# genetics-statistics/GEMMA

Hardware: AMD Instinct MI355X
Metric: SNPs/s (-lmm 1 Wald) at n=20k on 1/2/4/8 MI355X; U^T x HBM GB/s vs roofline (higher is better)
Workload: dtype f64 (U^T x as int8-digit MFMA products with exact int32 accumulation; every column of U scaled by its exact maximum and rounded to 6 base-256 digits = 2^-48 of that maximum -- fp64 keeps 2^-53 per entry; value_strict / strict_leg (7g6m: U^T x at or below the fp64 GEMM's own error) and fp64_gemm_path

## Files before the change

### gemma_amd/build.py

```python
import os
import shutil
import subprocess

HERE = os.path.dirname(os.path.abspath(__file__))
CSRC = os.path.join(HERE, "csrc")
LIB = os.path.join(HERE, "libgemma_hip.so")
UNITS = {
    "gemma_hip.hip": ["dgemm_mfma.hip.h", "lmm_grid.hip.h", "i8gemm.hip.h", "i8gemm_sparse.hip.h", "i8gemm_sparse2.hip.h", "i8gemm_sparse2_r16.hip.h", "i8gemm_dense16.hip.h", "lmm_assoc.hip.h",
                      "lmm_search.hip.h", "comm.hip.h", "comm_shm.hpp", "kin_i8.hip.h", "ingest.hip.h", "qc.hip.h", "lm_assoc.hip.h", "mvlmm.hip.h",
                      "mvlmm_kernels.hip.h", "eigh_tu.h", "tu_common.h",
                      "abi_kinship.inc.h", "abi_eigen_qc.inc.h", "abi_lmm_stage.inc.h", "abi_utx.inc.h", "abi_lmm_batch.inc.h",
                      "abi_mvlmm.inc.h", "abi_gxe_lm.inc.h", "abi_kept_comm.inc.h", "abi_vc.inc.h", "vc_tu.h", "abi_prdt.inc.h", "prdt_tu.h",
                      "abi_mqs.inc.h", "mqs_tu.h", "abi_cor.inc.h", "cor_tu.h"],
    "eigh_tu.hip": ["dgemm_mfma.hip.h", "eigh.hip.h", "eigh2.hip.h", "eigh_tu.h", "tu_common.h"],
    "vc_tu.hip": ["dgemm_mfma.hip.h", "spd_inv.hip.h", "vc.hip.h", "vc_tu.h", "tu_common.h", "host_linalg.h", "../../include/gemma_vc_hybrid.hpp"],
    "prdt_tu.hip": ["dgemm_mfma.hip.h", "geno_mv.hip.h", "dev_common.hip.h", "eigh_tu.h", "prdt_tu.h", "tu_common.h"],
    "mqs_tu.hip": ["dgemm_mfma.hip.h", "mqs.hip.h", "dev_common.hip.h", "mqs_tu.h", "tu_common.h", "host_linalg.h"],
    "cor_tu.hip": ["dgemm_mfma.hip.h", "cor.hip.h", "dev_common.hip.h", "cor_tu.h", "tu_common.h"],
    "mvlmm_kernels.hip": ["mvlmm.hip.h", "mvlmm_kernels.hip.h"],
    "mvlmm_kernels_wide.hip": ["mvlmm.hip.h", "mvlmm_kernels.hip.h"],
    "mvlmm_kernels_rt.hip": ["mvlmm.hip.h", "mvlmm_kernels.hip.h"],
    "mvlmm_kernels_d6.hip": ["mvlmm.hip.h", "mvlmm_kernels.hip.h"],
    "mvlmm_kernels_d7.hip": ["mvlmm.hip.h", "mvlmm_kernels.hip.h"],
    "mvlmm_kernels_d8.hip": ["mvlmm.hip.h", "mvlmm_kernels.hip.h"],
}
PUBLIC_HEADER_USERS = ("gemma_hip.hip", "eigh_tu.hip", "vc_tu.hip", "prdt_tu.hip", "mqs_tu.hip", "cor_tu.hip")
SOURCES = list(UNITS)
HEADERS = sorted({h for hs in UNITS.values() for h in hs})


def hipcc():
    for cand in (os.environ.get("HIPCC"), "/opt/rocm/bin/hipcc", shutil.which("hipcc")):
        if cand and os.path.exists(cand):
            return cand
    raise RuntimeError("hipcc not found: the gfx950 library cannot be built")


def stale():
    if not os.path.exists(LIB):
        return True
    t = os.path.getmtime(LIB)
    deps = [os.path.join(CSRC, f) for f in SOURCES + HEADERS]
    deps.append(os.path.join(HERE, "..", "include", "gemma_hip.h"))
    return any(os.path.getmtime(d) > t for d in deps)


def build(force=False, verbose=False):
    if not force and not stale():
        return LIB
    cc = hipcc()
    objdir = os.path.join(HERE, "_obj")
    os.makedirs(objdir, exist_ok=True)
    procs, objs = [], []
    for src in SOURCES:
        obj = os.path.join(objdir, src.replace(".hip", ".o"))
        objs.append(obj)
        hdrs = UNITS[src]
        deps = [os.path.join(CSRC, f) for f in [src] + hdrs]
        if src in PUBLIC_HEADER_USERS:
            deps.append(os.path.join(HERE, "..", "include", "gemma_hip.h"))
        if not force and os.path.exists(obj) and all(os.path.getmtime(d) <= os.path.getmtime(obj) for d in deps):
            continue
        cmd = [cc, "--offload-arch=gfx950", "-O3", "-std=c++17", "-fPIC", "-c", os.path.join(CSRC, src), "-o", obj]
        if verbose:
            print(" ".join(cmd))
        procs.append((cmd, subprocess.Popen(cmd, cwd=CSRC)))
    for cmd, pr in procs:
        if pr.wait() != 0:
            raise subprocess.CalledProcessError(pr.returncode, cmd)
    cmd = [cc, "--offload-arch=gfx950", "-fPIC", "-shared", "-o", LIB] + objs
    if verbose:
        print(" ".join(cmd))
    subprocess.check_call(cmd, cwd=CSRC)
    return LIB


if __name__ == "__main__":
    print(build(force=True, verbose=True))
```

### gemma_amd/csrc/abi_gxe_lm.inc.h

```cpp

extern "C" int gemma_hip_lmm_set_env(const double *env) {
  NEED_INIT();
  if (!g_ctx.lmm_active) return fail(GEMMA_HIP_ESTATE, "lmm_set_env before lmm_setup");
  if (!env) return fail(GEMMA_HIP_EINVAL, "lmm_set_env: null pointer");
  const size_t n = g_ctx.cfg.n, c = g_ctx.cfg.n_cvt;
  if (c + 2 > (size_t)GEN_CMAX_WIDE)
    return fail(GEMMA_HIP_EINVAL, "lmm_set_env: n_cvt + 2 = %zu covariates not supported (<= %d)", c + 2, GEN_CMAX_WIDE);
  if (n <= c + 3) return fail(GEMMA_HIP_EINVAL, "lmm_set_env: n <= n_cvt + 3");
  if (g_ctx.gxe_env.reserve(n * 8) || g_ctx.gxe_UtWt.reserve((c + 1) * n * 8))
    return fail(GEMMA_HIP_ENOMEM, "lmm_set_env: buffers");
  HIPCHK(hipMemcpy(g_ctx.gxe_env.p, env, n * 8, hipMemcpyHostToDevice));
  HIPCHK(hipMemcpy(g_ctx.gxe_UtWt.p, g_ctx.UtWt.p, c * n * 8, hipMemcpyDeviceToDevice));
  HIPCHK(launch_dgemm('T', 'N', (long)n, 1, (long)n, 1.0, g_ctx.U, (long)n, g_ctx.gxe_env.as<double>(), 1, 0.0,
                      g_ctx.gxe_UtWt.as<double>() + c * n, 1, false, false, 0));
  HIPCHK(hipDeviceSynchronize());
  const double df = (double)n - (double)(c + 2) - 1.0;
  g_ctx.gxe_lnbeta = lgamma(df / 2.0) + lgamma(0.5) - lgamma(df / 2.0 + 0.5);
  g_ctx.gxe_ready = true;
  return GEMMA_HIP_OK;
}

extern "C" int gemma_hip_lmm_gxe_batch_d(int kind, const void *geno, size_t l, size_t ld, gemma_sumstat *out_d,
                                         void *stream) {
  NEED_INIT();
  if (!g_ctx.lmm_active || !g_ctx.gxe_ready) return fail(GEMMA_HIP_ESTATE, "lmm_gxe_batch before lmm_setup + lmm_set_env");
  if (l == 0) return GEMMA_HIP_OK;
  if (kind == GEMMA_GENO_F64_IDV_MAJOR) return fail(GEMMA_HIP_EINVAL, "lmm_gxe_batch: SNP-major input only");
  int rc = check_batch_args("lmm_gxe_batch", kind, geno, l, ld, out_d);
  if (rc) return rc;
  hipStream_t s = S(stream);
  const size_t n = g_ctx.cfg.n, c = g_ctx.cfg.n_cvt;
  const size_t ldx = (n + 1) & ~(size_t)1;
  if (int rcf = xp_flush(s)) return rcf;
  if (g_ctx.X.reserve(l * ldx * 8) || g_ctx.UtX.reserve(l * ldx * 8) || g_ctx.gxe_Z.reserve(l * ldx * 8) ||
      g_ctx.gxe_UtZ.reserve(l * ldx * 8) || g_ctx.gxe_flip.reserve(l * sizeof(int)))
    return fail(GEMMA_HIP_ENOMEM, "lmm_gxe_batch: cannot allocate 4 x %zu bytes", l * ldx * 8);
  double *X = g_ctx.X.as<double>(), *UtX = g_ctx.UtX.as<double>();
  double *Z = g_ctx.gxe_Z.as<double>(), *UtZ = g_ctx.gxe_UtZ.as<double>();
  {
    ProfScope ps(GEMMA_STAGE_INGEST, s);
    IngestGxeArgs a;
    a.src = geno; a.ld = (long)ld; a.l = (long)l;
    a.idx_map = g_ctx.have_map ? g_ctx.idx_map.as<int>() : nullptr;
    a.n = (int)n; a.env = g_ctx.gxe_env.as<double>(); a.X = X; a.Z = Z; a.ldo = (long)ldx;
    a.flip = g_ctx.gxe_flip.as<int>();
    const unsigned grid = (unsigned)((l + 3) / 4);
    if (kind == GEMMA_GENO_PLINK_2BIT)
      hipLaunchKernelGGL(ingest_gxe_kernel<true>, dim3(grid), dim3(256), 0, s, a);
    else
      hipLaunchKernelGGL(ingest_gxe_kernel<false>, dim3(grid), dim3(256), 0, s, a);
    HIPCHK(hipGetLastError());
  }
  {
    ProfScope ps(GEMMA_STAGE_UTX_GEMM, s);
    const double *Ug;
    long ldu;
    int rcu = gemm_U(&Ug, &ldu, s);
    if (rcu) return rcu;
    HIPCHK(launch_dgemm('N', 'N', (long)l, (long)n, (long)n, 1.0, X, (long)ldx, Ug, ldu, 0.0, UtX, (long)ldx,
                        false, false, s));
    HIPCHK(launch_dgemm('N', 'N', (long)l, (long)n, (long)n, 1.0, Z, (long)ldx, Ug, ldu, 0.0, UtZ, (long)ldx,
                        false, false, s));
  }
  AssocArgs a = g_ctx.assoc_proto;
  a.UtX = UtX; a.UtZ = UtZ; a.flip = g_ctx.gxe_flip.as<int>();
  a.ld = (long)ldx; a.l = (long)l;
  a.eval = g_ctx.eval; a.Uty = g_ctx.Uty; a.UtWt = g_ctx.gxe_UtWt.as<double>();
  a.out = reinterpret_cast<SumStat *>(out_d);
  a.lnbeta_half_df = g_ctx.gxe_lnbeta;
  a.grid_T = nullptr;
  a.have_grid = 0;
  a.have_logdet_ends = g_ctx.assoc_proto.have_logdet_ends;
  const unsigned grid = (unsigned)((l + 3) / 4);
  {
    ProfScope ps(GEMMA_STAGE_ASSOC, s);
    switch (c + 2) {
    case 3: hipLaunchKernelGGL(lmm_gxe_kernel<3>, dim3(grid), dim3(256), 0, s, a); break;
    case 4: hipLaunchKernelGGL(lmm_gxe_kernel<4>, dim3(grid), dim3(256), 0, s, a); break;
    default:
      if (c + 2 > (size_t)GEN_CMAX) {
        int rcw = wide_attr(lmm_gxe_wide_kernel);
        if (rcw) return rcw;
        hipLaunchKernelGGL(lmm_gxe_wide_kernel, dim3((unsigned)l), dim3(64), wide_lds_bytes(c + 2), s, a, (int)(c + 2));
      } else {
        hipLaunchKernelGGL(lmm_gxe_generic_kernel, dim3(grid), dim3(256), 0, s, a, (int)(c + 2));
      }
      break;
    }
    HIPCHK(hipGetLastError());
  }
  return GEMMA_HIP_OK;
}

extern "C" int gemma_hip_lmm_gxe_batch(int kind, const void *geno, size_t l, size_t ld, gemma_sumstat *out) {
  NEED_INIT();
  if (!g_ctx.lmm_active || !g_ctx.gxe_ready) return fail(GEMMA_HIP_ESTATE, "lmm_gxe_batch before lmm_setup + lmm_set_env");
  if (l == 0) return GEMMA_HIP_OK;
  if (kind == GEMMA_GENO_F64_IDV_MAJOR) return fail(GEMMA_HIP_EINVAL, "lmm_gxe_batch: SNP-major input only");
  int rc = check_batch_args("lmm_gxe_batch", kind, geno, l, ld, out);
  if (rc) return rc;
  const size_t esz = (kind == GEMMA_GENO_PLINK_2BIT) ? 1 : 8;
  if (g_ctx.stage_in.reserve(l * ld * esz) || g_ctx.stage_out.reserve(l * sizeof(gemma_sumstat)))
    return fail(GEMMA_HIP_ENOMEM, "lmm_gxe_batch: staging %zu bytes", l * ld * esz);
  HIPCHK(hipMemcpy(g_ctx.stage_in.p, geno, l * ld * esz, hipMemcpyHostToDevice));
  rc = gemma_hip_lmm_gxe_batch_d(kind, g_ctx.stage_in.p, l, ld, g_ctx.stage_out.as<gemma_sumstat>(), nullptr);
  if (rc) return rc;
  HIPCHK(hipMemcpy(out, g_ctx.stage_out.p, l * sizeof(gemma_sumstat), hipMemcpyDeviceToHost));
  return GEMMA_HIP_OK;
}

extern "C" int gemma_hip_dbg_utx(int kind, const void *geno, size_t l, size_t ld, int path, double *UtX_host) {
  NEED_INIT();
  if (!g_ctx.lmm_active) return fail(GEMMA_HIP_ESTATE, "dbg_utx before lmm_setup");
  if (l == 0) return GEMMA_HIP_OK;
  int rc = check_batch_args("dbg_utx", kind, geno, l, ld, UtX_host);
  if (rc) return rc;
  const size_t n = g_ctx.cfg.n;
  const size_t rows = (kind == GEMMA_GENO_F64_IDV_MAJOR) ? n : l;
  const size_t esz = (kind == GEMMA_GENO_PLINK_2BIT) ? 1 : 8;
  if (g_ctx.stage_in.reserve(rows * ld * esz)) return fail(GEMMA_HIP_ENOMEM, "dbg_utx: staging");
  HIPCHK(hipMemcpy(g_ctx.stage_in.p, geno, rows * ld * esz, hipMemcpyHostToDevice));
  double *UtX;
  size_t ldx;
  rc = compute_utx(kind, g_ctx.stage_in.p, l, ld, path ? 1 : 0, &UtX, &ldx, 0);
  if (rc) return rc;
  HIPCHK(hipMemcpy2D(UtX_host, n * 8, UtX, ldx * 8, n * 8, l, hipMemcpyDeviceToHost));
  return GEMMA_HIP_OK;
}

extern "C" int gemma_hip_lmm_batch(int kind, const void *geno, size_t l, size_t ld, gemma_sumstat *out) {
  NEED_INIT();
  if (!g_ctx.lmm_active) return fail(GEMMA_HIP_ESTATE, "lmm_batch before lmm_setup");
  if (l == 0) return GEMMA_HIP_OK;
  const size_t n = g_ctx.cfg.n;
  const size_t per_row = (kind == GEMMA_GENO_PLINK_2BIT && g_ctx.have_map) ? g_ctx.ni_total : n;
  const size_t need = min_ld_for(kind, per_row, l);
  if (need == (size_t)-1) return fail(GEMMA_HIP_EINVAL, "lmm_batch: unknown geno_kind %d", kind);
  if (!geno || !out || ld < need) return fail(GEMMA_HIP_EINVAL, "lmm_batch: ld=%zu < %zu", ld, need);
  const size_t rows = (kind == GEMMA_GENO_F64_IDV_MAJOR) ? n : l;
  const size_t esz = (kind == GEMMA_GENO_PLINK_2BIT) ? 1 : 8;
  if (g_ctx.stage_in.reserve(rows * ld * esz) || g_ctx.stage_out.reserve(l * sizeof(gemma_sumstat)))
    return fail(GEMMA_HIP_ENOMEM, "lmm_batch: staging %zu bytes", rows * ld * esz);
  HIPCHK(hipMemcpy2D(g_ctx.stage_in.p, ld * esz, geno, ld * esz, need * esz, rows, hipMemcpyHostToDevice));
  int rc = gemma_hip_lmm_batch_d(kind, g_ctx.stage_in.p, l, ld, g_ctx.stage_out.as<gemma_sumstat>(), nullptr);
  if (rc) return rc;
  HIPCHK(hipMemcpy(out, g_ctx.stage_out.p, l * sizeof(gemma_sumstat), hipMemcpyDeviceToHost));
  return GEMMA_HIP_OK;
}

extern "C" int gemma_hip_lm_setup(int a_mode, size_t n, size_t n_cvt, const double *W, const double *y) {
  NEED_INIT();
  g_ctx.knobs.load();
  if (g_ctx.lmm_active) return fail(GEMMA_HIP_ESTATE, "lm_setup while an LMM run is active");
  if (a_mode < 51 || a_mode > 54) return fail(GEMMA_HIP_EINVAL, "lm_setup: a_mode %d (51..54)", a_mode);
  if (!W || !y || n == 0 || n_cvt == 0 || n_cvt > (size_t)LM_CMAX || n <= n_cvt + 1 || n > 0x7fffffffUL)
    return fail(GEMMA_HIP_EINVAL, "lm_setup: bad arguments (n_cvt 1..%d)", LM_CMAX);
  const int c = (int)n_cvt;
  std::vector<double> WtW((size_t)c * c, 0.0), Wt((size_t)c * n), Wty(c, 0.0);
  double yy = 0.0;
  for (size_t i = 0; i < n; ++i) {
    yy += y[i] * y[i];
    for (int a = 0; a < c; ++a) {
      Wt[(size_t)a * n + i] = W[i * c + a];
      Wty[a] += W[i * c + a] * y[i];
      for (int b = 0; b < c; ++b) WtW[(size_t)a * c + b] += W[i * c + a] * W[i * c + b];
    }
  }
  if (!invert_small(WtW, c)) return fail(GEMMA_HIP_EINVAL, "lm_setup: W^T W is singular");
  double d = 0.0;
  for (int a = 0; a < c; ++a) {
    double t = 0.0;
    for (int b = 0; b < c; ++b) t += WtW[(size_t)a * c + b] * Wty[b];
    d += t * Wty[a];
  }
  if (g_ctx.lm_Wt.reserve(Wt.size() * 8) || g_ctx.lm_y.reserve(n * 8) || g_ctx.lm_small.reserve(((size_t)c * c + c) * 8))
    return fail(GEMMA_HIP_ENOMEM, "lm_setup: allocation");
  HIPCHK(hipMemcpy(g_ctx.lm_Wt.p, Wt.data(), Wt.size() * 8, hipMemcpyHostToDevice));
  HIPCHK(hipMemcpy(g_ctx.lm_y.p, y, n * 8, hipMemcpyHostToDevice));
  HIPCHK(hipMemcpy(g_ctx.lm_small.p, WtW.data(), (size_t)c * c * 8, hipMemcpyHostToDevice));
  HIPCHK(hipMemcpy(g_ctx.lm_small.as<double>() + (size_t)c * c, Wty.data(), c * 8, hipMemcpyHostToDevice));
  LmArgs &a = g_ctx.lm_proto;
  memset(&a, 0, sizeof a);
  a.Wt = g_ctx.lm_Wt.as<double>();
  a.y = g_ctx.lm_y.as<double>();
  a.WtWi = g_ctx.lm_small.as<double>();
  a.Wty = g_ctx.lm_small.as<double>() + (size_t)c * c;
  a.yPwy = yy - d;
  a.n = (int)n;
  a.c = c;
  a.test_mode = a_mode - 50;
  const double df = (double)n - (double)c - 1.0;
  a.lnbeta_half_df = lgamma(df / 2.0) + lgamma(0.5) - lgamma(df / 2.0 + 0.5);
  g_ctx.cfg.n = n;
  g_ctx.cfg.n_cvt = n_cvt;
  g_ctx.have_map = false;
  g_ctx.ni_total = 0;
  g_ctx.lm_active = true;
  return GEMMA_HIP_OK;
}

extern "C" int gemma_hip_lm_batch_d(int kind, const void *geno, size_t l, size_t ld, gemma_sumstat *out_d, void *stream) {
  NEED_INIT();
  if (!g_ctx.lm_active) return fail(GEMMA_HIP_ESTATE, "lm_batch before lm_setup");
  if (l == 0) return GEMMA_HIP_OK;
  const size_t n = g_ctx.cfg.n;
  const size_t per_row = (kind == GEMMA_GENO_PLINK_2BIT && g_ctx.have_map) ? g_ctx.ni_total : n;
  const size_t need = min_ld_for(kind, per_row, l);
  if (need == (size_t)-1) return fail(GEMMA_HIP_EINVAL, "lm_batch: unknown geno_kind %d", kind);
  if (!geno || !out_d || ld < need) return fail(GEMMA_HIP_EINVAL, "lm_batch: ld=%zu < %zu", ld, need);
  hipStream_t s = S(stream);
  const size_t ldx = (n + 1) & ~(size_t)1;
  if (g_ctx.X.reserve(l * ldx * 8)) return fail(GEMMA_HIP_ENOMEM, "lm_batch: cannot allocate %zu bytes", l * ldx * 8);
  double *X = g_ctx.X.as<double>();
  {
    ProfScope ps(GEMMA_STAGE_INGEST, s);
    if (kind == GEMMA_GENO_F64_IDV_MAJOR) {
      dim3 grid((unsigned)((l + 31) / 32), (unsigned)((n + 31) / 32));
      hipLaunchKernelGGL(transpose_kernel, grid, dim3(32, 8), 0, s, reinterpret_cast<const double *>(geno), (long)n,
                         (long)l, (long)ld, X, (long)ldx);
    } else {
      IngestArgs a;
      a.src = geno; a.ld = (long)ld; a.l = (long)l;
      a.idx_map = g_ctx.have_map ? g_ctx.idx_map.as<int>() : nullptr;
      a.n = (int)n; a.dst = X; a.ldo = (long)ldx; a.k_mode = 0;
      const unsigned grid = (unsigned)((l + 3) / 4);
      if (kind == GEMMA_GENO_PLINK_2BIT)
        hipLaunchKernelGGL(ingest_lmm_kernel<true>, dim3(grid), dim3(256), 0, s, a);
      else
        hipLaunchKernelGGL(ingest_lmm_kernel<false>, dim3(grid), dim3(256), 0, s, a);
    }
    HIPCHK(hipGetLastError());
  }
  LmArgs a = g_ctx.lm_proto;
  a.X = X; a.ld = (long)ldx; a.l = (long)l;
  a.out = reinterpret_cast<SumStat *>(out_d);
  {
    ProfScope ps(GEMMA_STAGE_ASSOC, s);
    hipLaunchKernelGGL(lm_assoc_kernel, dim3((unsigned)((l + 3) / 4)), dim3(256), 0, s, a);
    HIPCHK(hipGetLastError());
  }
  return GEMMA_HIP_OK;
}

extern "C" int gemma_hip_lm_batch(int kind, const void *geno, size_t l, size_t ld, gemma_sumstat *out) {
  NEED_INIT();
  if (!g_ctx.lm_active) return fail(GEMMA_HIP_ESTATE, "lm_batch before lm_setup");
  if (l == 0) return GEMMA_HIP_OK;
  const size_t n = g_ctx.cfg.n;
  const size_t per_row = (kind == GEMMA_GENO_PLINK_2BIT && g_ctx.have_map) ? g_ctx.ni_total : n;
  const size_t need = min_ld_for(kind, per_row, l);
  if (need == (size_t)-1) return fail(GEMMA_HIP_EINVAL, "lm_batch: unknown geno_kind %d", kind);
  if (!geno || !out || ld < need) return fail(GEMMA_HIP_EINVAL, "lm_batch: ld=%zu < %zu", ld, need);
  const size_t rows = (kind == GEMMA_GENO_F64_IDV_MAJOR) ? n : l;
  const size_t esz = (kind == GEMMA_GENO_PLINK_2BIT) ? 1 : 8;
  if (g_ctx.stage_in.reserve(rows * ld * esz) || g_ctx.stage_out.reserve(l * sizeof(gemma_sumstat)))
    return fail(GEMMA_HIP_ENOMEM, "lm_batch: staging %zu bytes", rows * ld * esz);
  HIPCHK(hipMemcpy2D(g_ctx.stage_in.p, ld * esz, geno, ld * esz, need * esz, rows, hipMemcpyHostToDevice));
  int rc = gemma_hip_lm_batch_d(kind, g_ctx.stage_in.p, l, ld, g_ctx.stage_out.as<gemma_sumstat>(), nullptr);
  if (rc) return rc;
  HIPCHK(hipMemcpy(out, g_ctx.stage_out.p, l * sizeof(gemma_sumstat), hipMemcpyDeviceToHost));
  return GEMMA_HIP_OK;
}

extern "C" int gemma_hip_lm_finish(void) {
  NEED_INIT();
  if (!g_ctx.lm_active) return fail(GEMMA_HIP_ESTATE, "lm_finish before lm_setup");
  HIPCHK(hipDeviceSynchronize());
  g_ctx.lm_Wt.release(); g_ctx.lm_y.release(); g_ctx.lm_small.release();
  g_ctx.X.release(); g_ctx.stage_in.release(); g_ctx.stage_out.release(); g_ctx.idx_map.release();
  g_ctx.lm_active = false;
  return GEMMA_HIP_OK;
}

extern "C" int gemma_hip_lmm_null(size_t n, size_t n_cvt, const double *eval, const double *UtW,
                                  const double *Uty, double l_min, double l_max, size_t n_region,
                                  double trace_G, double *out8) {
  NEED_INIT();
  if (!eval || !UtW || !Uty || !out8 || n == 0 || n_cvt == 0 || n_cvt > (size_t)GEN_CMAX_WIDE + 1)
    return fail(GEMMA_HIP_EINVAL, "lmm_null: bad arguments (n_cvt 1..%d)", GEN_CMAX_WIDE + 1);
  if (!(l_max > l_min) || n_region == 0 || n_region > (size_t)ASSOC_MAX_REGION || n <= n_cvt)
    return fail(GEMMA_HIP_EINVAL, "lmm_null: l_min/l_max/n_region/n");
  DevBuf dE, dW, dWt, dY, dO;
  auto cleanup = [&]() { dE.release(); dW.release(); dWt.release(); dY.release(); dO.release(); };
  if (dE.reserve(n * 8) || dW.reserve(n * n_cvt * 8) || dWt.reserve(n * n_cvt * 8) || dY.reserve(n * 8) ||
      dO.reserve(sizeof(NullOut))) {
    cleanup();
    return fail(GEMMA_HIP_ENOMEM, "lmm_null: allocation");
  }
  hipError_t e = hipMemcpy(dE.p, eval, n * 8, hipMemcpyHostToDevice);
  if (e == hipSuccess) e = hipMemcpy(dW.p, UtW, n * n_cvt * 8, hipMemcpyHostToDevice);
  if (e == hipSuccess) e = hipMemcpy(dY.p, Uty, n * 8, hipMemcpyHostToDevice);
  if (e == hipSuccess) {
    dim3 grid((unsigned)((n_cvt + 31) / 32), (unsigned)((n + 31) / 32));
    hipLaunchKernelGGL(transpose_kernel, grid, dim3(32, 8), 0, 0, dW.as<double>(), (long)n, (long)n_cvt,
                       (long)n_cvt, dWt.as<double>(), (long)n);
    AssocArgs a;
    memset(&a, 0, sizeof a);
    a.n = (int)n; a.n_region = (int)n_region; a.l_min = l_min; a.l_max = l_max;
    a.eval = dE.as<double>(); a.Uty = dY.as<double>(); a.UtWt = dWt.as<double>();
    const double lambda_interval = log(l_max / l_min) / (double)n_region;
    for (size_t i = 0; i <= n_region; ++i) a.lam_grid[i] = l_min * exp(lambda_interval * (double)i);
    NullOut *o = dO.as<NullOut>();
    switch (n_cvt) {
    case 1: hipLaunchKernelGGL(lmm_null_kernel<0>, dim3(1), dim3(64), 0, 0, a, o); break;
    case 2: hipLaunchKernelGGL(lmm_null_kernel<1>, dim3(1), dim3(64), 0, 0, a, o); break;
    case 3: hipLaunchKernelGGL(lmm_null_kernel<2>, dim3(1), dim3(64), 0, 0, a, o); break;
    case 4: hipLaunchKernelGGL(lmm_null_kernel<3>, dim3(1), dim3(64), 0, 0, a, o); break;
    case 5: hipLaunchKernelGGL(lmm_null_kernel<4>, dim3(1), dim3(64), 0, 0, a, o); break;
    default:
      if (n_cvt - 1 > (size_t)GEN_CMAX) {
        (void)hipFuncSetAttribute(reinterpret_cast<const void *>(lmm_null_wide_kernel),
                                  hipFuncAttributeMaxDynamicSharedMemorySize, (int)wide_lds_bytes(GEN_CMAX_WIDE));
        hipLaunchKernelGGL(lmm_null_wide_kernel, dim3(1), dim3(64), wide_lds_bytes(n_cvt - 1), 0, a, (int)n_cvt - 1, o);
      } else {
        hipLaunchKernelGGL(lmm_null_generic_kernel, dim3(1), dim3(64), 0, 0, a, (int)n_cvt - 1, o);
      }
      break;
    }
    e = hipGetLastError();
  }
  NullOut h;
  if (e == hipSuccess) e = hipMemcpy(&h, dO.p, sizeof h, hipMemcpyDeviceToHost);
  cleanup();
  if (e != hipSuccess) return fail(GEMMA_HIP_ERUNTIME, "lmm_null: %s", hipGetErrorString(e));
  out8[0] = h.l_mle; out8[1] = h.logl_mle; out8[2] = h.l_remle; out8[3] = h.logl_remle;
  double arg = -1.0 / h.dev2_remle, d1 = arg;
  if (arg < 0.001) d1 = fabs(arg);
  const double se = (d1 < 0.0) ? NAN : sqrt(d1);
  out8[4] = trace_G * h.l_remle / (trace_G * h.l_remle + 1.0);
  out8[5] = trace_G / ((trace_G * h.l_remle + 1.0) * (trace_G * h.l_remle + 1.0)) * se;
  out8[7] = h.Pyy_remle / (double)(n - n_cvt);
  out8[6] = out8[7] * h.l_remle;
  return GEMMA_HIP_OK;
}

extern "C" int gemma_hip_lmm_finish(double *time_UtX_min, double *time_opt_min) {
  NEED_INIT();
  if (!g_ctx.lmm_active) return fail(GEMMA_HIP_ESTATE, "lmm_finish before lmm_setup");
  HIPCHK(hipDeviceSynchronize());
  pipe_release();
  xp_release();
  prof_collect(GEMMA_STAGE_UTX_GEMM);
  prof_collect(GEMMA_STAGE_UTX_POST);
  prof_collect(GEMMA_STAGE_ASSOC);
  if (time_UtX_min)
    *time_UtX_min = (g_ctx.prof[GEMMA_STAGE_UTX_GEMM].acc_ms + g_ctx.prof[GEMMA_STAGE_UTX_POST].acc_ms) / 60000.0;
  if (time_opt_min) *time_opt_min = g_ctx.prof[GEMMA_STAGE_ASSOC].acc_ms / 60000.0;
  g_ctx.own_U.release(); g_ctx.own_eval.release(); g_ctx.own_Uty.release(); g_ctx.own_UtW.release();
  g_ctx.UtWt.release(); g_ctx.idx_map.release(); g_ctx.X.release(); g_ctx.UtX.release();
  g_ctx.stage_in.release(); g_ctx.stage_out.release();
  g_ctx.grid_R.release(); g_ctx.grid_F.release(); g_ctx.grid_T.release();
  g_ctx.table_P.release();
  g_ctx.cheb_R.release(); g_ctx.cheb_F.release(); g_ctx.cheb_T.release(); g_ctx.cheb_slots.release();
  g_ctx.cheb_list.release(); g_ctx.cheb_count.release(); g_ctx.cheb_D.release(); g_ctx.cheb_Ck.release();
  g_ctx.cheb_Gk.release(); g_ctx.cheb_Lk.release(); g_ctx.cheb_iv.release(); g_ctx.cheb_dends.release(); g_ctx.cheb_res.release();
  g_ctx.i8_Bt.release(); g_ctx.i8_q.release(); g_ctx.i8_qinv.release(); g_ctx.i8_cmax.release(); g_ctx.i8_A.release(); g_ctx.i8_C.release();
  raster_release();
  g_ctx.i8_mean.release(); g_ctx.i8_meta.release(); g_ctx.i8_rowsur.release(); g_ctx.i8_colsum.release(); g_ctx.i8_surlist.release();
  g_ctx.i8_ready = false;
  g_ctx.i8_colsum_ready = false;
  g_ctx.gxe_env.release(); g_ctx.gxe_UtWt.release(); g_ctx.gxe_Z.release(); g_ctx.gxe_UtZ.release();
  g_ctx.mv_Yt.release(); g_ctx.mv_out.release(); g_ctx.mv_scratch.release();
  g_ctx.mv_ready = g_ctx.mv_gxe = false;
  g_ctx.gxe_flip.release();
  g_ctx.gxe_ready = false;
  g_ctx.U = g_ctx.eval = g_ctx.Uty = nullptr;
  g_ctx.U_even_of = nullptr;
  g_ctx.U_even.release();
  g_ctx.lmm_active = false;
  return GEMMA_HIP_OK;
}
```

### gemma_amd/csrc/abi_kinship.inc.h

```cpp

extern "C" int gemma_hip_kin_begin(size_t n_total, int k_mode) {
  NEED_INIT();
  if (n_total == 0) return fail(GEMMA_HIP_EINVAL, "kin_begin: n_total == 0");
  if (k_mode != 1 && k_mode != 2) return fail(GEMMA_HIP_EINVAL, "kin_begin: k_mode %d", k_mode);
  g_ctx.qc_G.release(); g_ctx.qc_M.release(); g_ctx.qc_W.release(); g_ctx.qc_O.release();
  g_ctx.kin_ingested_valid = false;
  if (g_ctx.kin_K.reserve(n_total * n_total * 8))
    return fail(GEMMA_HIP_ENOMEM, "kin_begin: cannot allocate K (%zu bytes)", n_total * n_total * 8);
  HIPCHK(hipMemsetAsync(g_ctx.kin_K.p, 0, n_total * n_total * 8, 0));
  g_ctx.kin_active = true;
  g_ctx.kin_n = n_total;
  g_ctx.kin_mode = k_mode;
  g_ctx.kin_ns = 0;
  g_ctx.knobs.load();
  g_ctx.kin_i8 = (k_mode == 1) && g_ctx.knobs.kin_i8;
  g_ctx.kin_i8_used = false;
  return GEMMA_HIP_OK;
}

static void kin_i8_release() {
  g_ctx.kin_GtG.release(); g_ctx.kin_S.release(); g_ctx.kin_a.release(); g_ctx.kin_At.release(); g_ctx.kin_Gt.release();
  g_ctx.kin_A2.release(); g_ctx.kin_cnt.release(); g_ctx.kin_off.release(); g_ctx.kin_listS.release();
  g_ctx.kin_listJ.release(); g_ctx.kin_sub.release(); g_ctx.kin_cj.release(); g_ctx.kin_flag.release();
  g_ctx.kin_tmap.release();
  g_ctx.kin_tmap_tm = g_ctx.kin_tmap_tn = g_ctx.kin_tmap_count = 0;
  g_ctx.kin_i8_used = false;
}

static int kin_i8_tile_map(int tiles_m, int tiles_n) {
  if (g_ctx.kin_tmap_tm == tiles_m && g_ctx.kin_tmap_tn == tiles_n && g_ctx.kin_tmap.p) return GEMMA_HIP_OK;
  std::vector<int> map;
  const int GM = 8;
  for (int first = 0; first < tiles_m; first += GM) {
    const int gsz = std::min(GM, tiles_m - first);
    for (int tn = first >> 1; tn < tiles_n; ++tn)
      for (int tm = first; tm < first + gsz; ++tm)
        if (tn >= (tm >> 1)) {
          map.push_back(tm);
          map.push_back(tn);
        }
  }
  if (g_ctx.kin_tmap.reserve(map.size() * sizeof(int))) return fail(GEMMA_HIP_ENOMEM, "kin_add: tile map");
  HIPCHK(hipMemcpy(g_ctx.kin_tmap.p, map.data(), map.size() * sizeof(int), hipMemcpyHostToDevice));
  g_ctx.kin_tmap_tm = tiles_m;
  g_ctx.kin_tmap_tn = tiles_n;
  g_ctx.kin_tmap_count = (int)(map.size() / 2);
  return GEMMA_HIP_OK;
}

static int kin_add_i8(const void *geno, size_t l, size_t ld, hipStream_t s) {
  const size_t n = g_ctx.kin_n;
  const size_t ldk = (n + I8_BK - 1) / I8_BK * I8_BK;
  const size_t ldl = (l + I8_BK - 1) / I8_BK * I8_BK;
  const size_t rows_a = (n + I8P_BM - 1) / I8P_BM * I8P_BM;
  const size_t rows_b = (n + I8_BN - 1) / I8_BN * I8_BN;
  const size_t rows_t = std::max(rows_a, rows_b);
  if (!g_ctx.kin_i8_used) {
    if (g_ctx.kin_GtG.reserve(n * n * 8) || g_ctx.kin_S.reserve(n * n * 8) || g_ctx.kin_a.reserve((n + 1) * 8))
      return fail(GEMMA_HIP_ENOMEM, "kin_add: integer-path accumulators (%zu bytes)", 2 * n * n * 8);
    HIPCHK(hipMemsetAsync(g_ctx.kin_GtG.p, 0, n * n * 8, s));
    HIPCHK(hipMemsetAsync(g_ctx.kin_S.p, 0, n * n * 8, s));
    HIPCHK(hipMemsetAsync(g_ctx.kin_a.p, 0, (n + 1) * 8, s));
    g_ctx.kin_i8_used = true;
  }
  if (g_ctx.i8_A.reserve(l * ldk) || g_ctx.i8_mean.reserve(l * 8) || g_ctx.kin_At.reserve(rows_t * ldl) ||
      g_ctx.kin_Gt.reserve(rows_t * ldl) || g_ctx.i8_C.reserve(rows_a * rows_b * 4))
    return fail(GEMMA_HIP_ENOMEM, "kin_add: integer-path buffers");
  {
    ProfScope ps(GEMMA_STAGE_INGEST, s);
    IngestI8Args a;
    a.src = reinterpret_cast<const unsigned char *>(geno); a.ld = (long)ld; a.l = (long)l; a.idx_map = nullptr;
    a.n = (int)n; a.A = g_ctx.i8_A.as<int8_t>(); a.ldk = (long)ldk; a.mean = g_ctx.i8_mean.as<double>();
    hipLaunchKernelGGL(ingest_i8_kernel, dim3((unsigned)((l + 3) / 4)), dim3(256), 0, s, a);
    HIPCHK(hipGetLastError());
    if (g_ctx.kin_host_call) {
      HIPCHK(hipEventRecord(g_ctx.kin_ingested, s));
      g_ctx.kin_ingested_valid = true;
    }
    hipLaunchKernelGGL(kin_i8_transpose_kernel, dim3((unsigned)((ldl + 63) / 64), (unsigned)((rows_t + 63) / 64)), dim3(256), 0,
                       s, g_ctx.i8_A.as<int8_t>(), (long)l, (long)ldk, (long)n, g_ctx.kin_At.as<int8_t>(),
                       g_ctx.kin_Gt.as<int8_t>(), (long)ldl, (long)rows_t);
    HIPCHK(hipGetLastError());
  }
  {
    ProfScope ps(GEMMA_STAGE_KIN_GEMM, s);
    static bool attr_set = false;
    if (!attr_set) {
      HIPCHK(hipFuncSetAttribute(reinterpret_cast<const void *>(i8gemm_packed_kernel_t<false>),
                                 hipFuncAttributeMaxDynamicSharedMemorySize, 3 * I8P_STAGE));
      attr_set = true;
    }
    I8PackArgs g;
    g.A = g_ctx.kin_At.as<int8_t>();
    g.Bt = g_ctx.kin_Gt.as<int8_t>();
    g.C = g_ctx.i8_C.as<int>();
    g.ldk = (long)ldl; g.ldc = (long)rows_b;
    g.strideB = 0; g.strideC = 0;
    g.m_row0 = (long)rows_a;
    g.tiles_m = (int)(rows_a / I8P_BM); g.tiles_n = (int)(rows_b / I8_BN);
    g.nk = (int)(ldl / I8_BK);
    g.gm = 0; g.fuse = 0; g.digits = 1;
    unsigned ntiles = (unsigned)(g.tiles_m * g.tiles_n);
    {
      if (g_ctx.knobs.kin_upper) {
        if (int rc = kin_i8_tile_map(g.tiles_m, g.tiles_n)) return rc;
        g.tile_map = g_ctx.kin_tmap.as<int>();
        ntiles = (unsigned)g_ctx.kin_tmap_count;
      }
    }
    hipLaunchKernelGGL(i8gemm_packed_kernel_t<false>, dim3(ntiles, 1), dim3(512), 3 * I8P_STAGE, s, g);
    HIPCHK(hipGetLastError());
    hipLaunchKernelGGL(kin_i8_accum_kernel, dim3((unsigned)((n + 255) / 256), (unsigned)std::min<size_t>(n, 32768)), dim3(256), 0, s,
                       g_ctx.i8_C.as<int>(), (long)rows_b, (long)n, g_ctx.kin_GtG.as<double>());
    HIPCHK(hipGetLastError());
    KinCorrArgs c;
    c.A = g_ctx.i8_A.as<int8_t>(); c.At = g_ctx.kin_At.as<int8_t>(); c.mean = g_ctx.i8_mean.as<double>();
    c.l = (long)l; c.ldk = (long)ldk; c.ldl = (long)ldl; c.n = (long)n;
    c.S = g_ctx.kin_S.as<double>(); c.a = g_ctx.kin_a.as<double>(); c.smu2 = g_ctx.kin_a.as<double>() + n;
    c.lists_ok = nullptr;
    bool lists = g_ctx.knobs.kin_lists && l < ((size_t)1 << 18);
    const unsigned nseg = (unsigned)((n + KI8_SEG - 1) / KI8_SEG);
    size_t cap = std::max<size_t>(l * n / 16, (size_t)1 << 20);
    if (g_ctx.knobs.kin_list_cap) cap = std::max<size_t>((size_t)g_ctx.knobs.kin_list_cap, 1);
    cap = std::min<size_t>(cap, (size_t)1 << 30);
    const size_t ld2 = (size_t)256 * nseg;
    if (lists && (g_ctx.knobs.kin_lists_oom ||
                  g_ctx.kin_A2.reserve(l * ld2 * 4) || g_ctx.kin_cnt.reserve((l + n) * 4) || g_ctx.kin_off.reserve((l + n + 2) * 4) ||
                  g_ctx.kin_listS.reserve(cap * 4) || g_ctx.kin_listJ.reserve(cap * 4) ||
                  g_ctx.kin_sub.reserve(l * (size_t)(nseg + 1) * 4) || g_ctx.kin_cj.reserve(n * 8) || g_ctx.kin_flag.reserve(16))) {
      (void)hipGetLastError();
      lists = false;
    }
    if (lists) {
      int *cntS = g_ctx.kin_cnt.as<int>(), *cntJ = cntS + l, *offS = g_ctx.kin_off.as<int>(), *offJ = offS + l + 1;
      int *ok = g_ctx.kin_flag.as<int>();
      hipLaunchKernelGGL(kin_i8_pack2_kernel, dim3((unsigned)l, nseg), dim3(256), 0, s, g_ctx.i8_A.as<int8_t>(), (long)l,
                         (long)ldk, (int)nseg, g_ctx.kin_A2.as<unsigned>());
      hipLaunchKernelGGL(kin_i8_count_kernel, dim3((unsigned)((l + 3) / 4)), dim3(256), 0, s, g_ctx.i8_A.as<int8_t>(), (long)l,
                         (long)ldk, (long)ldk, cntS);
      hipLaunchKernelGGL(kin_i8_count_kernel, dim3((unsigned)((n + 3) / 4)), dim3(256), 0, s, g_ctx.kin_At.as<int8_t>(), (long)n,
                         (long)ldl, (long)ldl, cntJ);
      KinScanArgs sc;
      sc.cntS = cntS; sc.cntJ = cntJ; sc.offS = offS; sc.offJ = offJ; sc.l = (long)l; sc.n = (long)n; sc.cap = (long)cap;
      sc.ok = ok; sc.mean = g_ctx.i8_mean.as<double>(); sc.smu2 = g_ctx.kin_a.as<double>() + n;
      hipLaunchKernelGGL(kin_i8_scan_kernel, dim3(1), dim3(1024), 0, s, sc);
      hipLaunchKernelGGL(kin_i8_fill_kernel<false>, dim3((unsigned)((l + 3) / 4)), dim3(256), 0, s, g_ctx.i8_A.as<int8_t>(),
                         (long)l, (long)ldk, (long)ldk, offS, g_ctx.kin_listS.as<int>(), ok, (const double *)nullptr, (long)l,
                         (double *)nullptr, (double *)nullptr);
      hipLaunchKernelGGL(kin_i8_fill_kernel<true>, dim3((unsigned)((n + 3) / 4)), dim3(256), 0, s, g_ctx.kin_At.as<int8_t>(),
                         (long)n, (long)ldl, (long)ldl, offJ, g_ctx.kin_listJ.as<int>(), ok, g_ctx.i8_mean.as<double>(), (long)l,
                         g_ctx.kin_a.as<double>(), g_ctx.kin_cj.as<double>());
      hipLaunchKernelGGL(kin_i8_sub_kernel, dim3((unsigned)((l * (nseg + 1) + 255) / 256)), dim3(256), 0, s, offS,
                         g_ctx.kin_listS.as<int>(), (long)l, (int)nseg, ok, g_ctx.kin_sub.as<int>());
      KinCorr2Args c2;
      c2.A2 = g_ctx.kin_A2.as<unsigned>(); c2.ld2 = (long)ld2; c2.mean = g_ctx.i8_mean.as<double>(); c2.n = (long)n;
      c2.offJ = offJ; c2.listJ = g_ctx.kin_listJ.as<int>(); c2.offS = offS; c2.listS = g_ctx.kin_listS.as<int>();
      c2.sub = g_ctx.kin_sub.as<int>(); c2.nseg = (int)nseg; c2.cj = g_ctx.kin_cj.as<double>();
      c2.S = g_ctx.kin_S.as<double>(); c2.ok = ok;
      c2.dbg_skip_pairs = c2.dbg_skip_main = 0;
#ifdef GEMMA_HIP_KIN_TIMING_SWITCHES
      {
        const char *ed = getenv("GEMMA_HIP_KIN_DBG");
        c2.dbg_skip_pairs = (ed && ed[0] == '1') ? 1 : 0;
        c2.dbg_skip_main = (ed && ed[0] == '2') ? 1 : 0;
      }
#endif
      hipLaunchKernelGGL(kin_i8_corr2_kernel, dim3((unsigned)n, nseg), dim3(256), 0, s, c2);
      HIPCHK(hipGetLastError());
      c.lists_ok = ok;
    }
    hipLaunchKernelGGL(kin_i8_corr_kernel, dim3((unsigned)n, nseg), dim3(256), 0, s, c);
    HIPCHK(hipGetLastError());
  }
  g_ctx.kin_ns += l;
  return GEMMA_HIP_OK;
}

static int kin_fold_i8(hipStream_t s) {
  if (!g_ctx.kin_i8_used) return GEMMA_HIP_OK;
  const size_t n = g_ctx.kin_n;
  const unsigned nb = (unsigned)((n + 31) / 32);
  hipLaunchKernelGGL(kin_i8_fold_kernel, dim3(nb, nb), dim3(32, 8), 0, s, g_ctx.kin_K.as<double>(), (long)n,
                     g_ctx.kin_GtG.as<double>(), g_ctx.kin_S.as<double>(), g_ctx.kin_a.as<double>(),
                     g_ctx.kin_a.as<double>() + n);
  HIPCHK(hipGetLastError());
  HIPCHK(hipStreamSynchronize(s));
  kin_i8_release();
  return GEMMA_HIP_OK;
}

static size_t min_ld_for(int kind, size_t n_items_per_row, size_t l) {
  switch (kind) {
  case GEMMA_GENO_F64_SNP_MAJOR: return n_items_per_row;
  case GEMMA_GENO_PLINK_2BIT: return (n_items_per_row + 3) / 4;
  case GEMMA_GENO_F64_IDV_MAJOR: return l;
  default: return (size_t)-1;
  }
}

extern "C" int gemma_hip_kin_add_d(int kind, const void *geno, size_t l, size_t ld, void *stream) {
  NEED_INIT();
  if (!g_ctx.kin_active) return fail(GEMMA_HIP_ESTATE, "kin_add before kin_begin");
  if (l == 0) return GEMMA_HIP_OK;
  const size_t n = g_ctx.kin_n;
  const size_t need = min_ld_for(kind, n, l);
  if (need == (size_t)-1) return fail(GEMMA_HIP_EINVAL, "kin_add: unknown geno_kind %d", kind);
  if (!geno || ld < need) return fail(GEMMA_HIP_EINVAL, "kin_add: ld=%zu < %zu", ld, need);
  hipStream_t s = S(stream);
  if (g_ctx.kin_i8 && kind == GEMMA_GENO_PLINK_2BIT) return kin_add_i8(geno, l, ld, s);
  const size_t ldx = (n + 1) & ~(size_t)1;
  if (g_ctx.kin_X.reserve(l * ldx * 8))
    return fail(GEMMA_HIP_ENOMEM, "kin_add: cannot allocate %zu bytes", l * ldx * 8);
  double *X = g_ctx.kin_X.as<double>();
  {
    ProfScope ps(GEMMA_STAGE_INGEST, s);
    if (kind == GEMMA_GENO_F64_IDV_MAJOR) {
      dim3 grid((unsigned)((l + 31) / 32), (unsigned)((n + 31) / 32));
      hipLaunchKernelGGL(transpose_kernel, grid, dim3(32, 8), 0, s,
                         reinterpret_cast<const double *>(geno), (long)n, (long)l, (long)ld, X, (long)ldx);
    } else {
      IngestArgs a;
      a.src = geno; a.ld = (long)ld; a.l = (long)l; a.idx_map = nullptr; a.n = (int)n;
      a.dst = X; a.ldo = (long)ldx; a.k_mode = g_ctx.kin_mode;
      const unsigned grid = (unsigned)((l + 3) / 4);
      if (kind == GEMMA_GENO_PLINK_2BIT)
        hipLaunchKernelGGL(ingest_kin_kernel<true>, dim3(grid), dim3(256), 0, s, a);
      else
        hipLaunchKernelGGL(ingest_kin_kernel<false>, dim3(grid), dim3(256), 0, s, a);
    }
    HIPCHK(hipGetLastError());
  }
  if (g_ctx.kin_host_call) {
    HIPCHK(hipEventRecord(g_ctx.kin_ingested, s));
    g_ctx.kin_ingested_valid = true;
  }
  {
    ProfScope ps(GEMMA_STAGE_KIN_GEMM, s);
    HIPCHK(launch_dgemm('T', 'N', (long)n, (long)n, (long)l, 1.0, X, (long)ldx, X, (long)ldx, 1.0,
                        g_ctx.kin_K.as<double>(), (long)n, true, false, s));
  }
  g_ctx.kin_ns += l;
  return GEMMA_HIP_OK;
}

extern "C" int gemma_hip_kin_add(int kind, const void *geno, size_t l, size_t ld) {
  NEED_INIT();
  if (!g_ctx.kin_active) return fail(GEMMA_HIP_ESTATE, "kin_add before kin_begin");
  if (l == 0) return GEMMA_HIP_OK;
  const size_t n = g_ctx.kin_n;
  const size_t need = min_ld_for(kind, n, l);
  if (need == (size_t)-1) return fail(GEMMA_HIP_EINVAL, "kin_add: unknown geno_kind %d", kind);
  if (!geno || ld < need) return fail(GEMMA_HIP_EINVAL, "kin_add: ld=%zu < %zu", ld, need);
  const size_t rows = (kind == GEMMA_GENO_F64_IDV_MAJOR) ? n : l;
  const size_t esz = (kind == GEMMA_GENO_PLINK_2BIT) ? 1 : 8;
  const size_t bytes = rows * ld * esz;
  if (bytes > g_ctx.kin_stage.cap) g_ctx.kin_ingested_valid = false;
  if (g_ctx.kin_stage.reserve(bytes)) return fail(GEMMA_HIP_ENOMEM, "kin_add: staging %zu bytes", bytes);
  const size_t width = need * esz;
  if (!g_ctx.kin_copy) {
    if (hipStreamCreateWithFlags(&g_ctx.kin_copy, hipStreamNonBlocking) != hipSuccess ||
        hipEventCreateWithFlags(&g_ctx.kin_copied, hipEventDisableTiming) != hipSuccess ||
        hipEventCreateWithFlags(&g_ctx.kin_ingested, hipEventDisableTiming) != hipSuccess) {
      (void)hipGetLastError();
      if (g_ctx.kin_copy) (void)hipStreamDestroy(g_ctx.kin_copy);
      g_ctx.kin_copy = nullptr;
    }
  }
  if (!g_ctx.kin_copy) {
    HIPCHK(hipMemcpy2D(g_ctx.kin_stage.p, ld * esz, geno, ld * esz, width, rows, hipMemcpyHostToDevice));
    return gemma_hip_kin_add_d(kind, g_ctx.kin_stage.p, l, ld, nullptr);
  }
  if (g_ctx.kin_ingested_valid) HIPCHK(hipStreamWaitEvent(g_ctx.kin_copy, g_ctx.kin_ingested, 0));
  HIPCHK(hipMemcpy2DAsync(g_ctx.kin_stage.p, ld * esz, geno, ld * esz, width, rows, hipMemcpyHostToDevice, g_ctx.kin_copy));
  HIPCHK(hipEventRecord(g_ctx.kin_copied, g_ctx.kin_copy));
  HIPCHK(hipStreamWaitEvent(nullptr, g_ctx.kin_copied, 0));
  g_ctx.kin_host_call = true;
  const int rc = gemma_hip_kin_add_d(kind, g_ctx.kin_stage.p, l, ld, nullptr);
  g_ctx.kin_host_call = false;
  HIPCHK(hipEventSynchronize(g_ctx.kin_copied));
  return rc;
}

extern "C" int gemma_hip_kin_end_d(double *K_d, size_t *ns_used, void *stream) {
  NEED_INIT();
  if (!g_ctx.kin_active) return fail(GEMMA_HIP_ESTATE, "kin_end before kin_begin");
  const size_t n = g_ctx.kin_n;
  hipStream_t s = S(stream);
  {
    int rc = kin_fold_i8(s);
    if (rc) return rc;
  }
  if (ns_used) *ns_used = g_ctx.kin_ns;
  const double scale = g_ctx.kin_ns ? 1.0 / (double)g_ctx.kin_ns : 1.0;
  const unsigned nb = (unsigned)((n + 31) / 32);
  hipLaunchKernelGGL(symm_fill_scale_kernel, dim3(nb, nb), dim3(32, 8), 0, s, g_ctx.kin_K.as<double>(),
                     (long)n, (long)n, scale);
  HIPCHK(hipGetLastError());
  if (K_d) HIPCHK(hipMemcpyAsync(K_d, g_ctx.kin_K.p, n * n * 8, hipMemcpyDeviceToDevice, s));
  HIPCHK(hipStreamSynchronize(s));
  g_ctx.kin_active = false;
  g_ctx.kin_X.release();
  g_ctx.kin_stage.release();
  g_ctx.kin_K.release();
  return GEMMA_HIP_OK;
}

extern "C" int gemma_hip_kin_end(double *K, size_t *ns_used) {
  NEED_INIT();
  if (!g_ctx.kin_active) return fail(GEMMA_HIP_ESTATE, "kin_end before kin_begin");
  const size_t n = g_ctx.kin_n;
  {
    int rc = kin_fold_i8(nullptr);
    if (rc) return rc;
  }
  if (ns_used) *ns_used = g_ctx.kin_ns;
  const double scale = g_ctx.kin_ns ? 1.0 / (double)g_ctx.kin_ns : 1.0;
  const unsigned nb = (unsigned)((n + 31) / 32);
  hipLaunchKernelGGL(symm_fill_scale_kernel, dim3(nb, nb), dim3(32, 8), 0, 0, g_ctx.kin_K.as<double>(),
                     (long)n, (long)n, scale);
  HIPCHK(hipGetLastError());
  if (K) HIPCHK(hipMemcpy(K, g_ctx.kin_K.p, n * n * 8, hipMemcpyDeviceToHost));
  g_ctx.kin_active = false;
  g_ctx.kin_X.release();
  g_ctx.kin_stage.release();
  g_ctx.kin_K.release();
  return GEMMA_HIP_OK;
}
```

### gemma_amd/csrc/abi_lmm_batch.inc.h

```cpp

static void xp_release() {
  Ctx::XPipe &x = g_ctx.xp;
  if (x.P) (void)hipStreamDestroy(x.P);
  if (x.Q) (void)hipStreamDestroy(x.Q);
  if (x.in_ready) (void)hipEventDestroy(x.in_ready);
  if (x.ingest_done) (void)hipEventDestroy(x.ingest_done);
  x.ingest_done = nullptr;
  x.ingest_valid = false;
  for (int i = 0; i < 2; ++i) {
    if (x.prod_done[i]) (void)hipEventDestroy(x.prod_done[i]);
    if (x.post_done[i]) (void)hipEventDestroy(x.post_done[i]);
    x.prod_done[i] = x.post_done[i] = nullptr;
    x.post_valid[i] = false;
  }
  x.P = x.Q = nullptr;
  x.in_ready = nullptr;
  x.count = 0;
  x.pending = false;
  x.cus = -1;
  x.shadow_A.release(); x.shadow_C.release(); x.shadow_mean.release(); x.shadow_rowsur.release();
}
static int xp_init() {
  Ctx::XPipe &x = g_ctx.xp;
  const int ncu = g_ctx.prop.multiProcessorCount;
  int cus = g_ctx.knobs.pipe_cus;
  if (cus < 0 || cus * 2 > ncu || ncu % 32 != 0 || cus % 8 != 0 || (cus && (ncu / 8) % (cus / 8) != 0)) cus = 0;
  if (x.P && x.cus == cus) return GEMMA_HIP_OK;
  HIPCHK(hipDeviceSynchronize());
  xp_release();
  if (cus > 0) {
    const int words = ncu / 32, per_xcd = cus / 8, cu_per_xcd = ncu / 8, stepj = cu_per_xcd / per_xcd;
    std::vector<unsigned> mp((size_t)words, 0xFFFFFFFFu), mq((size_t)words, 0u);
    for (int j = 0; j < cu_per_xcd; j += stepj)
      for (int xcd = 0; xcd < 8; ++xcd) {
        const int c = 8 * j + xcd;
        mp[c >> 5] &= ~(1u << (c & 31));
        mq[c >> 5] |= 1u << (c & 31);
      }
    HIPCHK(hipExtStreamCreateWithCUMask(&x.P, (uint32_t)words, mp.data()));
    HIPCHK(hipExtStreamCreateWithCUMask(&x.Q, (uint32_t)words, mq.data()));
  } else {
    HIPCHK(hipStreamCreateWithFlags(&x.P, hipStreamDefault));
    HIPCHK(hipStreamCreateWithFlags(&x.Q, hipStreamDefault));
  }
  HIPCHK(hipEventCreateWithFlags(&x.in_ready, hipEventDisableTiming));
  HIPCHK(hipEventCreateWithFlags(&x.ingest_done, hipEventDisableTiming));
  for (int i = 0; i < 2; ++i) {
    HIPCHK(hipEventCreateWithFlags(&x.prod_done[i], hipEventDisableTiming));
    HIPCHK(hipEventCreateWithFlags(&x.post_done[i], hipEventDisableTiming));
  }
  x.cus = cus;
  return GEMMA_HIP_OK;
}
static int xp_flush(hipStream_t s) {
  Ctx::XPipe &x = g_ctx.xp;
  if (!x.pending) return GEMMA_HIP_OK;
  for (int i = 0; i < 2; ++i)
    if (x.post_valid[i]) HIPCHK(hipStreamWaitEvent(s, x.post_done[i], 0));
  x.pending = false;
  x.ingest_valid = false;
  return GEMMA_HIP_OK;
}
static int xp_abort(int rc) {
  Ctx::XPipe &x = g_ctx.xp;
  (void)hipDeviceSynchronize();
  x.count = 0;
  x.post_valid[0] = x.post_valid[1] = false;
  x.pending = false;
  x.ingest_valid = false;
  return rc;
}
static void xp_swap_sets() {
  Ctx::XPipe &x = g_ctx.xp;
  std::swap(g_ctx.i8_A, x.shadow_A); std::swap(g_ctx.i8_C, x.shadow_C);
  std::swap(g_ctx.i8_mean, x.shadow_mean); std::swap(g_ctx.i8_rowsur, x.shadow_rowsur);
}


static int compute_utx(int kind, const void *geno, size_t l, size_t ld, int path, double **UtX_out, size_t *ldx_out,
                       hipStream_t s) {
  {
    int rcf = xp_flush(s);
    if (rcf) return rcf;
  }
  const size_t n = g_ctx.cfg.n;
  const size_t ldx = (n + 1) & ~(size_t)1;
  const bool want_i8 = (path < 0 ? utx_i8_mode() == 1 : path == 1);
  const bool plink_i8 = want_i8 && kind == GEMMA_GENO_PLINK_2BIT;
  if (g_ctx.UtX.reserve(l * ldx * 8) || (!plink_i8 && g_ctx.X.reserve(l * ldx * 8)))
    return fail(GEMMA_HIP_ENOMEM, "lmm_batch: cannot allocate 2 x %zu bytes", l * ldx * 8);
  double *UtX = g_ctx.UtX.as<double>();
  *UtX_out = UtX;
  *ldx_out = ldx;
  g_ctx.last_utx_path = plink_i8 ? 1 : 0;
  if (plink_i8) return utx_plink_i8(geno, l, ld, UtX, ldx, s);
  double *X = g_ctx.X.as<double>();
  bool done = false;
  if (kind == GEMMA_GENO_F64_IDV_MAJOR) {
    {
      ProfScope ps(GEMMA_STAGE_INGEST, s);
      dim3 grid((unsigned)((l + 31) / 32), (unsigned)((n + 31) / 32));
      hipLaunchKernelGGL(transpose_kernel, grid, dim3(32, 8), 0, s, reinterpret_cast<const double *>(geno),
                         (long)n, (long)l, (long)ld, X, (long)ldx);
      HIPCHK(hipGetLastError());
    }
    if (want_i8) {
      int rc = utx_f64_try_i8(X, l, ldx, false, UtX, ldx, s, &done);
      if (rc) return rc;
    }
  } else if (kind == GEMMA_GENO_F64_SNP_MAJOR && want_i8) {
    int rc = utx_f64_try_i8(reinterpret_cast<const double *>(geno), l, ld, true, UtX, ldx, s, &done);
    if (rc) return rc;
  }
  if (done) return GEMMA_HIP_OK;
  if (kind != GEMMA_GENO_F64_IDV_MAJOR) {
    ProfScope ps(GEMMA_STAGE_INGEST, s);
    IngestArgs a;
    a.src = geno; a.ld = (long)ld; a.l = (long)l;
    a.idx_map = g_ctx.have_map ? g_ctx.idx_map.as<int>() : nullptr;
    a.n = (int)n; a.dst = X; a.ldo = (long)ldx; a.k_mode = 0;
    const unsigned grid = (unsigned)((l + 3) / 4);
    if (kind == GEMMA_GENO_PLINK_2BIT)
      hipLaunchKernelGGL(ingest_lmm_kernel<true>, dim3(grid), dim3(256), 0, s, a);
    else
      hipLaunchKernelGGL(ingest_lmm_kernel<false>, dim3(grid), dim3(256), 0, s, a);
    HIPCHK(hipGetLastError());
  }
  {
    ProfScope ps(GEMMA_STAGE_UTX_GEMM, s);
    const double *Ug;
    long ldu;
    int rcu = gemm_U(&Ug, &ldu, s);
    if (rcu) return rcu;
    note_utx_kernel(GEMMA_UTX_KERNEL_DGEMM_F64, 0, 0, 0);
    HIPCHK(launch_dgemm('N', 'N', (long)l, (long)n, (long)n, 1.0, X, (long)ldx, Ug, ldu, 0.0, UtX,
                        (long)ldx, false, false, s));
  }
  return GEMMA_HIP_OK;
}

static int check_batch_args(const char *who, int kind, const void *geno, size_t l, size_t ld, const void *out) {
  const size_t n = g_ctx.cfg.n;
  const size_t per_row = (kind == GEMMA_GENO_PLINK_2BIT && g_ctx.have_map) ? g_ctx.ni_total : n;
  const size_t need = min_ld_for(kind, per_row, l);
  if (need == (size_t)-1) return fail(GEMMA_HIP_EINVAL, "%s: unknown geno_kind %d", who, kind);
  if (!geno || !out || ld < need) return fail(GEMMA_HIP_EINVAL, "%s: ld=%zu < %zu", who, ld, need);
  return GEMMA_HIP_OK;
}

static int overlap_chunks(size_t l) {
  if (!g_ctx.knobs.overlap) return 1;
  if (utx_i8_mode() != 1 || i8_sparse_mode() != 2) return 1;
  int q = g_ctx.knobs.overlap_chunks;
  q = std::max(1, std::min(q, 16));
  while (q > 1 && l < (size_t)q * 2 * S2_BM) --q;
  return q;
}
static int overlap_init() {
  if (g_ctx.ov_stream) return GEMMA_HIP_OK;
  HIPCHK(hipStreamCreateWithFlags(&g_ctx.ov_stream, hipStreamNonBlocking));
  for (auto &e : g_ctx.ov_ready) HIPCHK(hipEventCreateWithFlags(&e, hipEventDisableTiming));
  HIPCHK(hipEventCreateWithFlags(&g_ctx.ov_done, hipEventDisableTiming));
  return GEMMA_HIP_OK;
}
static int lmm_batch_plink_chunked(const void *geno, size_t l, size_t ld, gemma_sumstat *out_d, int chunks, hipStream_t s) {
  const size_t n = g_ctx.cfg.n;
  const size_t ldx = (n + 1) & ~(size_t)1;
  int rc = overlap_init();
  if (rc) return rc;
  if (g_ctx.UtX.reserve(l * ldx * 8)) return fail(GEMMA_HIP_ENOMEM, "lmm_batch: cannot allocate %zu bytes", l * ldx * 8);
  double *UtX = g_ctx.UtX.as<double>();
  g_ctx.last_utx_path = 1;
  I8Dims d;
  if ((rc = i8_begin(l, &d, s))) return rc;
  {
    ProfScope ps(GEMMA_STAGE_INGEST, s);
    IngestI8Args a;
    a.src = reinterpret_cast<const unsigned char *>(geno); a.ld = (long)ld; a.l = (long)l;
    a.idx_map = g_ctx.have_map ? g_ctx.idx_map.as<int>() : nullptr;
    a.n = (int)d.n; a.A = g_ctx.i8_A.as<int8_t>(); a.ldk = (long)d.ldk;
    a.mean = g_ctx.i8_mean.as<double>();
    hipLaunchKernelGGL(ingest_i8_kernel, dim3((unsigned)((l + 3) / 4)), dim3(256), 0, s, a);
    HIPCHK(hipGetLastError());
  }
  if ((rc = i8_meta_build(d, s))) return rc;
  const size_t per = round_up((l + chunks - 1) / chunks, (size_t)S2_BM);
  hipStream_t side = g_ctx.ov_stream;
  int c = 0;
  for (size_t row0 = 0; row0 < l; row0 += per, ++c) {
    const size_t rows = std::min(per, l - row0), rows_pad = std::min(per, d.lpad - row0);
    if ((rc = i8_gemm_rows(d, row0, rows_pad, s, UtX, ldx, rows))) break;
    if (hipEventRecord(g_ctx.ov_ready[c], s) != hipSuccess || hipStreamWaitEvent(side, g_ctx.ov_ready[c], 0) != hipSuccess) {
      rc = fail(GEMMA_HIP_ERUNTIME, "lmm_batch: %s", hipGetErrorString(hipGetLastError()));
      break;
    }
    if ((rc = i8_post_rows(l, d, row0, rows, UtX, ldx, side))) break;
    if ((rc = launch_assoc(UtX + row0 * ldx, rows, ldx, out_d + row0, side))) break;
  }
  (void)hipEventRecord(g_ctx.ov_done, side);
  (void)hipStreamWaitEvent(s, g_ctx.ov_done, 0);
  return rc;
}

static int xp_flush_fwd(hipStream_t s) { return xp_flush(s); }

extern "C" int gemma_hip_lmm_pipe_flush(void *stream) {
  NEED_INIT();
  return xp_flush(S(stream));
}

extern "C" int gemma_hip_lmm_batch_pipe_d(int kind, const void *geno, size_t l, size_t ld, gemma_sumstat *out_d, void *stream) {
  NEED_INIT();
  if (!g_ctx.lmm_active) return fail(GEMMA_HIP_ESTATE, "lmm_batch_pipe before lmm_setup");
  if (l == 0) return GEMMA_HIP_OK;
  int rc = check_batch_args("lmm_batch_pipe", kind, geno, l, ld, out_d);
  if (rc) return rc;
  hipStream_t s = S(stream);
  if (kind != GEMMA_GENO_PLINK_2BIT || utx_i8_mode() != 1 || i8_sparse_mode() != 2) {
    if ((rc = xp_flush(s))) return rc;
    return gemma_hip_lmm_batch_d(kind, geno, l, ld, out_d, stream);
  }
  if ((rc = xp_init())) return rc;
  Ctx::XPipe &x = g_ctx.xp;
  const int slot = (int)(x.count & 1);
  const size_t n = g_ctx.cfg.n;
  const size_t ldx = (n + 1) & ~(size_t)1;
  if (g_ctx.UtX.reserve(l * ldx * 8)) return fail(GEMMA_HIP_ENOMEM, "lmm_batch_pipe: cannot allocate %zu bytes", l * ldx * 8);
  if (s != nullptr && x.ingest_valid) HIPCHK(hipStreamWaitEvent(s, x.ingest_done, 0));
  xp_swap_sets();
  if (s != nullptr) {
    HIPCHK(hipEventRecord(x.in_ready, s));
    HIPCHK(hipStreamWaitEvent(x.P, x.in_ready, 0));
  }
  if (x.post_valid[slot]) HIPCHK(hipStreamWaitEvent(x.P, x.post_done[slot], 0));
  g_ctx.last_utx_path = 1;
  I8Dims d;
  if ((rc = i8_begin(l, &d, x.P, false))) return xp_abort(rc);
  {
    ProfScope ps(GEMMA_STAGE_INGEST, x.P);
    IngestI8Args a;
    a.src = reinterpret_cast<const unsigned char *>(geno); a.ld = (long)ld; a.l = (long)l;
    a.idx_map = g_ctx.have_map ? g_ctx.idx_map.as<int>() : nullptr;
    a.n = (int)d.n; a.A = g_ctx.i8_A.as<int8_t>(); a.ldk = (long)d.ldk;
    a.mean = g_ctx.i8_mean.as<double>();
    hipLaunchKernelGGL(ingest_i8_kernel, dim3((unsigned)((l + 3) / 4)), dim3(256), 0, x.P, a);
    if (hipGetLastError() != hipSuccess) return xp_abort(fail(GEMMA_HIP_ERUNTIME, "lmm_batch_pipe: ingest launch"));
  }
  if (hipEventRecord(x.ingest_done, x.P) != hipSuccess) return xp_abort(fail(GEMMA_HIP_ERUNTIME, "lmm_batch_pipe: event"));
  x.ingest_valid = true;
  if ((rc = i8_meta_build(d, x.P))) return xp_abort(rc);
  if ((rc = i8_gemm_rows(d, 0, d.lpad, x.P))) return xp_abort(rc);
  HIPCHK(hipEventRecord(x.prod_done[slot], x.P));
  HIPCHK(hipStreamWaitEvent(x.Q, x.prod_done[slot], 0));
  double *UtX = g_ctx.UtX.as<double>();
  rc = i8_post_rows(l, d, 0, l, UtX, ldx, x.Q);
  if (!rc) rc = launch_assoc(UtX, l, ldx, out_d, x.Q);
  (void)hipEventRecord(x.post_done[slot], x.Q);
  x.post_valid[slot] = true;
  x.pending = true;
  x.count += 1;
  return rc;
}

extern "C" int gemma_hip_lmm_batch_d(int kind, const void *geno, size_t l, size_t ld, gemma_sumstat *out_d,
                                     void *stream) {
  NEED_INIT();
  if (!g_ctx.lmm_active) return fail(GEMMA_HIP_ESTATE, "lmm_batch before lmm_setup");
  if (l == 0) return GEMMA_HIP_OK;
  int rc = check_batch_args("lmm_batch", kind, geno, l, ld, out_d);
  if (rc) return rc;
  hipStream_t s = S(stream);
  if ((rc = xp_flush(s))) return rc;
  if (kind == GEMMA_GENO_PLINK_2BIT) {
    const int chunks = overlap_chunks(l);
    if (chunks > 1) return lmm_batch_plink_chunked(geno, l, ld, out_d, chunks, s);
  }
  double *UtX;
  size_t ldx;
  rc = compute_utx(kind, geno, l, ld, -1, &UtX, &ldx, s);
  if (rc) return rc;
  return launch_assoc(UtX, l, ldx, out_d, s);
}

extern "C" int gemma_hip_lmm_gene_batch_d(const double *Y_d, size_t l, size_t ld, gemma_sumstat *out_d, void *stream) {
  NEED_INIT();
  if (!g_ctx.lmm_active) return fail(GEMMA_HIP_ESTATE, "lmm_gene_batch before lmm_setup");
  if (l == 0) return GEMMA_HIP_OK;
  const size_t n = g_ctx.cfg.n, c = g_ctx.cfg.n_cvt;
  if (!Y_d || !out_d || ld < n) return fail(GEMMA_HIP_EINVAL, "lmm_gene_batch: ld=%zu < n=%zu", ld, n);
  hipStream_t s = S(stream);
  const size_t ldx = (n + 1) & ~(size_t)1;
  if (int rcf = xp_flush(S(stream))) return rcf;
  if (g_ctx.UtX.reserve(l * ldx * 8)) return fail(GEMMA_HIP_ENOMEM, "lmm_gene_batch: %zu bytes", l * ldx * 8);
  double *UtY = g_ctx.UtX.as<double>();
  {
    ProfScope ps(GEMMA_STAGE_UTX_GEMM, s);
    const double *Ug;
    long ldu;
    int rcu = gemm_U(&Ug, &ldu, s);
    if (rcu) return rcu;
    HIPCHK(launch_dgemm('N', 'N', (long)l, (long)n, (long)n, 1.0, Y_d, (long)ld, Ug, ldu, 0.0, UtY, (long)ldx,
                        false, false, s));
  }
  AssocArgs a = g_ctx.assoc_proto;
  a.UtX = UtY; a.ld = (long)ldx; a.l = (long)l;
  a.eval = g_ctx.eval; a.Uty = g_ctx.Uty; a.UtWt = g_ctx.UtWt.as<double>();
  a.out = reinterpret_cast<SumStat *>(out_d);
  a.grid_T = nullptr;
  a.have_grid = 0;
  const unsigned grid = (unsigned)((l + 3) / 4);
  {
    ProfScope ps(GEMMA_STAGE_ASSOC, s);
    switch (c) {
    case 1: hipLaunchKernelGGL(lmm_gene_kernel<1>, dim3(grid), dim3(256), 0, s, a); break;
    case 2: hipLaunchKernelGGL(lmm_gene_kernel<2>, dim3(grid), dim3(256), 0, s, a); break;
    case 3: hipLaunchKernelGGL(lmm_gene_kernel<3>, dim3(grid), dim3(256), 0, s, a); break;
    case 4: hipLaunchKernelGGL(lmm_gene_kernel<4>, dim3(grid), dim3(256), 0, s, a); break;
    default:
      if (c > (size_t)GEN_CMAX) {
        int rcw = wide_attr(lmm_gene_wide_kernel);
        if (rcw) return rcw;
        hipLaunchKernelGGL(lmm_gene_wide_kernel, dim3((unsigned)l), dim3(64), wide_lds_bytes(c), s, a, (int)c);
      } else {
        hipLaunchKernelGGL(lmm_gene_generic_kernel, dim3(grid), dim3(256), 0, s, a, (int)c);
      }
      break;
    }
    HIPCHK(hipGetLastError());
  }
  return GEMMA_HIP_OK;
}

extern "C" int gemma_hip_lmm_gene_batch(const double *Y, size_t l, size_t ld, gemma_sumstat *out) {
  NEED_INIT();
  if (!g_ctx.lmm_active) return fail(GEMMA_HIP_ESTATE, "lmm_gene_batch before lmm_setup");
  if (l == 0) return GEMMA_HIP_OK;
  const size_t n = g_ctx.cfg.n;
  if (!Y || !out || ld < n) return fail(GEMMA_HIP_EINVAL, "lmm_gene_batch: ld=%zu < n=%zu", ld, n);
  if (g_ctx.stage_in.reserve(l * ld * 8) || g_ctx.stage_out.reserve(l * sizeof(gemma_sumstat)))
    return fail(GEMMA_HIP_ENOMEM, "lmm_gene_batch: staging %zu bytes", l * ld * 8);
  HIPCHK(hipMemcpy(g_ctx.stage_in.p, Y, l * ld * 8, hipMemcpyHostToDevice));
  int rc = gemma_hip_lmm_gene_batch_d(g_ctx.stage_in.as<double>(), l, ld, g_ctx.stage_out.as<gemma_sumstat>(), nullptr);
  if (rc) return rc;
  HIPCHK(hipMemcpy(out, g_ctx.stage_out.p, l * sizeof(gemma_sumstat), hipMemcpyDeviceToHost));
  return GEMMA_HIP_OK;
}
```

### gemma_amd/csrc/abi_utx.inc.h

```cpp

struct I8Dims {
  size_t n, ldk, npad, lpad, mrows;
  int fuse, digits, nplanes;
  int mdrop;
  int complete;
  int epi;
};
static const int *i8_anymiss(const I8Dims &d) { return d.complete ? g_ctx.i8_rowsur.as<int>() + d.lpad : nullptr; }
static int i8_sparse_mode() { return g_ctx.knobs.i8_sparse; }
static int i8_begin(size_t l, I8Dims *d, hipStream_t s, bool allow_epi = true) {
  int rc = i8_prepare_u(s);
  if (rc) return rc;
  d->n = g_ctx.cfg.n; d->ldk = g_ctx.i8_ldk; d->npad = g_ctx.i8_npad;
  d->lpad = round_up(l, i8_sparse_mode() == 2 ? (size_t)S2_BM : (size_t)I8P_BM); d->mrows = 2 * d->lpad;
  d->fuse = (g_ctx.knobs.i8_fuse && (double)d->n * 2.0 * 128.0 * 257.0 < 2147483648.0) ? 1 : 0;
  d->digits = g_ctx.i8_digits;
  d->nplanes = d->fuse ? (d->digits + 1) / 2 : d->digits;
  d->mdrop = (g_ctx.knobs.i8_mdrop && d->fuse && d->digits == 7 && i8_sparse_mode() == 2 && g_ctx.knobs.i8_rows == 16) ? 1 : 0;
  d->complete = (g_ctx.knobs.i8_complete && i8_sparse_mode() == 2 && g_ctx.knobs.i8_rows == 16) ? 1 : 0;
  d->epi = (allow_epi && g_ctx.knobs.i8_epilogue && i8_sparse_mode() == 2 && g_ctx.knobs.i8_rows == 16 && d->nplanes >= 2) ? 1 : 0;
  const size_t c_elems = (size_t)(d->nplanes - d->epi) * d->mrows * d->npad;
  if (g_ctx.i8_A.reserve(d->lpad * d->ldk) || g_ctx.i8_C.reserve(c_elems * 4) || g_ctx.i8_mean.reserve(l * 8))
    return fail(GEMMA_HIP_ENOMEM, "lmm_batch: int8 product buffers (%zu bytes)", d->lpad * d->ldk + c_elems * 4);
  if (d->lpad != l) HIPCHK(hipMemsetAsync(g_ctx.i8_A.p, 0, d->lpad * d->ldk, s));
  return GEMMA_HIP_OK;
}

static int i8_meta_build(const I8Dims &d, hipStream_t s) {
  const int mode = i8_sparse_mode();
  if (mode == 0) return GEMMA_HIP_OK;
  ProfScope ps(GEMMA_STAGE_INGEST, s);
  const size_t nk = d.ldk / I8_BK, total = d.lpad * nk * (mode == 2 ? 4 : 2);
  if (g_ctx.i8_meta.reserve(total * sizeof(uint4)) || g_ctx.i8_rowsur.reserve((d.lpad + 1) * sizeof(int)))
    return fail(GEMMA_HIP_ENOMEM, "lmm_batch: mask words of the sparse product");
  HIPCHK(hipMemsetAsync(g_ctx.i8_rowsur.p, 0, (d.lpad + 1) * sizeof(int), s));
  if (mode == 2)
    hipLaunchKernelGGL(sparse2_meta_kernel, dim3((unsigned)((total + 255) / 256)), dim3(256), 0, s, g_ctx.i8_A.as<int8_t>(),
                       (long)d.lpad, (long)d.ldk, g_ctx.i8_meta.as<uint4>(), g_ctx.i8_rowsur.as<int>(),
                       const_cast<int *>(i8_anymiss(d)));
  else
    hipLaunchKernelGGL(sparse_meta_kernel, dim3((unsigned)((total + 255) / 256)), dim3(256), 0, s, g_ctx.i8_A.as<int8_t>(),
                       (long)d.lpad, (long)d.ldk, g_ctx.i8_meta.as<uint4>(), g_ctx.i8_rowsur.as<int>());
  HIPCHK(hipGetLastError());
  g_ctx.i8_flag_at = (mode == 2 && d.complete) ? (long)d.lpad : -1;
  g_ctx.i8_rowsur_n = (long)d.lpad;
  return GEMMA_HIP_OK;
}

static int raster_for(int tiles_m, int tiles_n, int rb, hipStream_t s, const int2 **map_d) {
  Ctx::RasterSlot *lru = &g_ctx.i8_raster[0];
  for (auto &r : g_ctx.i8_raster) {
    if (r.tm == tiles_m && r.tn == tiles_n && r.rb == rb && r.dev.p) {
      r.used = ++g_ctx.i8_raster_clock;
      *map_d = r.dev.as<int2>();
      return GEMMA_HIP_OK;
    }
    if (r.used < lru->used) lru = &r;
  }
  if (lru->dev.p) HIPCHK(hipDeviceSynchronize());
  s2_build_raster(tiles_m, tiles_n, rb, lru->host);
  lru->tm = lru->tn = lru->rb = 0;
  if (lru->dev.reserve(lru->host.size() * sizeof(int2)))
    return fail(GEMMA_HIP_ENOMEM, "lmm_batch: tile raster (%zu bytes)", lru->host.size() * sizeof(int2));
  HIPCHK(hipMemcpyAsync(lru->dev.p, lru->host.data(), lru->host.size() * sizeof(int2), hipMemcpyHostToDevice, s));
  HIPCHK(hipStreamSynchronize(s));
  lru->tm = tiles_m; lru->tn = tiles_n; lru->rb = rb;
  lru->used = ++g_ctx.i8_raster_clock;
  *map_d = lru->dev.as<int2>();
  return GEMMA_HIP_OK;
}

static int i8_gemm_rows(const I8Dims &d, size_t row0, size_t rows_pad, hipStream_t s, double *UtX = nullptr, size_t ldx = 0,
                        size_t rows = 0) {
  const int mode = i8_sparse_mode();
  const bool sparse = mode != 0;
  if (d.epi && (mode != 2 || g_ctx.knobs.i8_rows != 16 || !UtX || rows == 0))
    return fail(GEMMA_HIP_ESTATE, "lmm_batch: the epilogue form of the int8 product without its destination");
  g_ctx.i8_last_epi = d.epi;
  ProfScope ps(GEMMA_STAGE_UTX_GEMM, s);
  static bool attr_set = false;
  if (!attr_set) {
    HIPCHK(hipFuncSetAttribute(reinterpret_cast<const void *>(i8gemm_packed_kernel_t<true>),
                               hipFuncAttributeMaxDynamicSharedMemorySize, 3 * I8P_STAGE));
    attr_set = true;
  }
  I8PackArgs g;
  g.A = g_ctx.i8_A.as<int8_t>();
  g.Bt = g_ctx.i8_Bt.as<int8_t>();
  g.C = g_ctx.i8_C.as<int>();
  g.ldk = (long)d.ldk; g.ldc = (long)d.npad;
  g.strideB = (long)(d.npad * d.ldk); g.strideC = (long)(d.mrows * d.npad);
  g.m_row0 = (long)d.lpad;
  g.tiles_m = (int)(d.lpad / I8P_BM); g.tiles_n = (int)(d.npad / I8_BN);
  g.nk = (int)(d.ldk / I8_BK);
  g.gm = g_ctx.knobs.i8_gm;
  g.fuse = d.fuse;
  g.digits = d.digits;
  const dim3 grid((unsigned)(g.tiles_m * g.tiles_n), (unsigned)d.nplanes);
  if (mode == 2) {
    static bool attr3 = false;
    if (!attr3) {
      HIPCHK(hipFuncSetAttribute(reinterpret_cast<const void *>(i8gemm_sparse2_kernel),
                                 hipFuncAttributeMaxDynamicSharedMemorySize, S2_NST * S2_STAGE));
      HIPCHK(hipFuncSetAttribute(reinterpret_cast<const void *>(i8gemm_sparse2_r16_kernel),
                                 hipFuncAttributeMaxDynamicSharedMemorySize, S2_R16_LDS));
      HIPCHK(hipFuncSetAttribute(reinterpret_cast<const void *>(i8gemm_sparse2_r16_g_kernel),
                                 hipFuncAttributeMaxDynamicSharedMemorySize, S2_R16_LDS));
      HIPCHK(hipFuncSetAttribute(reinterpret_cast<const void *>(i8gemm_sparse2_r16_ep_kernel),
                                 hipFuncAttributeMaxDynamicSharedMemorySize, S2_R16_LDS));
      HIPCHK(hipFuncSetAttribute(reinterpret_cast<const void *>(i8gemm_sparse2_r16_ep_g_kernel),
                                 hipFuncAttributeMaxDynamicSharedMemorySize, S2_R16_LDS));
      attr3 = true;
    }
    Sparse2Args g2;
    g2.AM = g_ctx.i8_meta.as<uint4>() + (row0 / S2_BM) * (size_t)g.nk * S2_BM * 4;
    g2.Bt = g.Bt; g2.C = g.C + row0 * (size_t)g.ldc - (d.epi ? g.strideC : 0); g2.ldk = g.ldk; g2.ldc = g.ldc; g2.strideB = g.strideB; g2.strideC = g.strideC;
    g2.m_row0 = g.m_row0;
    g2.tiles_m = (int)(rows_pad / S2_BM); g2.tiles_n = (int)(d.npad / S2_BN);
    g2.nk = g.nk; g2.gm = g.gm; g2.fuse = g.fuse; g2.digits = g.digits;
    int raster_rb = 0;
    {
      const int rb = g_ctx.knobs.i8_raster;
      if (rb > 0) {
        const int2 *map_d = nullptr;
        int rc_map = raster_for(g2.tiles_m, g2.tiles_n, rb, s, &map_d);
        if (rc_map) return rc_map;
        g2.tile_map = map_d;
        raster_rb = rb;
      }
    }
    note_utx_kernel(g_ctx.knobs.i8_rows == 32 ? GEMMA_UTX_KERNEL_RECORDS_R32 : GEMMA_UTX_KERNEL_RECORDS_R16, d.digits, d.fuse,
                    raster_rb);
    if (g_ctx.knobs.i8_rows == 32) {
      hipLaunchKernelGGL(i8gemm_sparse2_kernel, dim3((unsigned)(g2.tiles_m * g2.tiles_n), (unsigned)d.nplanes), dim3(512),
                         S2_NST * S2_STAGE, s, g2);
    } else if (d.epi) {
      const unsigned wgs = (unsigned)(g2.tiles_m * g2.tiles_n);
      g2.anymiss = i8_anymiss(d);
      g2.plane0 = 1;
      g2.run_if = g2.anymiss ? 1 : 0;
      hipLaunchKernelGGL(i8gemm_sparse2_r16_kernel, dim3(wgs, (unsigned)d.nplanes - 1u), dim3(512), S2_R16_LDS, s, g2);
      if (g2.anymiss) {
        g2.run_if = 2;
        hipLaunchKernelGGL(i8gemm_sparse2_r16_g_kernel, dim3(wgs, (unsigned)d.nplanes - 1u), dim3(512), S2_R16_LDS, s, g2);
      }
      g2.plane0 = 0;
      g2.UtX = UtX + row0 * ldx; g2.ldx = (long)ldx; g2.l = (long)rows; g2.n = (long)d.n;
      g2.mean = g_ctx.i8_mean.as<double>() + row0; g2.qinv = g_ctx.i8_qinv.as<double>();
      g2.m_scale = 1.0; g2.nplanes = d.nplanes;
      if (d.mdrop) {
        g2.run_if = 0;
        hipLaunchKernelGGL(i8gemm_sparse2_r16_ep_g_kernel, dim3(wgs, 1u), dim3(512), S2_R16_LDS, s, g2);
      } else {
        g2.run_if = g2.anymiss ? 1 : 0;
        hipLaunchKernelGGL(i8gemm_sparse2_r16_ep_kernel, dim3(wgs, 1u), dim3(512), S2_R16_LDS, s, g2);
        if (g2.anymiss) {
          g2.run_if = 2;
          hipLaunchKernelGGL(i8gemm_sparse2_r16_ep_g_kernel, dim3(wgs, 1u), dim3(512), S2_R16_LDS, s, g2);
        }
      }
    } else {
      const unsigned wgs = (unsigned)(g2.tiles_m * g2.tiles_n), first = d.mdrop ? 1u : 0u;
      g2.anymiss = i8_anymiss(d);
      g2.plane0 = (int)first;
      g2.run_if = g2.anymiss ? 1 : 0;
      hipLaunchKernelGGL(i8gemm_sparse2_r16_kernel, dim3(wgs, (unsigned)d.nplanes - first), dim3(512), S2_R16_LDS, s, g2);
      if (g2.anymiss) {
        g2.run_if = 2;
        hipLaunchKernelGGL(i8gemm_sparse2_r16_g_kernel, dim3(wgs, (unsigned)d.nplanes - first), dim3(512), S2_R16_LDS, s, g2);
      }
      if (d.mdrop) {
        g2.plane0 = 0; g2.run_if = 0;
        hipLaunchKernelGGL(i8gemm_sparse2_r16_g_kernel, dim3(wgs, 1u), dim3(512), S2_R16_LDS, s, g2);
      }
    }
  } else if (sparse) {
    static bool attr2 = false;
    if (!attr2) {
      HIPCHK(hipFuncSetAttribute(reinterpret_cast<const void *>(i8gemm_sparse_kernel),
                                 hipFuncAttributeMaxDynamicSharedMemorySize, 3 * SP_STAGE));
      attr2 = true;
    }
    SparseMeta sm;
    sm.m4 = g_ctx.i8_meta.as<uint4>();
    sm.row_surplus = g_ctx.i8_rowsur.as<int>();
    sm.ntiles = (long)g.nk;
    note_utx_kernel(GEMMA_UTX_KERNEL_SPARSE_BYTES, d.digits, d.fuse, 0);
    hipLaunchKernelGGL(i8gemm_sparse_kernel, grid, dim3(512), 3 * SP_STAGE, s, g, sm);
  } else {
    note_utx_kernel(GEMMA_UTX_KERNEL_DENSE_I8, d.digits, d.fuse, 0);
    hipLaunchKernelGGL(i8gemm_packed_kernel_t<true>, grid, dim3(512), 3 * I8P_STAGE, s, g);
  }
  HIPCHK(hipGetLastError());
  return GEMMA_HIP_OK;
}

static int i8_post_rows(size_t l, const I8Dims &d, size_t row0, size_t rows, double *UtX, size_t ldx, hipStream_t s) {
  const bool sparse = i8_sparse_mode() != 0;
  ProfScope ps(GEMMA_STAGE_UTX_POST, s);
  int *sur_cnt = nullptr, *sur_list = nullptr;
  const int8_t *Arow = g_ctx.i8_A.as<int8_t>() + row0 * d.ldk;
  if (sparse) {
    if (g_ctx.i8_surlist.reserve(l * (SUR_MAX + 1) * sizeof(int)))
      return fail(GEMMA_HIP_ENOMEM, "lmm_batch: dropped-call lists");
    sur_cnt = g_ctx.i8_surlist.as<int>() + row0;
    sur_list = g_ctx.i8_surlist.as<int>() + l + row0 * SUR_MAX;
    hipLaunchKernelGGL(i8_surplus_list_kernel, dim3((unsigned)((rows + 3) / 4)), dim3(256), 0, s, Arow, (long)d.ldk,
                       g_ctx.i8_rowsur.as<int>() + row0, (long)rows, sur_cnt, sur_list);
    HIPCHK(hipGetLastError());
  }
  if (!d.epi) {
    hipLaunchKernelGGL(i8_combine_kernel, dim3((unsigned)((d.n + 1023) / 1024), (unsigned)std::min<size_t>(rows, 65535)),
                       dim3(256), 0, s,
                       g_ctx.i8_C.as<int>() + row0 * d.npad, (long)d.npad, (long)(d.mrows * d.npad), (long)d.lpad,
                       g_ctx.i8_mean.as<double>() + row0, g_ctx.i8_qinv.as<double>(), (long)rows, (long)d.n, UtX + row0 * ldx, (long)ldx,
                       1.0, d.fuse, d.digits, sur_cnt, sur_list, g_ctx.U, (long)d.n, d.mdrop, i8_anymiss(d));
    HIPCHK(hipGetLastError());
  } else if (sparse) {
    hipLaunchKernelGGL(i8_surplus_short_kernel, dim3((unsigned)rows), dim3(256), 0, s, sur_cnt, sur_list,
                       g_ctx.i8_mean.as<double>() + row0, g_ctx.U, (long)d.n, (long)d.n, (long)rows, UtX + row0 * ldx, (long)ldx);
    HIPCHK(hipGetLastError());
  }
  if (sparse) {
    hipLaunchKernelGGL(i8_surplus_fix_kernel, dim3((unsigned)rows), dim3(256), 0, s, Arow, (long)d.ldk,
                       g_ctx.i8_rowsur.as<int>() + row0, g_ctx.i8_mean.as<double>() + row0, g_ctx.U, (long)d.n, (long)d.n,
                       (long)rows, UtX + row0 * ldx, (long)ldx, SUR_MAX);
    HIPCHK(hipGetLastError());
  }
  return GEMMA_HIP_OK;
}

static int i8_product(size_t l, const I8Dims &d, double *UtX, size_t ldx, hipStream_t s) {
  int rc = i8_meta_build(d, s);
  if (!rc) rc = i8_gemm_rows(d, 0, d.lpad, s, UtX, ldx, l);
  if (!rc) rc = i8_post_rows(l, d, 0, l, UtX, ldx, s);
  return rc;
}

static int utx_plink_i8(const void *geno, size_t l, size_t ld, double *UtX, size_t ldx, hipStream_t s) {
  I8Dims d;
  int rc = i8_begin(l, &d, s);
  if (rc) return rc;
  {
    ProfScope ps(GEMMA_STAGE_INGEST, s);
    IngestI8Args a;
    a.src = reinterpret_cast<const unsigned char *>(geno); a.ld = (long)ld; a.l = (long)l;
    a.idx_map = g_ctx.have_map ? g_ctx.idx_map.as<int>() : nullptr;
    a.n = (int)d.n; a.A = g_ctx.i8_A.as<int8_t>(); a.ldk = (long)d.ldk;
    a.mean = g_ctx.i8_mean.as<double>();
    hipLaunchKernelGGL(ingest_i8_kernel, dim3((unsigned)((l + 3) / 4)), dim3(256), 0, s, a);
    HIPCHK(hipGetLastError());
  }
  return i8_product(l, d, UtX, ldx, s);
}

static bool dosage_i8_enabled() { return g_ctx.knobs.dosage_i8 != 0; }
static int utx_dosage_i8(const double *src, size_t l, size_t ld, bool nan_missing, bool two, bool have_m, const I8Dims &d,
                         double *UtX, size_t ldx, hipStream_t s) {
  const int np = (two ? 2 : 1) + (have_m ? 1 : 0);
  const size_t plane_a = d.lpad * d.ldk, plane_c = d.lpad * d.npad;
  if (g_ctx.i8_A.reserve((size_t)np * plane_a) || g_ctx.i8_C.reserve((size_t)np * d.digits * plane_c * 4) ||
      g_ctx.i8_colsum.reserve(d.n * 8))
    return fail(GEMMA_HIP_ENOMEM, "lmm_batch: dosage planes (%zu bytes)", (size_t)np * (plane_a + d.digits * plane_c * 4));
  int8_t *A0 = g_ctx.i8_A.as<int8_t>();
  {
    ProfScope ps(GEMMA_STAGE_INGEST, s);
    if (d.lpad != l) HIPCHK(hipMemsetAsync(A0, 0, (size_t)np * plane_a, s));
    PackDosageArgs a;
    a.src = src; a.ld = (long)ld; a.l = (long)l; a.n = (int)d.n; a.nan_missing = nan_missing ? 1 : 0; a.two = two ? 1 : 0;
    a.A0 = A0; a.A1 = two ? A0 + plane_a : nullptr; a.Am = have_m ? A0 + (size_t)(np - 1) * plane_a : nullptr;
    a.ldk = (long)d.ldk; a.mean = g_ctx.i8_mean.as<double>();
    hipLaunchKernelGGL(pack_dosage_kernel, dim3((unsigned)((l + 3) / 4)), dim3(256), 0, s, a);
    HIPCHK(hipGetLastError());
    if (!g_ctx.i8_colsum_ready) {
      hipLaunchKernelGGL(u_digit_colsum_kernel, dim3((unsigned)((d.n + 3) / 4)), dim3(256), 0, s, g_ctx.i8_Bt.as<int8_t>(),
                         (long)d.ldk, (long)(d.npad * d.ldk), g_ctx.i8_qinv.as<double>(), (long)d.n, d.digits,
                         g_ctx.i8_colsum.as<double>());
      HIPCHK(hipGetLastError());
      g_ctx.i8_colsum_ready = true;
    }
  }
  {
    ProfScope ps(GEMMA_STAGE_UTX_GEMM, s);
    static bool attr_set = false;
    if (!attr_set) {
      HIPCHK(hipFuncSetAttribute(reinterpret_cast<const void *>(i8gemm_packed_kernel_t<false, true>),
                                 hipFuncAttributeMaxDynamicSharedMemorySize, 3 * I8P_STAGE));
      HIPCHK(hipFuncSetAttribute(reinterpret_cast<const void *>(i8gemm_dense16_kernel_t<true>),
                                 hipFuncAttributeMaxDynamicSharedMemorySize, 3 * I8P_STAGE));
      attr_set = true;
    }
    for (int a = 0; a < np; ++a) {
      I8PackArgs g;
      g.A = A0 + (size_t)a * plane_a;
      g.Bt = g_ctx.i8_Bt.as<int8_t>();
      g.C = g_ctx.i8_C.as<int>() + (size_t)a * d.digits * plane_c;
      g.ldk = (long)d.ldk; g.ldc = (long)d.npad;
      g.strideB = (long)(d.npad * d.ldk); g.strideC = (long)plane_c;
      g.m_row0 = 0;
      g.tiles_m = (int)(d.lpad / I8P_BM); g.tiles_n = (int)(d.npad / I8_BN);
      g.nk = (int)(d.ldk / I8_BK);
      g.gm = g_ctx.knobs.i8_gm;
      g.fuse = 0;
      g.digits = d.digits;
      if (g_ctx.knobs.dosage_rows == 32) {
        note_utx_kernel(GEMMA_UTX_KERNEL_DOSAGE_I8, d.digits, 0, 0);
        hipLaunchKernelGGL((i8gemm_packed_kernel_t<false, true>), dim3((unsigned)(g.tiles_m * g.tiles_n), (unsigned)d.digits),
                           dim3(512), 3 * I8P_STAGE, s, g);
      } else {
        note_utx_kernel(GEMMA_UTX_KERNEL_DOSAGE_I8_R16, d.digits, 0, 0);
        hipLaunchKernelGGL((i8gemm_dense16_kernel_t<true>), dim3((unsigned)(g.tiles_m * g.tiles_n), (unsigned)d.digits),
                           dim3(512), 3 * I8P_STAGE, s, g);
      }
      HIPCHK(hipGetLastError());
    }
  }
  {
    ProfScope ps(GEMMA_STAGE_UTX_POST, s);
    hipLaunchKernelGGL(i8_combine_dosage_kernel, dim3((unsigned)((d.n + 255) / 256), (unsigned)std::min<size_t>(l, 65535)),
                       dim3(256), 0, s, g_ctx.i8_C.as<int>(), (long)d.npad, (long)plane_c, g_ctx.i8_mean.as<double>(),
                       g_ctx.i8_qinv.as<double>(), g_ctx.i8_colsum.as<double>(), (long)l, (long)d.n, UtX, (long)ldx, d.digits,
                       two ? 1 : 0, have_m ? 1 : 0, two ? 1000.0 : 100.0);
    HIPCHK(hipGetLastError());
  }
  return GEMMA_HIP_OK;
}

static int utx_f64_try_i8(const double *src, size_t l, size_t ld, bool nan_missing, double *UtX, size_t ldx,
                          hipStream_t s, bool *done) {
  *done = false;
  I8Dims d;
  int rc = i8_begin(l, &d, s);
  if (rc) return rc;
  if (g_ctx.scratch.reserve(16)) return fail(GEMMA_HIP_ENOMEM, "lmm_batch: scratch");
  const int init[4] = {1, 1, 1, 0};
  HIPCHK(hipMemcpyAsync(g_ctx.scratch.p, init, sizeof init, hipMemcpyHostToDevice, s));
  {
    ProfScope ps(GEMMA_STAGE_INGEST, s);
    PackF64Args a;
    a.src = src; a.ld = (long)ld; a.l = (long)l; a.n = (int)d.n; a.nan_missing = nan_missing ? 1 : 0;
    a.A = g_ctx.i8_A.as<int8_t>(); a.ldk = (long)d.ldk; a.mean = g_ctx.i8_mean.as<double>();
    a.all_hard = g_ctx.scratch.as<int>();
    hipLaunchKernelGGL(pack_f64_kernel, dim3((unsigned)((l + 3) / 4)), dim3(256), 0, s, a);
    HIPCHK(hipGetLastError());
  }
  int verdict[4] = {0, 0, 0, 0};
  HIPCHK(hipMemcpyAsync(verdict, g_ctx.scratch.p, sizeof verdict, hipMemcpyDeviceToHost, s));
  HIPCHK(hipStreamSynchronize(s));
  if (verdict[0]) {
    *done = true;
    g_ctx.last_utx_path = 1;
    return i8_product(l, d, UtX, ldx, s);
  }
  if (verdict[1] && dosage_i8_enabled()) {
    *done = true;
    g_ctx.last_utx_path = verdict[2] ? 2 : 3;
    return utx_dosage_i8(src, l, ld, nan_missing, !verdict[2], verdict[3] != 0, d, UtX, ldx, s);
  }
  return GEMMA_HIP_OK;
}

static int gemm_U(const double **U, long *ld, hipStream_t s) {
  const size_t n = g_ctx.cfg.n;
  *U = g_ctx.U;
  *ld = (long)n;
  if ((n & 1) == 0) return GEMMA_HIP_OK;
  if (g_ctx.U_even_of != g_ctx.U) {
    if (g_ctx.U_even.reserve(n * (n + 1) * 8)) return fail(GEMMA_HIP_ENOMEM, "lmm_batch: even-ld copy of U");
    HIPCHK(hipMemcpy2DAsync(g_ctx.U_even.p, (n + 1) * 8, g_ctx.U, n * 8, n * 8, n, hipMemcpyDeviceToDevice, s));
    g_ctx.U_even_of = g_ctx.U;
  }
  *U = g_ctx.U_even.as<double>();
  *ld = (long)n + 1;
  return GEMMA_HIP_OK;
}
```

### gemma_amd/csrc/gemma_hip.hip

```cpp
#include <hip/hip_runtime.h>

#include <cmath>
#include <cstdarg>
#include <cstdio>
#include <cstdlib>
#include <cstring>
#include <string>
#include <vector>

#include "../../include/gemma_hip.h"
#include "tu_common.h"
#include "dgemm_mfma.hip.h"
#include "eigh_tu.h"
#include "vc_tu.h"
#include "prdt_tu.h"
#include "mqs_tu.h"
#include "cor_tu.h"
#include "ingest.hip.h"
#include "lm_assoc.hip.h"
#include "lmm_assoc.hip.h"
#include "lmm_grid.hip.h"
#include "i8gemm.hip.h"
#include "i8gemm_sparse.hip.h"
#include "i8gemm_sparse2.hip.h"
#include "i8gemm_sparse2_r16.hip.h"
#include "i8gemm_dense16.hip.h"
#include "qc.hip.h"
#include "mvlmm.hip.h"
#include "comm.hip.h"
#include "kin_i8.hip.h"

using namespace gemma_hip;

namespace {

struct StageProf {
  std::vector<std::pair<hipEvent_t, hipEvent_t>> ev;
  double acc_ms = 0.0;
  long launches = 0;
};

struct Knobs {
  int utx_i8 = 1;
  int i8_digits = 0;
  int i8_sparse = 2;
  int i8_fuse = 1;
  int i8_gm = 0;
  int i8_raster = S2_DEFAULT_RASTER;
  int i8_rows = 16;
  int i8_scale_max = 1;
  int i8_mdrop = 0;
  int i8_complete = 1;
  int i8_epilogue = 1;
  int dosage_i8 = 1;
  int dosage_rows = 16;
  int overlap = 0;
  int overlap_chunks = 4;
  int table_v2 = 1;
  int table_pf = 0;
  int force_generic = 0;
  int assoc_variant = 44;
  int mvlmm_rt = 0;
  int pipe_cus = 64;
  int kin_i8 = 1, kin_upper = 1, kin_lists = 1, kin_lists_oom = 0;
  long long kin_list_cap = 0;
  static int geti(const char *name, int dflt) {
    const char *e = getenv(name);
    return (e && *e) ? atoi(e) : dflt;
  }
  void load() {
    utx_i8 = geti("GEMMA_HIP_UTX_I8", 1);
    const int dg = geti("GEMMA_HIP_I8_DIGITS", 0);
    i8_digits = (dg == 6 || dg == 7) ? dg : 0;
    const char *es = getenv("GEMMA_HIP_I8_SPARSE");
    i8_sparse = (es && es[0] >= '0' && es[0] <= '2') ? es[0] - '0' : 2;
    const char *ef = getenv("GEMMA_HIP_I8_FUSE");
    i8_fuse = (ef && ef[0] == '0') ? 0 : 1;
    i8_gm = geti("GEMMA_HIP_I8_GM", 0);
    i8_raster = geti("GEMMA_HIP_I8_RASTER", S2_DEFAULT_RASTER);
    i8_rows = geti("GEMMA_HIP_I8_ROWS", 16) == 32 ? 32 : 16;
    const char *esc = getenv("GEMMA_HIP_I8_SCALE");
    i8_scale_max = (esc && strcmp(esc, "pow2") == 0) ? 0 : 1;
    const char *efm = getenv("GEMMA_HIP_I8_FORM");
    i8_mdrop = (efm && strcmp(efm, "7g6m") == 0) ? 1 : 0;
    if (i8_mdrop) i8_digits = 7;
    const char *ecp = getenv("GEMMA_HIP_I8_COMPLETE");
    i8_complete = (ecp && ecp[0] == '0') ? 0 : 1;
    const char *eep = getenv("GEMMA_HIP_I8_EPILOGUE");
    i8_epilogue = (eep && eep[0] == '0') ? 0 : 1;
    const char *ed = getenv("GEMMA_HIP_UTX_DOSAGE_I8");
    dosage_i8 = (ed && ed[0] == '0') ? 0 : 1;
    dosage_rows = geti("GEMMA_HIP_DOSAGE_ROWS", 16) == 32 ? 32 : 16;
    const char *eo = getenv("GEMMA_HIP_OVERLAP");
    overlap = (eo && eo[0] == '1') ? 1 : 0;
    overlap_chunks = geti("GEMMA_HIP_OVERLAP_CHUNKS", 4);
    const char *et = getenv("GEMMA_HIP_TABLE_V2");
    table_v2 = (et && et[0] == '0') ? 0 : 1;
    const char *ep = getenv("GEMMA_HIP_TABLE_PF");
    table_pf = (ep && ep[0] == '1') ? 1 : 0;
    const char *eg = getenv("GEMMA_HIP_FORCE_GENERIC");
    force_generic = (eg && eg[0] == '1') ? 1 : 0;
    assoc_variant = geti("GEMMA_HIP_ASSOC_VARIANT", 44);
    const char *er = getenv("GEMMA_HIP_MVLMM_RT");
    mvlmm_rt = (er && er[0] == '1') ? 1 : 0;
    pipe_cus = geti("GEMMA_HIP_PIPE_CUS", 64);
    const char *k1 = getenv("GEMMA_HIP_KIN_I8"), *k2 = getenv("GEMMA_HIP_KIN_UPPER"), *k3 = getenv("GEMMA_HIP_KIN_LISTS");
    const char *k4 = getenv("GEMMA_HIP_KIN_LISTS_OOM"), *k5 = getenv("GEMMA_HIP_KIN_LIST_CAP");
    kin_i8 = (k1 && k1[0] == '0') ? 0 : 1;
    kin_upper = (k2 && k2[0] == '0') ? 0 : 1;
    kin_lists = (k3 && k3[0] == '0') ? 0 : 1;
    kin_lists_oom = (k4 && k4[0] == '1') ? 1 : 0;
    kin_list_cap = (k5 && *k5) ? atoll(k5) : 0;
  }
};

struct Ctx {
  bool inited = false;
  Knobs knobs;
  int device = -1;
  int verbose = 0;
  std::string last_error;
  hipDeviceProp_t prop;
  bool profiling = false;
  StageProf prof[GEMMA_STAGE_COUNT];

  bool kin_active = false;
  size_t kin_n = 0;
  int kin_mode = 1;
  size_t kin_ns = 0;
  DevBuf kin_K, kin_X, kin_stage;
  hipStream_t kin_copy = nullptr;
  hipEvent_t kin_copied = nullptr, kin_ingested = nullptr;
  bool kin_ingested_valid = false, kin_host_call = false;
  DevBuf qc_G, qc_M, qc_W, qc_O;
  bool kin_i8 = false, kin_i8_used = false;
  DevBuf i8_meta, i8_rowsur;
  DevBuf U_even;
  const double *U_even_of = nullptr;
  DevBuf kin_GtG, kin_S, kin_a, kin_At, kin_Gt;
  DevBuf kin_A2, kin_cnt, kin_off, kin_listS, kin_listJ, kin_sub, kin_cj, kin_flag;
  DevBuf kin_tmap;
  hipStream_t ov_stream = nullptr;
  hipEvent_t ov_ready[16] = {}, ov_done = nullptr;
  struct XPipe {
    hipStream_t P = nullptr, Q = nullptr;
    hipEvent_t in_ready = nullptr, prod_done[2] = {}, post_done[2] = {};
    hipEvent_t ingest_done = nullptr;
    bool ingest_valid = false;
    bool post_valid[2] = {false, false};
    unsigned long long count = 0;
    bool pending = false;
    int cus = -1;
    DevBuf shadow_A, shadow_C, shadow_mean, shadow_rowsur;
  } xp;
  int kin_tmap_tm = 0, kin_tmap_tn = 0, kin_tmap_count = 0;

  bool lmm_active = false;
  gemma_lmm_cfg cfg;
  const double *U = nullptr, *eval = nullptr, *Uty = nullptr;
  DevBuf own_U, own_eval, own_Uty, own_UtW, UtWt, idx_map;
  size_t ni_total = 0;
  bool have_map = false;
  DevBuf X, UtX, stage_in, stage_out, carry;
  DevBuf grid_R, grid_F, grid_T;
  DevBuf cheb_R, cheb_F, cheb_T, cheb_slots, cheb_list, cheb_count, cheb_D, cheb_Ck, cheb_Gk, cheb_Lk, cheb_iv, cheb_dends, cheb_res;
  double cheb_mid[ASSOC_MAX_REGION], cheb_inv_half[ASSOC_MAX_REGION];
  GridGeom cheb_geom;
  DevBuf table_P;
  DevBuf gxe_env, gxe_UtWt, gxe_Z, gxe_UtZ, gxe_flip;
  bool gxe_ready = false;
  double gxe_lnbeta = 0.0;
  DevBuf mv_Yt, mv_out;
  DevBuf mv_scratch;
  bool mv_ready = false, mv_gxe = false;
  size_t mv_d = 0;
  MvArgs mv_proto;
  DevBuf i8_Bt, i8_q, i8_qinv, i8_cmax, i8_A, i8_C, i8_mean;
  unsigned long long cheb_qmask = 0;
  struct RasterSlot {
    DevBuf dev;
    std::vector<int2> host;
    int tm = 0, tn = 0, rb = 0, xcds = 8;
    unsigned long long used = 0;
  } i8_raster[6];
  unsigned long long i8_raster_clock = 0;
  DevBuf i8_surlist;
  DevBuf i8_colsum;
  bool i8_colsum_ready = false;
  int last_utx_path = 0;
  gemma_utx_kernel_info last_utx_kernel = {};
  int i8_last_epi = -1;
  long i8_rowsur_n = 0;
  long i8_flag_at = -1;
  bool i8_ready = false;
  size_t i8_ldk = 0, i8_npad = 0;
  int i8_digits = I8_DIGITS;
  GridGeom grid_geom;
  int carry_flip = 0;
  AssocArgs assoc_proto;

  bool lm_active = false;
  LmArgs lm_proto;
  DevBuf lm_Wt, lm_y, lm_small;

  DevBuf scratch;

  struct PipeSlot {
    void *pin_in = nullptr, *pin_out = nullptr;
    size_t pin_in_cap = 0, pin_out_cap = 0;
    DevBuf dev_in, dev_out;
    hipEvent_t h2d = nullptr, done = nullptr;
    size_t l = 0;
    bool busy = false;
  } pipe[2];
  hipStream_t pipe_copy = nullptr, pipe_comp = nullptr;
  int pipe_head = 0, pipe_count = 0;

  DevBuf kept_K, kept_UE;
  size_t kept_K_n = 0, kept_n = 0;
  double kept_trace = 0.0;
  Comm comm;
} g_ctx;

int fail(int code, const char *fmt, ...) {
  char buf[512];
  va_list ap;
  va_start(ap, fmt);
  vsnprintf(buf, sizeof buf, fmt, ap);
  va_end(ap);
  g_ctx.last_error = buf;
  if (g_ctx.verbose) fprintf(stderr, "gemma_hip: %s\n", buf);
  return code;
}

int ret(int rc, const std::string &msg) { return rc ? fail(rc, "%s", msg.c_str()) : GEMMA_HIP_OK; }

#define HIPCHK(expr)                                                                        \
  do {                                                                                      \
    hipError_t e_ = (expr);                                                                 \
    if (e_ != hipSuccess)                                                                   \
      return fail(GEMMA_HIP_ERUNTIME, "%s failed: %s (%s:%d)", #expr, hipGetErrorString(e_), \
                  __FILE__, __LINE__);                                                      \
  } while (0)

#define NEED_INIT()                                                                              \
  do {                                                                                           \
    if (!g_ctx.inited) {                                                                         \
      int rc_ = gemma_hip_init(-1, 0);                                                           \
      if (rc_ != GEMMA_HIP_OK) return rc_;                                                       \
    }                                                                                            \
  } while (0)

struct ProfScope {
  int stage;
  hipStream_t s;
  hipEvent_t a = nullptr, b = nullptr;
  ProfScope(int st, hipStream_t stream) : stage(st), s(stream) {
    if (g_ctx.profiling) {
      if (hipEventCreate(&a) == hipSuccess && hipEventCreate(&b) == hipSuccess)
        (void)hipEventRecord(a, s);
      else
        a = b = nullptr;
    }
  }
  ~ProfScope() {
    if (a && b) {
      (void)hipEventRecord(b, s);
      g_ctx.prof[stage].ev.emplace_back(a, b);
    }
  }
};

int prof_collect(int stage) {
  StageProf &p = g_ctx.prof[stage];
  for (auto &pr : p.ev) {
    (void)hipEventSynchronize(pr.second);
    float ms = 0.f;
    if (hipEventElapsedTime(&ms, pr.first, pr.second) == hipSuccess) {
      p.acc_ms += ms;
      p.launches += 1;
    }
    (void)hipEventDestroy(pr.first);
    (void)hipEventDestroy(pr.second);
  }
  p.ev.clear();
  return GEMMA_HIP_OK;
}

inline hipStream_t S(void *s) { return reinterpret_cast<hipStream_t>(s); }

}

static void pipe_release();
static void xp_release();
static int xp_flush_fwd(hipStream_t s);
static void raster_release() {
  for (auto &r : g_ctx.i8_raster) {
    r.dev.release();
    r.host.clear();
    r.tm = r.tn = r.rb = 0;
    r.used = 0;
  }
}
static void kin_i8_release();

extern "C" int gemma_hip_abi_version(void) { return GEMMA_HIP_ABI_VERSION; }

extern "C" const char *gemma_hip_strerror(int code) {
  switch (code) {
  case GEMMA_HIP_OK: return "ok";
  case GEMMA_HIP_EINVAL: return "invalid argument (range error)";
  case GEMMA_HIP_ENODEV: return "no usable gfx950 device";
  case GEMMA_HIP_ENOMEM: return "device memory allocation failed";
  case GEMMA_HIP_ERUNTIME: return "HIP runtime error";
  case GEMMA_HIP_ESTATE: return "call sequence violated";
  case GEMMA_HIP_ENOCONV: return "eigensolver did not converge";
  case GEMMA_HIP_ENOTPD: return "matrix not positive definite";
  default: return "unknown error";
  }
}

extern "C" const char *gemma_hip_last_error(void) { return g_ctx.last_error.c_str(); }

extern "C" int gemma_hip_init(int device, int verbose) {
  g_ctx.verbose = verbose;
  int ndev = 0;
  if (hipGetDeviceCount(&ndev) != hipSuccess || ndev <= 0) {
    (void)hipGetLastError();
    return fail(GEMMA_HIP_ENODEV, "no HIP device visible (this library has no CPU fallback)");
  }
  if (device >= 0) {
    if (device >= ndev) return fail(GEMMA_HIP_ENODEV, "device %d out of range (%d visible)", device, ndev);
    HIPCHK(hipSetDevice(device));
  }
  int cur = 0;
  HIPCHK(hipGetDevice(&cur));
  HIPCHK(hipGetDeviceProperties(&g_ctx.prop, cur));
  if (strncmp(g_ctx.prop.gcnArchName, "gfx950", 6) != 0)
    return fail(GEMMA_HIP_ENODEV, "device %d is %s; this build targets gfx950 only", cur,
                g_ctx.prop.gcnArchName);
  g_ctx.device = cur;
  g_ctx.inited = true;
  g_ctx.knobs.load();
  gemm_aux_init();
  if (verbose)
    fprintf(stderr, "gemma_hip: device %d %s (%s), %d CUs, %.1f GB\n", cur, g_ctx.prop.name,
            g_ctx.prop.gcnArchName, g_ctx.prop.multiProcessorCount,
            (double)g_ctx.prop.totalGlobalMem / 1e9);
  return GEMMA_HIP_OK;
}

extern "C" void gemma_hip_shutdown(void) {
  if (!g_ctx.inited) return;
  (void)hipDeviceSynchronize();
  for (int s = 0; s < GEMMA_STAGE_COUNT; ++s) prof_collect(s);
  g_ctx.kin_K.release(); g_ctx.kin_X.release(); g_ctx.kin_stage.release();
  g_ctx.qc_G.release(); g_ctx.qc_M.release(); g_ctx.qc_W.release(); g_ctx.qc_O.release();
  kin_i8_release();
  g_ctx.own_U.release(); g_ctx.own_eval.release(); g_ctx.own_Uty.release(); g_ctx.own_UtW.release();
  g_ctx.UtWt.release(); g_ctx.idx_map.release(); g_ctx.X.release(); g_ctx.UtX.release();
  g_ctx.stage_in.release(); g_ctx.stage_out.release(); g_ctx.carry.release(); g_ctx.scratch.release();
  g_ctx.i8_Bt.release(); g_ctx.i8_q.release(); g_ctx.i8_qinv.release(); g_ctx.i8_cmax.release(); g_ctx.i8_A.release(); g_ctx.i8_C.release();
  raster_release();
  g_ctx.mv_Yt.release(); g_ctx.mv_out.release(); g_ctx.mv_scratch.release();
  g_ctx.mv_ready = g_ctx.mv_gxe = false;
  g_ctx.i8_mean.release(); g_ctx.i8_meta.release(); g_ctx.i8_rowsur.release(); g_ctx.i8_colsum.release(); g_ctx.i8_surlist.release();
  g_ctx.i8_ready = g_ctx.i8_colsum_ready = false;
  g_ctx.table_P.release(); g_ctx.U_even.release();
  g_ctx.U_even_of = nullptr;
  pipe_release();
  xp_release();
  if (g_ctx.ov_stream) {
    (void)hipStreamDestroy(g_ctx.ov_stream);
    for (auto &e : g_ctx.ov_ready)
      if (e) (void)hipEventDestroy(e);
    if (g_ctx.ov_done) (void)hipEventDestroy(g_ctx.ov_done);
    g_ctx.ov_stream = nullptr;
    for (auto &e : g_ctx.ov_ready) e = nullptr;
    g_ctx.ov_done = nullptr;
  }
  if (g_ctx.kin_copy) {
    (void)hipStreamDestroy(g_ctx.kin_copy);
    if (g_ctx.kin_copied) (void)hipEventDestroy(g_ctx.kin_copied);
    if (g_ctx.kin_ingested) (void)hipEventDestroy(g_ctx.kin_ingested);
    g_ctx.kin_copy = nullptr;
    g_ctx.kin_copied = g_ctx.kin_ingested = nullptr;
    g_ctx.kin_ingested_valid = false;
  }
  g_ctx.kin_active = g_ctx.lmm_active = false;
  g_ctx.kept_K.release(); g_ctx.kept_UE.release();
  g_ctx.kept_K_n = g_ctx.kept_n = 0;
  g_ctx.comm.finalize();
  gemm_aux_destroy();
  eigh_tu_shutdown();
  vc_tu_shutdown();
  prdt_tu_shutdown();
  mqs_tu_shutdown();
  cor_tu_shutdown();
  g_ctx.inited = false;
}

extern "C" int gemma_hip_device_info(char *name, size_t len, int *n_cu, size_t *hbm_bytes) {
  NEED_INIT();
  if (name && len) {
    snprintf(name, len, "%s (%s)", g_ctx.prop.name, g_ctx.prop.gcnArchName);
  }
  if (n_cu) *n_cu = g_ctx.prop.multiProcessorCount;
  if (hbm_bytes) *hbm_bytes = g_ctx.prop.totalGlobalMem;
  return GEMMA_HIP_OK;
}

extern "C" int gemma_hip_profile_enable(int on) {
  g_ctx.profiling = (on != 0);
  return GEMMA_HIP_OK;
}

extern "C" int gemma_hip_profile_read(int stage, double *total_ms, long *launches, int reset) {
  NEED_INIT();
  if (stage < 0 || stage >= GEMMA_STAGE_COUNT) return fail(GEMMA_HIP_EINVAL, "bad stage %d", stage);
  prof_collect(stage);
  if (total_ms) *total_ms = g_ctx.prof[stage].acc_ms;
  if (launches) *launches = g_ctx.prof[stage].launches;
  if (reset) {
    g_ctx.prof[stage].acc_ms = 0.0;
    g_ctx.prof[stage].launches = 0;
  }
  return GEMMA_HIP_OK;
}

static int check_gemm(char ta, char tb, size_t M, size_t N, size_t K, size_t lda, size_t ldb,
                      size_t ldc) {
  const bool tA = (ta == 'T' || ta == 't'), tB = (tb == 'T' || tb == 't');
  if (!tA && ta != 'N' && ta != 'n') return fail(GEMMA_HIP_EINVAL, "dgemm: bad TransA '%c'", ta);
  if (!tB && tb != 'N' && tb != 'n') return fail(GEMMA_HIP_EINVAL, "dgemm: bad TransB '%c'", tb);
  const size_t a_cols = tA ? M : K, b_cols = tB ? K : N;
  if (lda < a_cols || ldb < b_cols || ldc < N)
    return fail(GEMMA_HIP_EINVAL, "Range error in dgemm (lda=%zu ldb=%zu ldc=%zu for M=%zu N=%zu K=%zu)",
                lda, ldb, ldc, M, N, K);
  return GEMMA_HIP_OK;
}

extern "C" int gemma_hip_dgemm_d(char ta, char tb, size_t M, size_t N, size_t K, double alpha,
                                 const double *A, size_t lda, const double *B, size_t ldb,
                                 double beta, double *C, size_t ldc, void *stream) {
  NEED_INIT();
  int rc = check_gemm(ta, tb, M, N, K, lda, ldb, ldc);
  if (rc) return rc;
  if (M == 0 || N == 0) return GEMMA_HIP_OK;
  ProfScope ps(GEMMA_STAGE_UTX_GEMM, S(stream));
  HIPCHK(launch_dgemm(ta, tb, (long)M, (long)N, (long)K, alpha, A, (long)lda, B, (long)ldb, beta, C,
                      (long)ldc, false, false, S(stream)));
  return GEMMA_HIP_OK;
}

extern "C" int gemma_hip_dgemm(char ta, char tb, size_t M, size_t N, size_t K, double alpha,
                               const double *A, size_t lda, const double *B, size_t ldb,
                               double beta, double *C, size_t ldc) {
  NEED_INIT();
  int rc = check_gemm(ta, tb, M, N, K, lda, ldb, ldc);
  if (rc) return rc;
  if (M == 0 || N == 0) return GEMMA_HIP_OK;
  const bool tA = (ta == 'T' || ta == 't'), tB = (tb == 'T' || tb == 't');
  const size_t a_rows = tA ? K : M, b_rows = tB ? N : K;
  const size_t a_bytes = a_rows * lda * 8, b_bytes = b_rows * ldb * 8, c_bytes = M * ldc * 8;
  DevBuf dA, dB, dC;
  if (dA.reserve(a_bytes ? a_bytes : 8) || dB.reserve(b_bytes ? b_bytes : 8) || dC.reserve(c_bytes)) {
    dA.release(); dB.release(); dC.release();
    return fail(GEMMA_HIP_ENOMEM, "dgemm: cannot allocate %zu bytes", a_bytes + b_bytes + c_bytes);
  }
  auto h2d = [&](void *d, const double *h, size_t rows, size_t cols, size_t ld) -> hipError_t {
    if (rows == 0 || cols == 0) return hipSuccess;
    return hipMemcpy2D(d, ld * 8, h, ld * 8, cols * 8, rows, hipMemcpyHostToDevice);
  };
  hipError_t e = h2d(dA.p, A, a_rows, tA ? M : K, lda);
  if (e == hipSuccess) e = h2d(dB.p, B, b_rows, tB ? K : N, ldb);
  if (e == hipSuccess && beta != 0.0) e = h2d(dC.p, C, M, N, ldc);
  if (e == hipSuccess)
    e = launch_dgemm(ta, tb, (long)M, (long)N, (long)K, alpha, dA.as<double>(), (long)lda,
                     dB.as<double>(), (long)ldb, beta, dC.as<double>(), (long)ldc, false, false, 0);
  if (e == hipSuccess) e = hipMemcpy2D(C, ldc * 8, dC.p, ldc * 8, N * 8, M, hipMemcpyDeviceToHost);
  dA.release(); dB.release(); dC.release();
  if (e != hipSuccess) return fail(GEMMA_HIP_ERUNTIME, "dgemm: %s", hipGetErrorString(e));
  return GEMMA_HIP_OK;
}

#include "abi_kinship.inc.h"
#include "abi_eigen_qc.inc.h"
#include "abi_lmm_stage.inc.h"
#include "abi_utx.inc.h"
#include "abi_lmm_batch.inc.h"
#include "abi_mvlmm.inc.h"
#include "abi_gxe_lm.inc.h"
#include "abi_kept_comm.inc.h"
#include "abi_vc.inc.h"
#include "abi_prdt.inc.h"
#include "abi_mqs.inc.h"
#include "abi_cor.inc.h"
```

### gemma_amd/csrc/i8gemm_sparse2.hip.h

```cpp
#pragma once
#include <algorithm>
#include <vector>
#include "i8gemm_sparse.hip.h"

namespace gemma_hip {

constexpr int S2_BM = 256, S2_BN = 128;
constexpr int S2_AMB = 16384;
constexpr int S2_STAGE = 32768;
constexpr int S2_NST = 4;
#ifndef S2_ADVANCE
#define S2_ADVANCE 1
#endif
#ifndef S2_LOOPDMA
#define S2_LOOPDMA 1
#endif

struct Sparse2Args {
  const uint4 *AM;
  const int8_t *Bt;
  int *C;
  long ldk, ldc, strideB, strideC, m_row0;
  int tiles_m, tiles_n, nk, gm, fuse, digits;
  int plane0 = 0;
  const int2 *tile_map = nullptr;
  const int *anymiss = nullptr;
  int run_if = 0;
  double *UtX = nullptr;
  long ldx = 0, l = 0, n = 0;
  const double *mean = nullptr, *qinv = nullptr;
  double m_scale = 1.0;
  int nplanes = 0;
};

__global__ __launch_bounds__(256) void sparse2_meta_kernel(const int8_t *__restrict__ A, long lpad, long ldk,
                                                           uint4 *__restrict__ AM, int *__restrict__ row_surplus,
                                                           int *anymiss = nullptr ) {
  const long nk = ldk / I8_BK;
  const long id = (long)blockIdx.x * 256 + threadIdx.x;
  if (id >= lpad * nk * 4) return;
  const int c = (int)(id & 3);
  const long rr = (id >> 2) & 255, tk = id >> 10;
  const long tmi = tk / nk, kt = tk - tmi * nk;
  const long row = tmi * S2_BM + rr;
  const int p = c >> 1, h = c & 1;
  const int8_t *base = A + row * ldk + kt * I8_BK;
  unsigned w[4];
#pragma unroll
  for (int e = 0; e < 2; ++e) {
    const int8_t *src = base + 32 * (2 * p + e) + 16 * h;
    unsigned g2 = 0;
#pragma unroll
    for (int i = 0; i < 4; ++i) g2 |= (*reinterpret_cast<const unsigned *>(src + 4 * i) & 0x03030303u) << (2 * i);
    w[e] = g2;
  }
  {
    const int8_t *src = base + 32 * (2 * p + h);
    unsigned idx = 0, bits = 0;
    int surplus = 0;
    for (int gq = 0; gq < 8; ++gq) {
      const unsigned word = *reinterpret_cast<const unsigned *>(src + 4 * gq);
      const unsigned m = (word >> 4) & 0x01010101u;
      const unsigned pat = (m | (m >> 7) | (m >> 14) | (m >> 21)) & 0xFu;
      const int cnt = __popc(pat);
      const int p0 = cnt >= 1 ? __ffs(pat) - 1 : 0;
      const unsigned rest = pat & (pat - 1);
      const int p1 = cnt >= 2 ? __ffs(rest) - 1 : (p0 == 3 ? 2 : 3);
      idx |= (unsigned)(p0 | (p1 << 2)) << (4 * gq);
      const int e0 = 2 * gq, e1 = 2 * gq + 1;
      bits |= (unsigned)(cnt >= 1) << (8 * (e0 & 3) + (e0 >> 2));
      bits |= (unsigned)(cnt >= 2) << (8 * (e1 & 3) + (e1 >> 2));
      surplus += cnt > 2 ? cnt - 2 : 0;
    }
    w[2] = idx;
    w[3] = bits;
    if (surplus) atomicAdd(row_surplus + row, surplus);
    if (anymiss && bits != 0 && *reinterpret_cast<volatile int *>(anymiss) == 0) *reinterpret_cast<volatile int *>(anymiss) = 1;
  }
  AM[id] = make_uint4(w[0], w[1], w[2], w[3]);
}

__device__ __forceinline__ i32x4 s2_unpack_g(int w) {
  i32x4 v;
  const unsigned u = (unsigned)w;
#pragma unroll
  for (int i = 0; i < 4; ++i) v[i] = (int)((u >> (2 * i)) & 0x03030303u);
  return v;
}
__device__ __forceinline__ i32x4 s2_expand(int bits) {
  i32x4 v;
  const unsigned u = (unsigned)bits;
#pragma unroll
  for (int i = 0; i < 4; ++i) v[i] = (int)((u >> i) & 0x01010101u);
  return v;
}

static inline void s2_build_raster(int tiles_m, int tiles_n, int rb, std::vector<int2> &map, int PR = 8) {
  const int NX = 8, PC = 32 / PR;
  if (rb != 1 && rb != 2 && rb != 4 && rb != 8) rb = 2;
  const int cbs = NX / rb;
  std::vector<std::vector<int2>> seq(NX);
  for (int band0 = 0, band = 0; band0 < tiles_m; band0 += rb * PR, ++band)
    for (int col0 = 0; col0 < tiles_n; col0 += cbs * PC)
      for (int xx = 0; xx < NX; ++xx) {
        const int x = (xx + band) % NX;
        const int r0 = band0 + (xx % rb) * PR, c0 = col0 + (xx / rb) * PC;
        const int nr = std::min(PR, std::min(tiles_m, band0 + rb * PR) - r0), nc = std::min(PC, std::min(tiles_n, col0 + cbs * PC) - c0);
        if (nr <= 0 || nc <= 0) continue;
        for (int c = 0; c < nc; ++c)
          for (int r = 0; r < nr; ++r) seq[x].push_back(make_int2(r0 + r, c0 + c));
      }
  const int total = tiles_m * tiles_n;
  std::vector<int> want(NX);
  for (int x = 0; x < NX; ++x) want[x] = total / NX + (x < total % NX ? 1 : 0);
  std::vector<int2> spare;
  for (int x = 0; x < NX; ++x)
    while ((int)seq[x].size() > want[x]) {
      spare.push_back(seq[x].back());
      seq[x].pop_back();
    }
  for (int x = 0; x < NX; ++x)
    while ((int)seq[x].size() < want[x]) {
      seq[x].push_back(spare.back());
      spare.pop_back();
    }
  map.assign((size_t)total, make_int2(0, 0));
  for (int x = 0; x < NX; ++x)
    for (int o = 0; o < want[x]; ++o) map[(size_t)o * NX + x] = seq[x][o];
}

template <int NI>
__global__ __launch_bounds__(512, 2) void i8gemm_sparse2_kernel_t(Sparse2Args g) {
  constexpr int NJ = 4 / NI;
  extern __shared__ __attribute__((aligned(1024))) int8_t i8lds[];
  int tm, tn;
  if (g.tile_map) {
    const int2 t2 = g.tile_map[blockIdx.x];
    tm = __builtin_amdgcn_readfirstlane(t2.x);
    tn = __builtin_amdgcn_readfirstlane(t2.y);
  } else {
    const int nwg = gridDim.x, b = blockIdx.x;
    const int q = nwg >> 3, r = nwg & 7, x = b & 7, o = b >> 3;
    const int L = (x < r ? x * (q + 1) : r * (q + 1) + (x - r) * q) + o;
    const int GM = g.gm > 0 ? g.gm : 8;
    const int per_group = GM * g.tiles_n;
    const int grp = L / per_group;
    const int first_m = grp * GM;
    const int gsz = min(g.tiles_m - first_m, GM);
    const int in = L - grp * per_group;
    tm = first_m + in % gsz;
    tn = in / gsz;
  }
  const int plane = blockIdx.y;
  const int odd = g.digits & 1;
  const int d_first = g.fuse ? (odd ? (plane == 0 ? 0 : 2 * plane) : 2 * plane + 1) : plane;
  const int nd = (g.fuse && !(odd && plane == 0)) ? 2 : 1;
  const int t = threadIdx.x, lane = t & 63;
  const int wave = __builtin_amdgcn_readfirstlane(t >> 6);
  const int wm = NI == 2 ? wave >> 1 : wave, wn = NI == 2 ? wave & 1 : 0;
  const int r32 = lane & 31, h = lane >> 5;

  const uint4 *asrc[2];
  const int8_t *bsrc[2];
  int adst[2], bdst[2];
#define S2_INIT_SRC(DIGIT)                                                                                        \
  do {                                                                                                            \
    _Pragma("unroll") for (int j = 0; j < 2; ++j) {                                                               \
      const int qp = 2 * wave + j;                                                                                \
      const int row = 16 * qp + (lane >> 2);                                                                      \
      asrc[j] = g.AM + ((long)tm * g.nk * S2_BM + row) * 4 + ((lane & 3) ^ ((row >> 2) & 3));                     \
      adst[j] = qp * 1024;                                                                                        \
      const int col = 8 * qp + (lane >> 3);                                                                       \
      bsrc[j] = g.Bt + (long)(DIGIT) * g.strideB + ((long)tn * S2_BN + col) * g.ldk + 16 * ((lane & 7) ^ ((col >> 1) & 7)); \
      bdst[j] = S2_AMB + qp * 1024;                                                                               \
    }                                                                                                             \
  } while (0)
  int amo[2], fb[4];
  {
    const int row = wm * 32 * NI + r32;
#pragma unroll
    for (int p = 0; p < 2; ++p) amo[p] = row * 64 + (((2 * p + h) ^ ((row >> 2) & 3)) << 4);
    const int col = wn * 32 * NJ + r32;
#pragma unroll
    for (int ks = 0; ks < 4; ++ks) fb[ks] = S2_AMB + col * 128 + (((2 * ks + h) ^ ((col >> 1) & 7)) << 4);
  }

  i32x16 accg[NI][NJ], accm[NI][NJ];
#pragma unroll
  for (int i = 0; i < NI; ++i)
#pragma unroll
    for (int j = 0; j < NJ; ++j)
#pragma unroll
      for (int r = 0; r < 16; ++r) { accg[i][j][r] = 0; accm[i][j][r] = 0; }

  i32x4 am[2][NI];
  i32x4 ga[2][NI];
  i32x4 bb[2][NJ];
  i32x4 ms[NI];

#define S2_DMA_A(j, SOFF)                                                                                         \
  do {                                                                                                            \
    __builtin_amdgcn_global_load_lds((gemma_gptr_t)asrc[j], (gemma_lptr_t)(i8lds + (SOFF) + adst[j]), 16, 0, 0);  \
    if (S2_ADVANCE) asrc[j] += S2_BM * 4;                                                                         \
  } while (0)
#define S2_DMA_B(j, SOFF)                                                                                         \
  do {                                                                                                            \
    __builtin_amdgcn_global_load_lds((gemma_gptr_t)bsrc[j], (gemma_lptr_t)(i8lds + (SOFF) + bdst[j]), 16, 0, 0);  \
    if (S2_ADVANCE) bsrc[j] += I8_BK;                                                                             \
  } while (0)
#define S2_RAM(SOFF, P, i) am[(P)&1][i] = *reinterpret_cast<const i32x4 *>(i8lds + (SOFF) + amo[(P)&1] + (i) * 2048)
#define S2_RB(SOFF, KS, j) bb[(KS)&1][j] = *reinterpret_cast<const i32x4 *>(i8lds + (SOFF) + fb[KS] + (j) * 4096)
#define S2_UNP(KS, i) ga[(KS)&1][i] = s2_unpack_g(am[((KS) >> 1) & 1][i][(KS)&1])
#define S2_EXP(P, i) ms[i] = s2_expand(am[(P)&1][i][3])
#define S2_G(KS, i, j)                                                                                            \
  asm volatile("s_nop 1\n\tv_mfma_i32_32x32x32_i8 %0, %1, %2, %0"                                                 \
               : "+v"(accg[i][j]) : "v"(ga[(KS)&1][i]), "v"(bb[(KS)&1][j]))
#define S2_S(P, i, j)                                                                                             \
  do {                                                                                                            \
    const i32x8 bp_ = __builtin_shufflevector(bb[0][j], bb[1][j], 0, 1, 2, 3, 4, 5, 6, 7);                         \
    asm volatile("s_nop 1\n\tv_smfmac_i32_32x32x64_i8 %0, %1, %2, %3"                                             \
                 : "+v"(accm[i][j]) : "v"(ms[i]), "v"(bp_), "v"(am[(P)&1][i][2]));                                 \
  } while (0)
#define S2_KTILE(SC, SN, SD, MORE, LOAD3, VMW)                                                                    \
  do {                                                                                                            \
         \
    S2_G(0, 0, 0); S2_RB(SC, 1, 0); GEMMA_SB();                                                                   \
    S2_G(0, 0, 1); S2_RB(SC, 1, 1); S2_EXP(0, 0); GEMMA_SB();                                                     \
    S2_G(0, 1, 0); if ((LOAD3) && S2_LOOPDMA) S2_DMA_A(0, SD); GEMMA_SB();                                                        \
    S2_G(0, 1, 1); S2_EXP(0, 1); GEMMA_SB();                                                                      \
         \
    S2_S(0, 0, 0); S2_RAM(SC, 1, 0); GEMMA_SB();                                                                  \
    S2_S(0, 0, 1); S2_RAM(SC, 1, 1); S2_UNP(1, 0); GEMMA_SB();                                                    \
    S2_S(0, 1, 0); if ((LOAD3) && S2_LOOPDMA) S2_DMA_A(1, SD); GEMMA_SB();                                                        \
    S2_S(0, 1, 1); S2_UNP(1, 1); GEMMA_SB();                                                                      \
        \
    S2_G(1, 0, 0); S2_UNP(2, 0); GEMMA_SB(); S2_RB(SC, 2, 0); GEMMA_SB();                                         \
    S2_G(1, 0, 1); S2_RB(SC, 2, 1); GEMMA_SB();                                                                   \
    S2_G(1, 1, 0); S2_UNP(2, 1); if ((LOAD3) && S2_LOOPDMA) S2_DMA_B(0, SD); GEMMA_SB();                                          \
    S2_G(1, 1, 1); if ((LOAD3) && S2_LOOPDMA) S2_DMA_B(1, SD); GEMMA_SB();                                                        \
     \
                                                     \
    S2_G(2, 0, 0); S2_RB(SC, 3, 0); GEMMA_SB();                                                                   \
    S2_G(2, 0, 1); S2_RB(SC, 3, 1); GEMMA_SB();                                                                   \
    asm volatile("s_waitcnt vmcnt(" #VMW ")" ::: "memory");                                                       \
    __builtin_amdgcn_s_barrier();                                                                                 \
    GEMMA_SB();                                                                                                   \
    S2_G(2, 1, 0); S2_EXP(1, 0); GEMMA_SB();                                                                      \
    S2_G(2, 1, 1); S2_EXP(1, 1); GEMMA_SB();                                                                      \
     \
    S2_S(1, 0, 0); if (MORE) S2_RAM(SN, 0, 0); GEMMA_SB();                                                        \
    S2_S(1, 0, 1); if (MORE) S2_RAM(SN, 0, 1); GEMMA_SB();                                                        \
    S2_S(1, 1, 0); S2_UNP(3, 0); GEMMA_SB();                                                                      \
    S2_S(1, 1, 1); S2_UNP(3, 1); GEMMA_SB();                                                                      \
     \
    S2_G(3, 0, 0); if (MORE) S2_UNP(0, 0); GEMMA_SB();                                                            \
    if (MORE) { S2_RB(SN, 0, 0); S2_RB(SN, 0, 1); } GEMMA_SB();                                                   \
    S2_G(3, 0, 1); if (MORE) S2_UNP(0, 1); GEMMA_SB();                                                            \
    S2_G(3, 1, 0); GEMMA_SB();                                                                                    \
    S2_G(3, 1, 1); GEMMA_SB();                                                                                    \
  } while (0)

#define S2_KTILE_81(SC, SN, SD, MORE, LOAD3, VMW)                                                                 \
  do {                                                                                                            \
    S2_G(0, 0, 0); S2_RB(SC, 1, 0); S2_RB(SC, 1, 1); GEMMA_SB();                                                  \
    S2_G(0, 0, 1); S2_RB(SC, 1, 2); S2_RB(SC, 1, 3); GEMMA_SB();                                                  \
    S2_G(0, 0, 2); S2_EXP(0, 0); if ((LOAD3) && S2_LOOPDMA) S2_DMA_A(0, SD); GEMMA_SB();                          \
    S2_G(0, 0, 3); GEMMA_SB();                                                                                    \
    S2_S(0, 0, 0); S2_RAM(SC, 1, 0); GEMMA_SB();                                                                  \
    S2_S(0, 0, 1); S2_UNP(1, 0); GEMMA_SB();                                                                      \
    S2_S(0, 0, 2); if ((LOAD3) && S2_LOOPDMA) S2_DMA_A(1, SD); GEMMA_SB();                                        \
    S2_S(0, 0, 3); GEMMA_SB();                                                                                    \
    S2_G(1, 0, 0); S2_UNP(2, 0); GEMMA_SB(); S2_RB(SC, 2, 0); S2_RB(SC, 2, 1); GEMMA_SB();                        \
    S2_G(1, 0, 1); S2_RB(SC, 2, 2); S2_RB(SC, 2, 3); GEMMA_SB();                                                  \
    S2_G(1, 0, 2); if ((LOAD3) && S2_LOOPDMA) S2_DMA_B(0, SD); GEMMA_SB();                                        \
    S2_G(1, 0, 3); if ((LOAD3) && S2_LOOPDMA) S2_DMA_B(1, SD); GEMMA_SB();                                        \
    S2_G(2, 0, 0); S2_RB(SC, 3, 0); S2_RB(SC, 3, 1); GEMMA_SB();                                                  \
    S2_G(2, 0, 1); S2_RB(SC, 3, 2); S2_RB(SC, 3, 3); GEMMA_SB();                                                  \
    asm volatile("s_waitcnt vmcnt(" #VMW ")" ::: "memory");                                                       \
    __builtin_amdgcn_s_barrier();                                                                                 \
    GEMMA_SB();                                                                                                   \
    S2_G(2, 0, 2); S2_EXP(1, 0); GEMMA_SB();                                                                      \
    S2_G(2, 0, 3); GEMMA_SB();                                                                                    \
    S2_S(1, 0, 0); if (MORE) S2_RAM(SN, 0, 0); GEMMA_SB();                                                        \
    S2_S(1, 0, 1); S2_UNP(3, 0); GEMMA_SB();                                                                      \
    S2_S(1, 0, 2); GEMMA_SB();                                                                                    \
    S2_S(1, 0, 3); GEMMA_SB();                                                                                    \
    S2_G(3, 0, 0); if (MORE) S2_UNP(0, 0); GEMMA_SB();                                                            \
    if (MORE) { S2_RB(SN, 0, 0); S2_RB(SN, 0, 1); } GEMMA_SB();                                                   \
    S2_G(3, 0, 1); if (MORE) { S2_RB(SN, 0, 2); S2_RB(SN, 0, 3); } GEMMA_SB();                                    \
    S2_G(3, 0, 2); GEMMA_SB();                                                                                    \
    S2_G(3, 0, 3); GEMMA_SB();                                                                                    \
  } while (0)
#define S2_TILE(SC, SN, SD, MORE, LOAD3, VMW)                                                                     \
  do {                                                                                                            \
    if constexpr (NI == 2) S2_KTILE(SC, SN, SD, MORE, LOAD3, VMW);                                                \
    else S2_KTILE_81(SC, SN, SD, MORE, LOAD3, VMW);                                                               \
  } while (0)
  if (wave >= 4) __builtin_amdgcn_s_setprio(1);
  const int nk = g.nk;
  for (int dd = 0; dd < nd; ++dd) {
    if (dd > 0) {
      asm volatile("s_nop 15\n\ts_nop 7" ::: "memory");
#pragma unroll
      for (int i = 0; i < NI; ++i)
#pragma unroll
        for (int j = 0; j < NJ; ++j)
#pragma unroll
          for (int r = 0; r < 16; ++r) { accg[i][j][r] <<= 8; accm[i][j][r] <<= 8; }
    }
    S2_INIT_SRC(d_first - dd);
#pragma unroll
    for (int j = 0; j < 2; ++j) { S2_DMA_A(j, 0); S2_DMA_B(j, 0); }
    if (nk > 1) {
#pragma unroll
      for (int j = 0; j < 2; ++j) { S2_DMA_A(j, S2_STAGE); S2_DMA_B(j, S2_STAGE); }
    }
    if (nk > 2) {
#pragma unroll
      for (int j = 0; j < 2; ++j) { S2_DMA_A(j, 2 * S2_STAGE); S2_DMA_B(j, 2 * S2_STAGE); }
      asm volatile("s_waitcnt vmcnt(8)" ::: "memory");
    } else if (nk > 1) {
      asm volatile("s_waitcnt vmcnt(4)" ::: "memory");
    } else {
      asm volatile("s_waitcnt vmcnt(0)" ::: "memory");
    }
    __builtin_amdgcn_s_barrier();
    GEMMA_SB();
#pragma unroll
    for (int i = 0; i < NI; ++i) S2_RAM(0, 0, i);
#pragma unroll
    for (int j = 0; j < NJ; ++j) S2_RB(0, 0, j);
#pragma unroll
    for (int i = 0; i < NI; ++i) S2_UNP(0, i);
    GEMMA_SB();

    int sc = 0, sn = S2_STAGE, s2 = 2 * S2_STAGE, sd = 3 * S2_STAGE;
    int kt = 0;
    for (; kt + 3 < nk; ++kt) {
      S2_TILE(sc, sn, sd, true, true, 8);
      const int tmp = sc; sc = sn; sn = s2; s2 = sd; sd = tmp;
    }
    if (nk >= 3) {
      S2_TILE(sc, sn, sd, true, false, 4);
      const int tmp = sc; sc = sn; sn = s2; s2 = sd; sd = tmp;
    }
    if (nk >= 2) {
      S2_TILE(sc, sn, sd, true, false, 0);
      const int tmp = sc; sc = sn; sn = s2; s2 = sd; sd = tmp;
    }
    S2_TILE(sc, sn, sd, false, false, 0);
  }
#undef S2_INIT_SRC
#undef S2_DMA_A
#undef S2_DMA_B
#undef S2_RAM
#undef S2_RB
#undef S2_UNP
#undef S2_EXP
#undef S2_G
#undef S2_S
#undef S2_KTILE
#undef S2_KTILE_81
#undef S2_TILE

  asm volatile("s_nop 15\n\ts_nop 7" ::: "memory");
  int *Cg = g.C + (long)plane * g.strideC;
#pragma unroll
  for (int i = 0; i < NI; ++i)
#pragma unroll
    for (int j = 0; j < NJ; ++j) {
      const long col = (long)tn * S2_BN + wn * 32 * NJ + j * 32 + r32;
#pragma unroll
      for (int r = 0; r < 16; ++r) {
        const long row = (long)tm * S2_BM + wm * 32 * NI + i * 32 + (r & 3) + 8 * (r >> 2) + 4 * h;
        Cg[row * g.ldc + col] = accg[i][j][r];
        Cg[(g.m_row0 + row) * g.ldc + col] = accm[i][j][r];
      }
    }
}

#ifndef S2_DEFAULT_RASTER
#define S2_DEFAULT_RASTER 1
#endif
#ifndef S2_DEFAULT_NI
#define S2_DEFAULT_NI 1
#endif
static constexpr auto i8gemm_sparse2_kernel = i8gemm_sparse2_kernel_t<S2_DEFAULT_NI>;

}
```

### gemma_amd/csrc/i8gemm_sparse2_r16.hip.h

```cpp
#pragma once
#include "i8gemm_sparse2.hip.h"

#ifndef S2_R16_PREP_SPREAD
#define S2_R16_PREP_SPREAD 0
#endif
#ifndef S2_R16_NST
#define S2_R16_NST 4
#endif
#ifndef S2_R16_ABL_NO_S
#define S2_R16_ABL_NO_S 0
#endif
#ifndef S2_R16_ABL_NO_D
#define S2_R16_ABL_NO_D 0
#endif

namespace gemma_hip {

constexpr int S2_R16_LDS = S2_R16_NST * S2_STAGE;

template <bool WITH_S, bool COMBINE = false>
__device__ __forceinline__ void s2_r16_body(const Sparse2Args &g) {
  extern __shared__ __attribute__((aligned(1024))) int8_t i8lds[];
  constexpr bool NO_S = !WITH_S || S2_R16_ABL_NO_S;
  if (g.run_if) {
    const int any = __builtin_amdgcn_readfirstlane(*g.anymiss);
    if ((g.run_if == 1) != (any != 0)) return;
  }
  int tm, tn;
  if (g.tile_map) {
    const int2 t2 = g.tile_map[blockIdx.x];
    tm = __builtin_amdgcn_readfirstlane(t2.x);
    tn = __builtin_amdgcn_readfirstlane(t2.y);
  } else {
    const int nwg = gridDim.x, b = blockIdx.x;
    const int q_ = nwg >> 3, r = nwg & 7, x = b & 7, o = b >> 3;
    const int L = (x < r ? x * (q_ + 1) : r * (q_ + 1) + (x - r) * q_) + o;
    const int GM = g.gm > 0 ? g.gm : 8;
    const int per_group = GM * g.tiles_n;
    const int grp = L / per_group;
    const int first_m = grp * GM;
    const int gsz = min(g.tiles_m - first_m, GM);
    const int in = L - grp * per_group;
    tm = first_m + in % gsz;
    tn = in / gsz;
  }
  const int plane = blockIdx.y + g.plane0;
  const int odd = g.digits & 1;
  const int d_first = g.fuse ? (odd ? (plane == 0 ? 0 : 2 * plane) : 2 * plane + 1) : plane;
  const int nd = (g.fuse && !(odd && plane == 0)) ? 2 : 1;
  const int t = threadIdx.x, lane = t & 63;
  const int wave = __builtin_amdgcn_readfirstlane(t >> 6);
  const int r16 = lane & 15, q = lane >> 4;

  const uint4 *asrc[2];
  const int8_t *bsrc[2];
  int adst[2], bdst[2];
#define GS_INIT_SRC(DIGIT)                                                                                        \
  do {                                                                                                            \
    _Pragma("unroll") for (int j = 0; j < 2; ++j) {                                                               \
      const int qp = 2 * wave + j;                                                                                \
      const int row = 16 * qp + (lane >> 2);                                                                      \
      asrc[j] = g.AM + ((long)tm * g.nk * S2_BM + row) * 4 + ((lane & 3) ^ ((row >> 2) & 3));                     \
      adst[j] = qp * 1024;                                                                                        \
      const int col = 8 * qp + (lane >> 3);                                                                       \
      bsrc[j] = g.Bt + (long)(DIGIT) * g.strideB + ((long)tn * S2_BN + col) * g.ldk + 16 * ((lane & 7) ^ ((col >> 1) & 7)); \
      bdst[j] = S2_AMB + qp * 1024;                                                                               \
    }                                                                                                             \
  } while (0)
  int ro[2], fo[2];
  {
    const int row = wave * 32 + r16;
#pragma unroll
    for (int p = 0; p < 2; ++p) {
      ro[p] = row * 64 + (((2 * p + (q & 1)) ^ ((row >> 2) & 3)) << 4);
      fo[p] = S2_AMB + r16 * 128 + (((4 * p + q) ^ ((r16 >> 1) & 7)) << 4);
    }
  }

  i32x4 accg[2][8], accm[2][8];
#pragma unroll
  for (int i = 0; i < 2; ++i)
#pragma unroll
    for (int j = 0; j < 8; ++j) { accg[i][j] = (i32x4){0, 0, 0, 0}; accm[i][j] = (i32x4){0, 0, 0, 0}; }

  i32x4 rec[2][2];
  i32x4 ga[2][2];
  i32x4 ms[2];
  int ix[2];
  i32x8 T[4];

#define GS_DMA_A(j, SOFF)                                                                                         \
  do {                                                                                                            \
    __builtin_amdgcn_global_load_lds((gemma_gptr_t)asrc[j], (gemma_lptr_t)(i8lds + (SOFF) + adst[j]), 16, 0, 0);  \
    asrc[j] += S2_BM * 4;                                                                                         \
  } while (0)
#define GS_DMA_B(j, SOFF)                                                                                         \
  do {                                                                                                            \
    __builtin_amdgcn_global_load_lds((gemma_gptr_t)bsrc[j], (gemma_lptr_t)(i8lds + (SOFF) + bdst[j]), 16, 0, 0);  \
    bsrc[j] += I8_BK;                                                                                             \
  } while (0)
#define GS_RREC(SOFF, i, P) rec[i][P] = *reinterpret_cast<const i32x4 *>(i8lds + (SOFF) + ro[P] + (i) * 1024)
#define GS_RT(SOFF, SB, SL)                                                                                       \
  do {                                                                                                            \
    const i32x4 x_ = *reinterpret_cast<const i32x4 *>(i8lds + (SOFF) + fo[0] + (SB) * 2048);                      \
    const i32x4 y_ = *reinterpret_cast<const i32x4 *>(i8lds + (SOFF) + fo[1] + (SB) * 2048);                      \
    T[SL] = __builtin_shufflevector(x_, y_, 0, 1, 2, 3, 4, 5, 6, 7);                                              \
  } while (0)
#define GS_PREP(i)                                                                                                \
  do {                                                                                                            \
    ga[i][0] = s2_unpack_g((q >> 1) ? rec[i][0][1] : rec[i][0][0]);                                               \
    ga[i][1] = s2_unpack_g((q >> 1) ? rec[i][1][1] : rec[i][1][0]);                                               \
    ix[i] = (q >> 1) ? rec[i][1][2] : rec[i][0][2];                                                               \
    ms[i] = s2_expand((q >> 1) ? rec[i][1][3] : rec[i][0][3]);                                                    \
    asm volatile("" ::"v"(rec[i][0]), "v"(rec[i][1]));                                                            \
  } while (0)
#define GS_PREP_G(i, P) ga[i][P] = s2_unpack_g((q >> 1) ? rec[i][P][1] : rec[i][P][0])
#define GS_PREP_M(i)                                                                                              \
  do {                                                                                                            \
    ix[i] = (q >> 1) ? rec[i][1][2] : rec[i][0][2];                                                               \
    ms[i] = s2_expand((q >> 1) ? rec[i][1][3] : rec[i][0][3]);                                                    \
    asm volatile("" ::"v"(rec[i][0]), "v"(rec[i][1]));                                                            \
  } while (0)
#define GS_D(i, SB, P, SL)                                                                                        \
  do {                                                                                                            \
    if (!S2_R16_ABL_NO_D)                                                                                         \
      asm volatile("s_nop 1\n\tv_mfma_i32_16x16x64_i8 %0, %1, %2, %0"                                             \
                   : "+v"(accg[i][SB])                                                                            \
                   : "v"(ga[i][P]), "v"(__builtin_shufflevector(T[SL], T[SL], 4 * (P), 4 * (P) + 1, 4 * (P) + 2, 4 * (P) + 3))); \
  } while (0)
#define GS_S(i, SB, SL)                                                                                           \
  do {                                                                                                            \
    if (!NO_S)                                                                                                    \
      asm volatile("s_nop 1\n\tv_smfmac_i32_16x16x128_i8 %0, %1, %2, %3" : "+v"(accm[i][SB]) : "v"(ms[i]), "v"(T[SL]), "v"(ix[i])); \
  } while (0)
#define GS_STEP(SB, SL, X)                                                                                        \
  do {                                                                                                            \
    GS_D(0, SB, 0, SL); GEMMA_SB();                                                                               \
    GS_D(1, SB, 0, SL); X; GEMMA_SB();                                                                            \
    GS_D(0, SB, 1, SL); GEMMA_SB();                                                                               \
    GS_D(1, SB, 1, SL); GEMMA_SB();                                                                               \
    GS_S(0, SB, SL); GEMMA_SB();                                                                                  \
    GS_S(1, SB, SL); GEMMA_SB();                                                                                  \
  } while (0)
#define GS_KTILE(SC, SN, SD, MORE, LOAD3, VMW)                                                                    \
  do {                                                                                                            \
    GS_STEP(0, 0, { GS_RT(SC, 3, 3); if (LOAD3) GS_DMA_A(0, SD); });                                               \
    GS_STEP(1, 1, { GS_RT(SC, 4, 0); if (LOAD3) GS_DMA_A(1, SD); });                                               \
    GS_STEP(2, 2, { GS_RT(SC, 5, 1); if (LOAD3) GS_DMA_B(0, SD); });                                               \
    GS_STEP(3, 3, { GS_RT(SC, 6, 2); if (LOAD3) GS_DMA_B(1, SD); });                                               \
    GS_STEP(4, 0, { GS_RT(SC, 7, 3); });                                                                           \
    asm volatile("s_waitcnt vmcnt(" #VMW ")" ::: "memory");                                                       \
    __builtin_amdgcn_s_barrier();                                                                                 \
    GEMMA_SB();                                                                                                   \
    GS_STEP(5, 1, { if (MORE) { GS_RREC(SN, 0, 0); GS_RREC(SN, 0, 1); GS_RREC(SN, 1, 0); GS_RREC(SN, 1, 1);       \
                                GS_RT(SN, 0, 0); } });                                                             \
    GS_STEP(6, 2, { if (MORE) { GS_RT(SN, 1, 1); } });                                                             \
    if (S2_R16_PREP_SPREAD && (MORE)) {                                                                           \
      GS_D(0, 7, 0, 3); GEMMA_SB();                                                                               \
      GS_D(1, 7, 0, 3); { GS_RT(SN, 2, 2); GS_PREP_G(0, 0); } GEMMA_SB();                                          \
      GS_D(0, 7, 1, 3); { GS_PREP_G(1, 0); } GEMMA_SB();                                                           \
      GS_D(1, 7, 1, 3); { GS_PREP_G(0, 1); } GEMMA_SB();                                                           \
      GS_S(0, 7, 3); { GS_PREP_G(1, 1); } GEMMA_SB();                                                              \
      GS_S(1, 7, 3); { GS_PREP_M(0); } GEMMA_SB();                                                                 \
      { GS_PREP_M(1); } GEMMA_SB();                                                                                \
    } else {                                                                                                      \
      GS_STEP(7, 3, { if (MORE) { GS_RT(SN, 2, 2); } });                                                           \
      if (MORE) { GS_PREP(0); GS_PREP(1); }                                                                       \
      GEMMA_SB();                                                                                                 \
    }                                                                                                             \
  } while (0)

  if (wave >= 4) __builtin_amdgcn_s_setprio(1);
  const int nk = g.nk;
  for (int dd = 0; dd < nd; ++dd) {
    if (dd > 0) {
      asm volatile("s_nop 15\n\ts_nop 7" ::: "memory");
#pragma unroll
      for (int i = 0; i < 2; ++i)
#pragma unroll
        for (int j = 0; j < 8; ++j)
#pragma unroll
          for (int r = 0; r < 4; ++r) {
            accg[i][j][r] <<= 8;
            if (WITH_S) accm[i][j][r] <<= 8;
          }
    }
    GS_INIT_SRC(d_first - dd);
#pragma unroll
    for (int j = 0; j < 2; ++j) { GS_DMA_A(j, 0); GS_DMA_B(j, 0); }
    if (nk > 1) {
#pragma unroll
      for (int j = 0; j < 2; ++j) { GS_DMA_A(j, S2_STAGE); GS_DMA_B(j, S2_STAGE); }
    }
    if (nk > 2) {
#pragma unroll
      for (int j = 0; j < 2; ++j) { GS_DMA_A(j, 2 * S2_STAGE); GS_DMA_B(j, 2 * S2_STAGE); }
    }
    if (S2_R16_NST == 5 && nk > 3) {
#pragma unroll
      for (int j = 0; j < 2; ++j) { GS_DMA_A(j, 3 * S2_STAGE); GS_DMA_B(j, 3 * S2_STAGE); }
      asm volatile("s_waitcnt vmcnt(12)" ::: "memory");
    } else if (nk > 2) {
      asm volatile("s_waitcnt vmcnt(8)" ::: "memory");
    } else if (nk > 1) {
      asm volatile("s_waitcnt vmcnt(4)" ::: "memory");
    } else {
      asm volatile("s_waitcnt vmcnt(0)" ::: "memory");
    }
    __builtin_amdgcn_s_barrier();
    GEMMA_SB();
    GS_RT(0, 0, 0);
    GS_RT(0, 1, 1);
    GS_RT(0, 2, 2);
    GS_RREC(0, 0, 0); GS_RREC(0, 0, 1); GS_RREC(0, 1, 0); GS_RREC(0, 1, 1);
    GS_PREP(0);
    GS_PREP(1);
    GEMMA_SB();

    int sc = 0, sn = S2_STAGE, s2 = 2 * S2_STAGE, s3 = 3 * S2_STAGE, sd = (S2_R16_NST - 1) * S2_STAGE;
#define GS_ROTATE()                                                                                               \
  do {                                                                                                            \
    const int tmp = sc;                                                                                           \
    sc = sn; sn = s2;                                                                                             \
    if (S2_R16_NST == 5) { s2 = s3; s3 = sd; } else { s2 = sd; }                                                  \
    sd = tmp;                                                                                                     \
  } while (0)
    int kt = 0;
    if (S2_R16_NST == 5) {
      for (; kt + 4 < nk; ++kt) {
        GS_KTILE(sc, sn, sd, true, true, 12);
        GS_ROTATE();
      }
      if (nk >= 4) {
        GS_KTILE(sc, sn, sd, true, false, 8);
        GS_ROTATE();
      }
    } else {
      for (; kt + 3 < nk; ++kt) {
        GS_KTILE(sc, sn, sd, true, true, 8);
        GS_ROTATE();
      }
    }
    if (nk >= 3) {
      GS_KTILE(sc, sn, sd, true, false, 4);
      GS_ROTATE();
    }
    if (nk >= 2) {
      GS_KTILE(sc, sn, sd, true, false, 0);
      GS_ROTATE();
    }
    GS_KTILE(sc, sn, sd, false, false, 0);
#undef GS_ROTATE
  }

  asm volatile("s_nop 15\n\ts_nop 7" ::: "memory");
  if constexpr (COMBINE) {
    const int np = g.nplanes;
    const bool load_m = !(g.anymiss && __builtin_amdgcn_readfirstlane(*g.anymiss) == 0);
    const double w_hi = g.fuse ? 65536.0 : 256.0;
    const double w0 = (g.fuse && !odd) ? 65536.0 : 256.0;
    const long row_w = (long)tm * S2_BM + wave * 32, col_w = (long)tn * S2_BN;
    const long row_l = row_w + 4 * q, col_l = col_w + r16;
    const unsigned lo_c = (unsigned)((4 * q * g.ldc + r16) * 4), lo_x = (unsigned)((4 * q * g.ldx + r16) * 8);
#define EP_AT(T, BASE, LO) (*(T *)((const char *)(BASE) + (LO)))
#define EP_LOAD(DG, DM, I, H, P)                                                                                  \
  do {                                                                                                            \
    const int *cp_ = g.C + (long)(P) * g.strideC + (row_w + 16 * (I)) * g.ldc + col_w + 32 * (H);                 \
    _Pragma("unroll") for (int k_ = 0; k_ < 2; ++k_) _Pragma("unroll") for (int r_ = 0; r_ < 4; ++r_) {           \
      DG[4 * k_ + r_] = EP_AT(const int, cp_ + r_ * g.ldc + 16 * k_, lo_c);                                       \
      DM[4 * k_ + r_] = load_m ? EP_AT(const int, cp_ + (g.m_row0 + r_) * g.ldc + 16 * k_, lo_c) : 0;             \
    }                                                                                                             \
  } while (0)
    int cg[8], cm[8];
#pragma unroll
    for (int e = 0; e < 8; ++e) cg[e] = cm[e] = 0;
    if (np > 1) EP_LOAD(cg, cm, 0, 0, np - 1);
#pragma unroll
    for (int b = 0; b < 8; ++b) {
      const int i = b >> 2, h = b & 3;
      double tg[8], tk[8];
#pragma unroll
      for (int e = 0; e < 8; ++e) tg[e] = tk[e] = 0.0;
      for (int p = np - 1; p >= 1; --p) {
        int ng[8], nm[8];
#pragma unroll
        for (int e = 0; e < 8; ++e) ng[e] = nm[e] = 0;
        if (p > 1) EP_LOAD(ng, nm, i, h, p - 1);
        else if (b < 7) EP_LOAD(ng, nm, (b + 1) >> 2, (b + 1) & 3, np - 1);
#pragma unroll
        for (int e = 0; e < 8; ++e) {
          tg[e] = tg[e] * w_hi + (double)cg[e];
          tk[e] = tk[e] * w_hi + (double)cm[e];
          cg[e] = ng[e];
          cm[e] = nm[e];
        }
      }
#pragma unroll
      for (int r = 0; r < 4; ++r) {
        const bool row_in = row_l + 16 * i + r < g.l;
        const double ms = row_in ? EP_AT(const double, g.mean + row_w + 16 * i + r, (unsigned)(32 * q)) * g.m_scale : 0.0;
#pragma unroll
        for (int k = 0; k < 2; ++k) {
          const int e = 4 * k + r, sb = 2 * h + k;
          const int m0 = WITH_S ? accm[i][sb][r] : 0;
          tg[e] = tg[e] * w0 + (double)accg[i][sb][r];
          tk[e] = tk[e] * w0 + (double)m0;
          if (row_in && col_l + 16 * sb < g.n)
            EP_AT(double, g.UtX + (row_w + 16 * i + r) * g.ldx + col_w + 16 * sb, lo_x) =
                fma(ms, tk[e], tg[e]) * EP_AT(const double, g.qinv + col_w + 16 * sb, (unsigned)(8 * r16));
        }
      }
    }
#undef EP_AT
#undef EP_LOAD
  } else {
    int *Cg = g.C + (long)plane * g.strideC;
#pragma unroll
    for (int i = 0; i < 2; ++i)
#pragma unroll
      for (int sb = 0; sb < 8; ++sb) {
        const long col = (long)tn * S2_BN + 16 * sb + r16;
#pragma unroll
        for (int r = 0; r < 4; ++r) {
          const long row = (long)tm * S2_BM + wave * 32 + 16 * i + 4 * q + r;
          Cg[row * g.ldc + col] = accg[i][sb][r];
          if (WITH_S) Cg[(g.m_row0 + row) * g.ldc + col] = accm[i][sb][r];
        }
      }
  }
#undef GS_INIT_SRC
#undef GS_DMA_A
#undef GS_DMA_B
#undef GS_RREC
#undef GS_RT
#undef GS_PREP
#undef GS_PREP_G
#undef GS_PREP_M
#undef GS_D
#undef GS_S
#undef GS_STEP
#undef GS_KTILE
}

__global__ __launch_bounds__(512, 2) void i8gemm_sparse2_r16_kernel(Sparse2Args g) { s2_r16_body<true>(g); }
__global__ __launch_bounds__(512, 2) void i8gemm_sparse2_r16_g_kernel(Sparse2Args g) { s2_r16_body<false>(g); }
__global__ __launch_bounds__(512, 2) void i8gemm_sparse2_r16_ep_kernel(Sparse2Args g) { s2_r16_body<true, true>(g); }
__global__ __launch_bounds__(512, 2) void i8gemm_sparse2_r16_ep_g_kernel(Sparse2Args g) { s2_r16_body<false, true>(g); }

}
```

Baseline: 360,900.

## Rotate K start per workgroup, park epilogue accumulators in LDS, cache pad memset

Adds time-based K-loop rotation, on by default. Each workgroup starts its k-tile walk at an offset derived from a wall-clock tick and a per-tile period, measured with events on earlier launches, so concurrent workgroups spread their HBM reads instead of hitting the same addresses. The DMA addressing moves to a base-plus-offset scheme that wraps around nk. The fused combine epilogue is factored out and can park half the accumulators in LDS to cut register pressure while it streams the partial planes. The tail-padding memset of the int8 A buffer now clears only the padded rows and is skipped when the buffer layout is unchanged. This adds event overhead and timing-dependent behaviour, and risks stale pad state if the buffer is reused elsewhere.

```diff
diff --git a/gemma_amd/build.py b/gemma_amd/build.py
--- a/gemma_amd/build.py
+++ b/gemma_amd/build.py
@@ -6,7 +6,7 @@
 CSRC = os.path.join(HERE, "csrc")
 LIB = os.path.join(HERE, "libgemma_hip.so")
 UNITS = {
-    "gemma_hip.hip": ["dgemm_mfma.hip.h", "lmm_grid.hip.h", "i8gemm.hip.h", "i8gemm_sparse.hip.h", "i8gemm_sparse2.hip.h", "i8gemm_sparse2_r16.hip.h", "i8gemm_dense16.hip.h", "lmm_assoc.hip.h",
+    "gemma_hip.hip": ["dgemm_mfma.hip.h", "lmm_grid.hip.h", "i8gemm.hip.h", "i8gemm_sparse.hip.h", "i8gemm_sparse2.hip.h", "i8gemm_sparse2_r16.hip.h", "i8_krot.h", "i8gemm_dense16.hip.h", "lmm_assoc.hip.h",
                       "lmm_search.hip.h", "comm.hip.h", "comm_shm.hpp", "kin_i8.hip.h", "ingest.hip.h", "qc.hip.h", "lm_assoc.hip.h", "mvlmm.hip.h",
                       "mvlmm_kernels.hip.h", "eigh_tu.h", "tu_common.h",
                       "abi_kinship.inc.h", "abi_eigen_qc.inc.h", "abi_lmm_stage.inc.h", "abi_utx.inc.h", "abi_lmm_batch.inc.h",
diff --git a/gemma_amd/csrc/abi_gxe_lm.inc.h b/gemma_amd/csrc/abi_gxe_lm.inc.h
--- a/gemma_amd/csrc/abi_gxe_lm.inc.h
+++ b/gemma_amd/csrc/abi_gxe_lm.inc.h
@@ -355,6 +355,7 @@
   g_ctx.cheb_list.release(); g_ctx.cheb_count.release(); g_ctx.cheb_D.release(); g_ctx.cheb_Ck.release();
   g_ctx.cheb_Gk.release(); g_ctx.cheb_Lk.release(); g_ctx.cheb_iv.release(); g_ctx.cheb_dends.release(); g_ctx.cheb_res.release();
   g_ctx.i8_Bt.release(); g_ctx.i8_q.release(); g_ctx.i8_qinv.release(); g_ctx.i8_cmax.release(); g_ctx.i8_A.release(); g_ctx.i8_C.release();
+  g_ctx.i8_pad_zero.p = nullptr;
   raster_release();
   g_ctx.i8_mean.release(); g_ctx.i8_meta.release(); g_ctx.i8_rowsur.release(); g_ctx.i8_colsum.release(); g_ctx.i8_surlist.release();
   g_ctx.i8_ready = false;
diff --git a/gemma_amd/csrc/abi_kinship.inc.h b/gemma_amd/csrc/abi_kinship.inc.h
--- a/gemma_amd/csrc/abi_kinship.inc.h
+++ b/gemma_amd/csrc/abi_kinship.inc.h
@@ -63,6 +63,7 @@
     HIPCHK(hipMemsetAsync(g_ctx.kin_a.p, 0, (n + 1) * 8, s));
     g_ctx.kin_i8_used = true;
   }
+  g_ctx.i8_pad_zero.p = nullptr;
   if (g_ctx.i8_A.reserve(l * ldk) || g_ctx.i8_mean.reserve(l * 8) || g_ctx.kin_At.reserve(rows_t * ldl) ||
       g_ctx.kin_Gt.reserve(rows_t * ldl) || g_ctx.i8_C.reserve(rows_a * rows_b * 4))
     return fail(GEMMA_HIP_ENOMEM, "kin_add: integer-path buffers");
diff --git a/gemma_amd/csrc/abi_lmm_batch.inc.h b/gemma_amd/csrc/abi_lmm_batch.inc.h
--- a/gemma_amd/csrc/abi_lmm_batch.inc.h
+++ b/gemma_amd/csrc/abi_lmm_batch.inc.h
@@ -18,6 +18,7 @@
   x.count = 0;
   x.pending = false;
   x.cus = -1;
+  g_ctx.i8_pad_zero.p = nullptr;
   x.shadow_A.release(); x.shadow_C.release(); x.shadow_mean.release(); x.shadow_rowsur.release();
 }
 static int xp_init() {
diff --git a/gemma_amd/csrc/abi_utx.inc.h b/gemma_amd/csrc/abi_utx.inc.h
--- a/gemma_amd/csrc/abi_utx.inc.h
+++ b/gemma_amd/csrc/abi_utx.inc.h
@@ -22,7 +22,14 @@
   const size_t c_elems = (size_t)(d->nplanes - d->epi) * d->mrows * d->npad;
   if (g_ctx.i8_A.reserve(d->lpad * d->ldk) || g_ctx.i8_C.reserve(c_elems * 4) || g_ctx.i8_mean.reserve(l * 8))
     return fail(GEMMA_HIP_ENOMEM, "lmm_batch: int8 product buffers (%zu bytes)", d->lpad * d->ldk + c_elems * 4);
-  if (d->lpad != l) HIPCHK(hipMemsetAsync(g_ctx.i8_A.p, 0, d->lpad * d->ldk, s));
+  if (d->lpad != l) {
+    Ctx::PadZero &z = g_ctx.i8_pad_zero;
+    if (!(z.p == g_ctx.i8_A.p && z.cap == g_ctx.i8_A.cap && z.s == s && z.l == l && z.lpad == d->lpad && z.ldk == d->ldk)) {
+      z.p = nullptr;
+      HIPCHK(hipMemsetAsync(g_ctx.i8_A.as<int8_t>() + l * d->ldk, 0, (d->lpad - l) * d->ldk, s));
+      z.p = g_ctx.i8_A.p; z.cap = g_ctx.i8_A.cap; z.s = s; z.l = l; z.lpad = d->lpad; z.ldk = d->ldk;
+    }
+  }
   return GEMMA_HIP_OK;
 }
 
@@ -68,6 +75,47 @@
   lru->used = ++g_ctx.i8_raster_clock;
   *map_d = lru->dev.as<int2>();
   return GEMMA_HIP_OK;
+}
+
+static Ctx::KrotSlot *krot_slot(int tm, int tn, int nk, int planes, int tiles, int kind) {
+  Ctx::KrotSlot *lru = &g_ctx.i8_krot[0];
+  for (auto &k : g_ctx.i8_krot) {
+    if (k.kind == kind && k.tm == tm && k.tn == tn && k.nk == nk && k.planes == planes && k.tiles == tiles) {
+      k.used = ++g_ctx.i8_raster_clock;
+      return &k;
+    }
+    if (k.used < lru->used) lru = &k;
+  }
+  if (!lru->e0 && (hipEventCreate(&lru->e0) != hipSuccess || hipEventCreate(&lru->e1) != hipSuccess)) {
+    (void)hipGetLastError();
+    if (lru->e0) (void)hipEventDestroy(lru->e0);
+    lru->e0 = lru->e1 = nullptr;
+    return nullptr;
+  }
+  lru->tm = tm; lru->tn = tn; lru->nk = nk; lru->planes = planes; lru->tiles = tiles; lru->kind = kind;
+  lru->pending = false;
+  lru->period_fp8 = 0;
+  lru->used = ++g_ctx.i8_raster_clock;
+  return lru;
+}
+static void krot_poll(Ctx::KrotSlot *k) {
+  if (!k->pending) return;
+  const hipError_t q = hipEventQuery(k->e1);
+  if (q == hipErrorNotReady) { (void)hipGetLastError(); return; }
+  k->pending = false;
+  float ms = 0.f;
+  if (q != hipSuccess || hipEventElapsedTime(&ms, k->e0, k->e1) != hipSuccess) { (void)hipGetLastError(); return; }
+  if (g_ctx.wall_clock_khz == 0.0) {
+    int khz = 0;
+    if (hipDeviceGetAttribute(&khz, hipDeviceAttributeWallClockRate, g_ctx.device) != hipSuccess || khz <= 0) {
+      (void)hipGetLastError();
+      khz = 100000;
+    }
+    g_ctx.wall_clock_khz = (double)khz;
+  }
+  const long cus = std::max(1, g_ctx.prop.multiProcessorCount);
+  const long rounds = ((long)k->tm * k->tn * k->planes + cus - 1) / cus;
+  k->period_fp8 = s2_krot_period_fp8((double)ms, g_ctx.wall_clock_khz, rounds, k->tiles);
 }
 
 static int i8_gemm_rows(const I8Dims &d, size_t row0, size_t rows_pad, hipStream_t s, double *UtX = nullptr, size_t ldx = 0,
@@ -131,6 +179,23 @@
     }
     note_utx_kernel(g_ctx.knobs.i8_rows == 32 ? GEMMA_UTX_KERNEL_RECORDS_R32 : GEMMA_UTX_KERNEL_RECORDS_R16, d.digits, d.fuse,
                     raster_rb);
+    auto timed = [&](int kind, int planes, int nd_sum, auto &&launch) {
+      Ctx::KrotSlot *ks = nullptr;
+      g2.period_fp8 = 0; g2.krot_fix = -1;
+      if (g_ctx.knobs.i8_krot == 2) {
+        g2.krot_fix = g_ctx.knobs.i8_krot_fix;
+      } else if (g_ctx.knobs.i8_krot == 1 && planes > 0) {
+        ks = krot_slot(g2.tiles_m, g2.tiles_n, g2.nk, planes, (g2.nk * nd_sum + planes / 2) / planes, kind);
+        if (ks) {
+          krot_poll(ks);
+          g2.period_fp8 = ks->period_fp8;
+        }
+      }
+      const bool rec = ks && !ks->pending && hipEventRecord(ks->e0, s) == hipSuccess;
+      launch();
+      if (rec) ks->pending = hipEventRecord(ks->e1, s) == hipSuccess;
+    };
+    const int nd_hi = d.fuse ? 2 : 1, nd_0 = (d.fuse && !(d.digits & 1)) ? 2 : 1;
     if (g_ctx.knobs.i8_rows == 32) {
       hipLaunchKernelGGL(i8gemm_sparse2_kernel, dim3((unsigned)(g2.tiles_m * g2.tiles_n), (unsigned)d.nplanes), dim3(512),
                          S2_NST * S2_STAGE, s, g2);
@@ -138,40 +203,50 @@
       const unsigned wgs = (unsigned)(g2.tiles_m * g2.tiles_n);
       g2.anymiss = i8_anymiss(d);
       g2.plane0 = 1;
-      g2.run_if = g2.anymiss ? 1 : 0;
-      hipLaunchKernelGGL(i8gemm_sparse2_r16_kernel, dim3(wgs, (unsigned)d.nplanes - 1u), dim3(512), S2_R16_LDS, s, g2);
-      if (g2.anymiss) {
-        g2.run_if = 2;
-        hipLaunchKernelGGL(i8gemm_sparse2_r16_g_kernel, dim3(wgs, (unsigned)d.nplanes - 1u), dim3(512), S2_R16_LDS, s, g2);
-      }
+      timed(0, d.nplanes - 1, nd_hi * (d.nplanes - 1), [&] {
+        g2.run_if = g2.anymiss ? 1 : 0;
+        hipLaunchKernelGGL(i8gemm_sparse2_r16_kernel, dim3(wgs, (unsigned)d.nplanes - 1u), dim3(512), S2_R16_LDS, s, g2);
+        if (g2.anymiss) {
+          g2.run_if = 2;
+          hipLaunchKernelGGL(i8gemm_sparse2_r16_g_kernel, dim3(wgs, (unsigned)d.nplanes - 1u), dim3(512), S2_R16_LDS, s, g2);
+        }
+      });
       g2.plane0 = 0;
       g2.UtX = UtX + row0 * ldx; g2.ldx = (long)ldx; g2.l = (long)rows; g2.n = (long)d.n;
       g2.mean = g_ctx.i8_mean.as<double>() + row0; g2.qinv = g_ctx.i8_qinv.as<double>();
       g2.m_scale = 1.0; g2.nplanes = d.nplanes;
-      if (d.mdrop) {
-        g2.run_if = 0;
-        hipLaunchKernelGGL(i8gemm_sparse2_r16_ep_g_kernel, dim3(wgs, 1u), dim3(512), S2_R16_LDS, s, g2);
-      } else {
-        g2.run_if = g2.anymiss ? 1 : 0;
-        hipLaunchKernelGGL(i8gemm_sparse2_r16_ep_kernel, dim3(wgs, 1u), dim3(512), S2_R16_LDS, s, g2);
-        if (g2.anymiss) {
-          g2.run_if = 2;
+      g2.epi_park = g_ctx.knobs.i8_epi_park;
+      timed(1, 1, nd_0, [&] {
+        if (d.mdrop) {
+          g2.run_if = 0;
           hipLaunchKernelGGL(i8gemm_sparse2_r16_ep_g_kernel, dim3(wgs, 1u), dim3(512), S2_R16_LDS, s, g2);
+        } else {
+          g2.run_if = g2.anymiss ? 1 : 0;
+          hipLaunchKernelGGL(i8gemm_sparse2_r16_ep_kernel, dim3(wgs, 1u), dim3(512), S2_R16_LDS, s, g2);
+          if (g2.anymiss) {
+            g2.run_if = 2;
+            hipLaunchKernelGGL(i8gemm_sparse2_r16_ep_g_kernel, dim3(wgs, 1u), dim3(512), S2_R16_LDS, s, g2);
+          }
         }
-      }
+      });
     } else {
       const unsigned wgs = (unsigned)(g2.tiles_m * g2.tiles_n), first = d.mdrop ? 1u : 0u;
       g2.anymiss = i8_anymiss(d);
       g2.plane0 = (int)first;
-      g2.run_if = g2.anymiss ? 1 : 0;
-      hipLaunchKernelGGL(i8gemm_sparse2_r16_kernel, dim3(wgs, (unsigned)d.nplanes - first), dim3(512), S2_R16_LDS, s, g2);
-      if (g2.anymiss) {
-        g2.run_if = 2;
-        hipLaunchKernelGGL(i8gemm_sparse2_r16_g_kernel, dim3(wgs, (unsigned)d.nplanes - first), dim3(512), S2_R16_LDS, s, g2);
-      }
+      const int planes_hi = d.nplanes - (int)first;
+      timed(2, planes_hi, d.mdrop ? nd_hi * planes_hi : nd_hi * (d.nplanes - 1) + nd_0, [&] {
+        g2.run_if = g2.anymiss ? 1 : 0;
+        hipLaunchKernelGGL(i8gemm_sparse2_r16_kernel, dim3(wgs, (unsigned)d.nplanes - first), dim3(512), S2_R16_LDS, s, g2);
+        if (g2.anymiss) {
+          g2.run_if = 2;
+          hipLaunchKernelGGL(i8gemm_sparse2_r16_g_kernel, dim3(wgs, (unsigned)d.nplanes - first), dim3(512), S2_R16_LDS, s, g2);
+        }
+      });
       if (d.mdrop) {
         g2.plane0 = 0; g2.run_if = 0;
-        hipLaunchKernelGGL(i8gemm_sparse2_r16_g_kernel, dim3(wgs, 1u), dim3(512), S2_R16_LDS, s, g2);
+        timed(3, 1, nd_0, [&] {
+          hipLaunchKernelGGL(i8gemm_sparse2_r16_g_kernel, dim3(wgs, 1u), dim3(512), S2_R16_LDS, s, g2);
+        });
       }
     }
   } else if (sparse) {
@@ -263,6 +338,7 @@
       g_ctx.i8_colsum.reserve(d.n * 8))
     return fail(GEMMA_HIP_ENOMEM, "lmm_batch: dosage planes (%zu bytes)", (size_t)np * (plane_a + d.digits * plane_c * 4));
   int8_t *A0 = g_ctx.i8_A.as<int8_t>();
+  g_ctx.i8_pad_zero.p = nullptr;
   {
     ProfScope ps(GEMMA_STAGE_INGEST, s);
     if (d.lpad != l) HIPCHK(hipMemsetAsync(A0, 0, (size_t)np * plane_a, s));
diff --git a/gemma_amd/csrc/gemma_hip.hip b/gemma_amd/csrc/gemma_hip.hip
--- a/gemma_amd/csrc/gemma_hip.hip
+++ b/gemma_amd/csrc/gemma_hip.hip
@@ -47,6 +47,8 @@
   int i8_fuse = 1;
   int i8_gm = 0;
   int i8_raster = S2_DEFAULT_RASTER;
+  int i8_krot = 1, i8_krot_fix = 0;
+  int i8_epi_park = 1;
   int i8_rows = 16;
   int i8_scale_max = 1;
   int i8_mdrop = 0;
@@ -78,6 +80,12 @@
     i8_fuse = (ef && ef[0] == '0') ? 0 : 1;
     i8_gm = geti("GEMMA_HIP_I8_GM", 0);
     i8_raster = geti("GEMMA_HIP_I8_RASTER", S2_DEFAULT_RASTER);
+    const char *ekr = getenv("GEMMA_HIP_I8_KROT");
+    i8_krot = 1; i8_krot_fix = 0;
+    if (ekr && strncmp(ekr, "fix:", 4) == 0) { i8_krot = 2; i8_krot_fix = atoi(ekr + 4) & 0x7fffffff; }
+    else if (ekr && ekr[0] == '0') i8_krot = 0;
+    const char *epk = getenv("GEMMA_HIP_I8_EPI_PARK");
+    i8_epi_park = (epk && epk[0] == '0') ? 0 : 1;
     i8_rows = geti("GEMMA_HIP_I8_ROWS", 16) == 32 ? 32 : 16;
     const char *esc = getenv("GEMMA_HIP_I8_SCALE");
     i8_scale_max = (esc && strcmp(esc, "pow2") == 0) ? 0 : 1;
@@ -184,6 +192,19 @@
     unsigned long long used = 0;
   } i8_raster[6];
   unsigned long long i8_raster_clock = 0;
+  struct KrotSlot {
+    int tm = 0, tn = 0, nk = 0, planes = 0, tiles = 0, kind = -1;
+    hipEvent_t e0 = nullptr, e1 = nullptr;
+    bool pending = false;
+    unsigned period_fp8 = 0;
+    unsigned long long used = 0;
+  } i8_krot[8];
+  double wall_clock_khz = 0.0;
+  struct PadZero {
+    const void *p = nullptr;
+    size_t cap = 0, l = 0, lpad = 0, ldk = 0;
+    hipStream_t s = nullptr;
+  } i8_pad_zero;
   DevBuf i8_surlist;
   DevBuf i8_colsum;
   bool i8_colsum_ready = false;
@@ -301,6 +322,11 @@
     r.tm = r.tn = r.rb = 0;
     r.used = 0;
   }
+  for (auto &k : g_ctx.i8_krot) {
+    if (k.e0) (void)hipEventDestroy(k.e0);
+    if (k.e1) (void)hipEventDestroy(k.e1);
+    k = Ctx::KrotSlot();
+  }
 }
 static void kin_i8_release();
 
@@ -361,6 +387,7 @@
   g_ctx.UtWt.release(); g_ctx.idx_map.release(); g_ctx.X.release(); g_ctx.UtX.release();
   g_ctx.stage_in.release(); g_ctx.stage_out.release(); g_ctx.carry.release(); g_ctx.scratch.release();
   g_ctx.i8_Bt.release(); g_ctx.i8_q.release(); g_ctx.i8_qinv.release(); g_ctx.i8_cmax.release(); g_ctx.i8_A.release(); g_ctx.i8_C.release();
+  g_ctx.i8_pad_zero.p = nullptr;
   raster_release();
   g_ctx.mv_Yt.release(); g_ctx.mv_out.release(); g_ctx.mv_scratch.release();
   g_ctx.mv_ready = g_ctx.mv_gxe = false;
diff --git a/gemma_amd/csrc/i8_krot.h b/gemma_amd/csrc/i8_krot.h
--- /dev/null
+++ b/gemma_amd/csrc/i8_krot.h
@@ -0,0 +1,24 @@
+#pragma once
+
+#if defined(__HIPCC__) || defined(__CUDACC__)
+#define S2_KROT_HD __host__ __device__
+#else
+#define S2_KROT_HD
+#endif
+
+S2_KROT_HD inline int s2_krot_k0(unsigned long long ticks, unsigned period_fp8, int nk) {
+  if (period_fp8 == 0 || nk <= 1) return 0;
+  return (int)(((ticks << 8) / period_fp8) % (unsigned long long)nk);
+}
+
+S2_KROT_HD inline int s2_krot_fix(int k, int nk) { return nk <= 1 ? 0 : (int)((unsigned)k % (unsigned)nk); }
+
+S2_KROT_HD inline int s2_krot_next(int kt, int nk) { return kt + 1 >= nk ? 0 : kt + 1; }
+
+inline unsigned s2_krot_period_fp8(double ms, double clock_khz, long rounds, long tiles) {
+  if (!(ms > 0.0) || !(clock_khz > 0.0) || rounds <= 0 || tiles <= 0) return 0u;
+  const double p = ms * clock_khz * 256.0 / ((double)rounds * (double)tiles);
+  if (!(p >= 1.0)) return 1u;
+  if (p >= 4294967295.0) return 4294967295u;
+  return (unsigned)(p + 0.5);
+}
diff --git a/gemma_amd/csrc/i8gemm_sparse2.hip.h b/gemma_amd/csrc/i8gemm_sparse2.hip.h
--- a/gemma_amd/csrc/i8gemm_sparse2.hip.h
+++ b/gemma_amd/csrc/i8gemm_sparse2.hip.h
@@ -31,6 +31,9 @@
   const double *mean = nullptr, *qinv = nullptr;
   double m_scale = 1.0;
   int nplanes = 0;
+  unsigned period_fp8 = 0;
+  int krot_fix = -1;
+  int epi_park = 0;
 };
 
 __global__ __launch_bounds__(256) void sparse2_meta_kernel(const int8_t *__restrict__ A, long lpad, long ldk,
diff --git a/gemma_amd/csrc/i8gemm_sparse2_r16.hip.h b/gemma_amd/csrc/i8gemm_sparse2_r16.hip.h
--- a/gemma_amd/csrc/i8gemm_sparse2_r16.hip.h
+++ b/gemma_amd/csrc/i8gemm_sparse2_r16.hip.h
@@ -1,5 +1,6 @@
 #pragma once
 #include "i8gemm_sparse2.hip.h"
+#include "i8_krot.h"
 
 #ifndef S2_R16_PREP_SPREAD
 #define S2_R16_PREP_SPREAD 0
@@ -17,6 +18,123 @@
 namespace gemma_hip {
 
 constexpr int S2_R16_LDS = S2_R16_NST * S2_STAGE;
+
+constexpr int S2_R16_PARK_SLOT = 512 * 16;
+template <bool WITH_S, bool PARK>
+__device__ __forceinline__ void s2_r16_combine(const Sparse2Args &g, const int8_t *mine, const i32x4 (&accg)[2][8],
+                                               const i32x4 (&accm)[2][8], int tm, int tn, int wave, int q, int r16, int odd) {
+  static_assert(!PARK || S2_R16_LDS >= 16 * S2_R16_PARK_SLOT, "the parked row group needs 128 KiB of LDS");
+  constexpr int KB = 2, NE = 4 * KB, NH = 8 / KB;
+  const int np = g.nplanes;
+  const bool load_m = !(g.anymiss && __builtin_amdgcn_readfirstlane(*g.anymiss) == 0);
+  const double w_hi = g.fuse ? 65536.0 : 256.0;
+  const double w0 = (g.fuse && !odd) ? 65536.0 : 256.0;
+  const long row_w = (long)tm * S2_BM + wave * 32, col_w = (long)tn * S2_BN;
+  const long row_l = row_w + 4 * q, col_l = col_w + r16;
+  const unsigned lo_c = (unsigned)((4 * q * g.ldc + r16) * 4), lo_x = (unsigned)((4 * q * g.ldx + r16) * 8);
+#define EP_AT(T, BASE, LO) (*(T *)((const char *)(BASE) + (LO)))
+#define EP_LOAD(DG, DM, I, H, P)                                                                                  \
+  do {                                                                                                            \
+    const int *cp_ = g.C + (long)(P) * g.strideC + (row_w + 16 * (I)) * g.ldc + col_w + 16 * KB * (H);            \
+    if (!PARK) {                                                                                                  \
+      _Pragma("unroll") for (int k_ = 0; k_ < KB; ++k_) _Pragma("unroll") for (int r_ = 0; r_ < 4; ++r_) {        \
+        DG[4 * k_ + r_] = EP_AT(const int, cp_ + r_ * g.ldc + 16 * k_, lo_c);                                     \
+        DM[4 * k_ + r_] = load_m ? EP_AT(const int, cp_ + (g.m_row0 + r_) * g.ldc + 16 * k_, lo_c) : 0;           \
+      }                                                                                                           \
+    } else {                                                                                                      \
+        \
+       \
+                      \
+      _Pragma("unroll") for (int r_ = 0; r_ < 4; ++r_) {                                                          \
+        ep_gint_t bg_ = (ep_gint_t)(cp_ + r_ * g.ldc), bm_ = (ep_gint_t)(cp_ + m_off + r_ * g.ldc);               \
+        asm("" : "+s"(bg_), "+s"(bm_));                                                                           \
+        _Pragma("unroll") for (int k_ = 0; k_ < KB; ++k_) {                                                       \
+          DG[4 * k_ + r_] = *(ep_gint_t)((ep_gchar_t)(bg_ + 16 * k_) + lo_c);                                     \
+          DM[4 * k_ + r_] = *(ep_gint_t)((ep_gchar_t)(bm_ + 16 * k_) + lo_c) & m_keep;                            \
+        }                                                                                                         \
+      }                                                                                                           \
+    }                                                                                                             \
+  } while (0)
+  const long m_off = load_m ? g.m_row0 * g.ldc : 0;
+  const int m_keep = load_m ? -1 : 0;
+  typedef const __attribute__((address_space(1))) int *ep_gint_t;
+  typedef const __attribute__((address_space(1))) char *ep_gchar_t;
+  int cg[NE], cm[NE], dg[NE], dm[NE];
+#pragma unroll
+  for (int e = 0; e < NE; ++e) cg[e] = cm[e] = dg[e] = dm[e] = 0;
+  if (np > 1) EP_LOAD(cg, cm, 0, 0, np - 1);
+  if (PARK) EP_LOAD(dg, dm, 0, 0, np - 2);
+  double qv[8], mv[2][4];
+  if (PARK) {
+#pragma unroll
+    for (int sb = 0; sb < 8; ++sb) qv[sb] = g.qinv[min(col_l + 16 * sb, g.n - 1)];
+#pragma unroll
+    for (int i = 0; i < 2; ++i)
+#pragma unroll
+      for (int r = 0; r < 4; ++r) mv[i][r] = g.mean[min(row_l + 16 * i + r, g.l - 1)];
+  }
+#pragma unroll
+  for (int b = 0; b < 2 * NH; ++b) {
+    const int i = b / NH, h = b % NH;
+    i32x4 ag[KB], am[KB];
+#pragma unroll
+    for (int k = 0; k < KB; ++k) {
+      const int sb = KB * h + k;
+      if (PARK && i == 1) {
+        ag[k] = *reinterpret_cast<const i32x4 *>(mine + sb * S2_R16_PARK_SLOT);
+        am[k] = WITH_S ? *reinterpret_cast<const i32x4 *>(mine + (8 + sb) * S2_R16_PARK_SLOT) : (i32x4){0, 0, 0, 0};
+      } else {
+        ag[k] = accg[i][sb];
+        am[k] = WITH_S ? accm[i][sb] : (i32x4){0, 0, 0, 0};
+      }
+    }
+    double tg[NE], tk[NE];
+#pragma unroll
+    for (int e = 0; e < NE; ++e) tg[e] = tk[e] = 0.0;
+    for (int p = np - 1; p >= 1; --p) {
+      int ng[NE], nm[NE];
+#pragma unroll
+      for (int e = 0; e < NE; ++e) ng[e] = nm[e] = 0;
+      if (!PARK) {
+        if (p > 1) EP_LOAD(ng, nm, i, h, p - 1);
+        else if (b < 2 * NH - 1) EP_LOAD(ng, nm, (b + 1) / NH, (b + 1) % NH, np - 1);
+      } else {
+        if (p > 2) EP_LOAD(ng, nm, i, h, p - 2);
+        else if (b < 2 * NH - 1) EP_LOAD(ng, nm, (b + 1) / NH, (b + 1) % NH, np - 3 + p);
+      }
+#pragma unroll
+      for (int e = 0; e < NE; ++e) {
+        tg[e] = tg[e] * w_hi + (double)cg[e];
+        tk[e] = tk[e] * w_hi + (double)cm[e];
+        if (PARK) {
+          cg[e] = dg[e]; cm[e] = dm[e];
+          dg[e] = ng[e]; dm[e] = nm[e];
+        } else {
+          cg[e] = ng[e];
+          cm[e] = nm[e];
+        }
+      }
+    }
+#pragma unroll
+    for (int r = 0; r < 4; ++r) {
+      const bool row_in = row_l + 16 * i + r < g.l;
+      double ms;
+      if (PARK) ms = row_in ? mv[i][r] * g.m_scale : 0.0;
+      else ms = row_in ? EP_AT(const double, g.mean + row_w + 16 * i + r, (unsigned)(32 * q)) * g.m_scale : 0.0;
+#pragma unroll
+      for (int k = 0; k < KB; ++k) {
+        const int e = 4 * k + r, sb = KB * h + k;
+        tg[e] = tg[e] * w0 + (double)ag[k][r];
+        tk[e] = tk[e] * w0 + (double)am[k][r];
+        if (row_in && col_l + 16 * sb < g.n)
+          EP_AT(double, g.UtX + (row_w + 16 * i + r) * g.ldx + col_w + 16 * sb, lo_x) =
+              fma(ms, tk[e], tg[e]) * (PARK ? qv[sb] : EP_AT(const double, g.qinv + col_w + 16 * sb, (unsigned)(8 * r16)));
+      }
+    }
+  }
+#undef EP_AT
+#undef EP_LOAD
+}
 
 template <bool WITH_S, bool COMBINE = false>
 __device__ __forceinline__ void s2_r16_body(const Sparse2Args &g) {
@@ -52,20 +170,42 @@
   const int wave = __builtin_amdgcn_readfirstlane(t >> 6);
   const int r16 = lane & 15, q = lane >> 4;
 
-  const uint4 *asrc[2];
-  const int8_t *bsrc[2];
+  const char *abase, *bbase;
+  unsigned aoff[2], boff[2];
   int adst[2], bdst[2];
+#pragma unroll
+  for (int j = 0; j < 2; ++j) {
+    const int qp = 2 * wave + j;
+    const int row = 16 * qp + (lane >> 2);
+    aoff[j] = (unsigned)((row * 4 + ((lane & 3) ^ ((row >> 2) & 3))) * 16);
+    adst[j] = qp * 1024;
+    const int col = 8 * qp + (lane >> 3);
+    boff[j] = (unsigned)(col * (int)g.ldk + 16 * ((lane & 7) ^ ((col >> 1) & 7)));
+    bdst[j] = S2_AMB + qp * 1024;
+  }
+  __shared__ int k0_of_wg;
+  int k0 = 0;
+  if (g.krot_fix >= 0) {
+    k0 = s2_krot_fix(g.krot_fix, g.nk);
+  } else if (g.period_fp8) {
+    if (t == 0) k0_of_wg = s2_krot_k0(wall_clock64(), g.period_fp8, g.nk);
+    __syncthreads();
+    k0 = k0_of_wg;
+  }
+  k0 = __builtin_amdgcn_readfirstlane(k0);
+  int kleft;
 #define GS_INIT_SRC(DIGIT)                                                                                        \
   do {                                                                                                            \
-    _Pragma("unroll") for (int j = 0; j < 2; ++j) {                                                               \
-      const int qp = 2 * wave + j;                                                                                \
-      const int row = 16 * qp + (lane >> 2);                                                                      \
-      asrc[j] = g.AM + ((long)tm * g.nk * S2_BM + row) * 4 + ((lane & 3) ^ ((row >> 2) & 3));                     \
-      adst[j] = qp * 1024;                                                                                        \
-      const int col = 8 * qp + (lane >> 3);                                                                       \
-      bsrc[j] = g.Bt + (long)(DIGIT) * g.strideB + ((long)tn * S2_BN + col) * g.ldk + 16 * ((lane & 7) ^ ((col >> 1) & 7)); \
-      bdst[j] = S2_AMB + qp * 1024;                                                                               \
-    }                                                                                                             \
+    abase = reinterpret_cast<const char *>(g.AM + ((long)tm * g.nk + k0) * S2_BM * 4);                            \
+    bbase = reinterpret_cast<const char *>(g.Bt + (long)(DIGIT) * g.strideB + (long)tn * S2_BN * g.ldk + (long)k0 * I8_BK); \
+    kleft = g.nk - k0;                                                                                            \
+  } while (0)
+#define GS_DMA_NEXT()                                                                                             \
+  do {                                                                                                            \
+    const bool wrap_ = kleft == 1;                                                                                \
+    abase += wrap_ ? -(long)(g.nk - 1) * (S2_BM * 64) : (long)(S2_BM * 64);                                       \
+    bbase += wrap_ ? -(long)(g.nk - 1) * I8_BK : (long)I8_BK;                                                     \
+    kleft = wrap_ ? g.nk : kleft - 1;                                                                             \
   } while (0)
   int ro[2], fo[2];
   {
@@ -91,13 +231,11 @@
 
 #define GS_DMA_A(j, SOFF)                                                                                         \
   do {                                                                                                            \
-    __builtin_amdgcn_global_load_lds((gemma_gptr_t)asrc[j], (gemma_lptr_t)(i8lds + (SOFF) + adst[j]), 16, 0, 0);  \
-    asrc[j] += S2_BM * 4;                                                                                         \
+    __builtin_amdgcn_global_load_lds((gemma_gptr_t)(abase + aoff[j]), (gemma_lptr_t)(i8lds + (SOFF) + adst[j]), 16, 0, 0); \
   } while (0)
 #define GS_DMA_B(j, SOFF)                                                                                         \
   do {                                                                                                            \
-    __builtin_amdgcn_global_load_lds((gemma_gptr_t)bsrc[j], (gemma_lptr_t)(i8lds + (SOFF) + bdst[j]), 16, 0, 0);  \
-    bsrc[j] += I8_BK;                                                                                             \
+    __builtin_amdgcn_global_load_lds((gemma_gptr_t)(bbase + boff[j]), (gemma_lptr_t)(i8lds + (SOFF) + bdst[j]), 16, 0, 0); \
   } while (0)
 #define GS_RREC(SOFF, i, P) rec[i][P] = *reinterpret_cast<const i32x4 *>(i8lds + (SOFF) + ro[P] + (i) * 1024)
 #define GS_RT(SOFF, SB, SL)                                                                                       \
@@ -147,7 +285,7 @@
     GS_STEP(0, 0, { GS_RT(SC, 3, 3); if (LOAD3) GS_DMA_A(0, SD); });                                               \
     GS_STEP(1, 1, { GS_RT(SC, 4, 0); if (LOAD3) GS_DMA_A(1, SD); });                                               \
     GS_STEP(2, 2, { GS_RT(SC, 5, 1); if (LOAD3) GS_DMA_B(0, SD); });                                               \
-    GS_STEP(3, 3, { GS_RT(SC, 6, 2); if (LOAD3) GS_DMA_B(1, SD); });                                               \
+    GS_STEP(3, 3, { GS_RT(SC, 6, 2); if (LOAD3) { GS_DMA_B(1, SD); GS_DMA_NEXT(); } });                            \
     GS_STEP(4, 0, { GS_RT(SC, 7, 3); });                                                                           \
     asm volatile("s_waitcnt vmcnt(" #VMW ")" ::: "memory");                                                       \
     __builtin_amdgcn_s_barrier();                                                                                 \
@@ -188,17 +326,21 @@
     GS_INIT_SRC(d_first - dd);
 #pragma unroll
     for (int j = 0; j < 2; ++j) { GS_DMA_A(j, 0); GS_DMA_B(j, 0); }
+    GS_DMA_NEXT();
     if (nk > 1) {
 #pragma unroll
       for (int j = 0; j < 2; ++j) { GS_DMA_A(j, S2_STAGE); GS_DMA_B(j, S2_STAGE); }
+      GS_DMA_NEXT();
     }
     if (nk > 2) {
 #pragma unroll
       for (int j = 0; j < 2; ++j) { GS_DMA_A(j, 2 * S2_STAGE); GS_DMA_B(j, 2 * S2_STAGE); }
+      GS_DMA_NEXT();
     }
     if (S2_R16_NST == 5 && nk > 3) {
 #pragma unroll
       for (int j = 0; j < 2; ++j) { GS_DMA_A(j, 3 * S2_STAGE); GS_DMA_B(j, 3 * S2_STAGE); }
+      GS_DMA_NEXT();
       asm volatile("s_waitcnt vmcnt(12)" ::: "memory");
     } else if (nk > 2) {
       asm volatile("s_waitcnt vmcnt(8)" ::: "memory");
@@ -255,64 +397,19 @@
 
   asm volatile("s_nop 15\n\ts_nop 7" ::: "memory");
   if constexpr (COMBINE) {
-    const int np = g.nplanes;
-    const bool load_m = !(g.anymiss && __builtin_amdgcn_readfirstlane(*g.anymiss) == 0);
-    const double w_hi = g.fuse ? 65536.0 : 256.0;
-    const double w0 = (g.fuse && !odd) ? 65536.0 : 256.0;
-    const long row_w = (long)tm * S2_BM + wave * 32, col_w = (long)tn * S2_BN;
-    const long row_l = row_w + 4 * q, col_l = col_w + r16;
-    const unsigned lo_c = (unsigned)((4 * q * g.ldc + r16) * 4), lo_x = (unsigned)((4 * q * g.ldx + r16) * 8);
-#define EP_AT(T, BASE, LO) (*(T *)((const char *)(BASE) + (LO)))
-#define EP_LOAD(DG, DM, I, H, P)                                                                                  \
-  do {                                                                                                            \
-    const int *cp_ = g.C + (long)(P) * g.strideC + (row_w + 16 * (I)) * g.ldc + col_w + 32 * (H);                 \
-    _Pragma("unroll") for (int k_ = 0; k_ < 2; ++k_) _Pragma("unroll") for (int r_ = 0; r_ < 4; ++r_) {           \
-      DG[4 * k_ + r_] = EP_AT(const int, cp_ + r_ * g.ldc + 16 * k_, lo_c);                                       \
-      DM[4 * k_ + r_] = load_m ? EP_AT(const int, cp_ + (g.m_row0 + r_) * g.ldc + 16 * k_, lo_c) : 0;             \
-    }                                                                                                             \
-  } while (0)
-    int cg[8], cm[8];
-#pragma unroll
-    for (int e = 0; e < 8; ++e) cg[e] = cm[e] = 0;
-    if (np > 1) EP_LOAD(cg, cm, 0, 0, np - 1);
-#pragma unroll
-    for (int b = 0; b < 8; ++b) {
-      const int i = b >> 2, h = b & 3;
-      double tg[8], tk[8];
-#pragma unroll
-      for (int e = 0; e < 8; ++e) tg[e] = tk[e] = 0.0;
-      for (int p = np - 1; p >= 1; --p) {
-        int ng[8], nm[8];
-#pragma unroll
-        for (int e = 0; e < 8; ++e) ng[e] = nm[e] = 0;
-        if (p > 1) EP_LOAD(ng, nm, i, h, p - 1);
-        else if (b < 7) EP_LOAD(ng, nm, (b + 1) >> 2, (b + 1) & 3, np - 1);
-#pragma unroll
-        for (int e = 0; e < 8; ++e) {
-          tg[e] = tg[e] * w_hi + (double)cg[e];
-          tk[e] = tk[e] * w_hi + (double)cm[e];
-          cg[e] = ng[e];
-          cm[e] = nm[e];
-        }
-      }
-#pragma unroll
-      for (int r = 0; r < 4; ++r) {
-        const bool row_in = row_l + 16 * i + r < g.l;
-        const double ms = row_in ? EP_AT(const double, g.mean + row_w + 16 * i + r, (unsigned)(32 * q)) * g.m_scale : 0.0;
-#pragma unroll
-        for (int k = 0; k < 2; ++k) {
-          const int e = 4 * k + r, sb = 2 * h + k;
-          const int m0 = WITH_S ? accm[i][sb][r] : 0;
-          tg[e] = tg[e] * w0 + (double)accg[i][sb][r];
-          tk[e] = tk[e] * w0 + (double)m0;
-          if (row_in && col_l + 16 * sb < g.n)
-            EP_AT(double, g.UtX + (row_w + 16 * i + r) * g.ldx + col_w + 16 * sb, lo_x) =
-                fma(ms, tk[e], tg[e]) * EP_AT(const double, g.qinv + col_w + 16 * sb, (unsigned)(8 * r16));
-        }
-      }
-    }
-#undef EP_AT
-#undef EP_LOAD
+    if (g.epi_park && g.nplanes >= 3) {
+      __builtin_amdgcn_s_barrier();
+      int8_t *mine = i8lds + 16 * t;
+#pragma unroll
+      for (int j = 0; j < 8; ++j) {
+        *reinterpret_cast<i32x4 *>(mine + j * S2_R16_PARK_SLOT) = accg[1][j];
+        if (WITH_S) *reinterpret_cast<i32x4 *>(mine + (8 + j) * S2_R16_PARK_SLOT) = accm[1][j];
+      }
+      asm volatile("" ::: "memory");
+      s2_r16_combine<WITH_S, true>(g, mine, accg, accm, tm, tn, wave, q, r16, odd);
+    } else {
+      s2_r16_combine<WITH_S, false>(g, i8lds, accg, accm, tm, tn, wave, q, r16, odd);
+    }
   } else {
     int *Cg = g.C + (long)plane * g.strideC;
 #pragma unroll
@@ -329,6 +426,7 @@
       }
   }
 #undef GS_INIT_SRC
+#undef GS_DMA_NEXT
 #undef GS_DMA_A
 #undef GS_DMA_B
 #undef GS_RREC
```

Result: no change. 357,400 (-1.0%).
